# yangfei1223/CRFConv

Measured on AMD Instinct MI355X. Metric: M points/sec fwd+bwd, S3DIS 40960-pt cloud, K=16, 3 CRF iters; mIoU parity, higher is better.
Workload: dtype f32; 1 GPU; BASELINE configs[1]: S3DIS-like synthetic clouds (one point per 4 cm voxel of an 8x8x3 m box), 4 clouds x 40960 pts per GPU, K=16, ratios [4,4,4,4,2], PointConvBig(in=6, classes=13, use_crf, steps=3), train mode: fwd + weighted CE + bwd + flat-bucket grad all-reduce + SGD(momentum) step; tables resident in HBM; point order from the device collate: morton; global_batch=4, points_per_cloud=40960, parallelism=dp1 (batch-sharded)

## Files before the change

### crfconv_amd/_lib.py

```python
import ctypes
import os

_HERE = os.path.dirname(os.path.abspath(__file__))
LIB_PATH = os.environ.get('CRFCONV_LIB') or os.path.join(_HERE, 'libcrfconv_amd.so')

_vp, _i, _i64, _sz, _f = ctypes.c_void_p, ctypes.c_int, ctypes.c_int64, ctypes.c_size_t, ctypes.c_float
_d = ctypes.c_double
_u64 = ctypes.c_uint64

SIGNATURES = {
    'crfconv_abi_version': (_i, []),
    'crfconv_last_error': (ctypes.c_char_p, []),
    'crfconv_knn': (_i, [_vp, _sz, _sz, _vp, _sz, _sz, _vp]),
    'crfconv_knn_omp': (_i, [_vp, _sz, _sz, _vp, _sz, _sz, _vp]),
    'crfconv_knn_batch': (_i, [_vp, _sz, _sz, _sz, _vp, _sz, _sz, _vp]),
    'crfconv_knn_batch_omp': (_i, [_vp, _sz, _sz, _sz, _vp, _sz, _sz, _vp]),
    'crfconv_knn_batch_dev_workspace': (_sz, [_sz, _sz, _sz, _sz]),
    'crfconv_knn_batch_dev': (_i, [_vp, _sz, _sz, _sz, _vp, _sz, _sz, _vp, _vp, _vp, _sz, _vp]),
    'crfconv_fps': (_i, [_vp, _i, _vp, _vp, _vp, _vp, _vp, _vp, _vp, _vp]),
    'crfconv_grid_subsample': (_i64, [_vp, _i64, _vp, _i, _vp, _i, _f, _vp, _vp, _vp, _i64]),
    'crfconv_grid_subsample_dev_workspace': (_sz, [_i64, _i, _i]),
    'crfconv_grid_subsample_dev': (_i64, [_vp, _i64, _vp, _i, _vp, _i, _f, _vp, _vp, _vp, _i64, _vp, _sz, _vp]),
    'crfconv_index_narrow': (_i, [_vp, _i64, _i64, _i, _i64, _vp, _vp, _vp, _vp]),
    'crfconv_index_narrow_sorted': (_i, [_vp, _i64, _i64, _i, _i64, _i, _vp, _vp, _vp, _vp]),
    'crfconv_reverse_csr_workspace': (_sz, [_i64, _i64]),
    'crfconv_reverse_csr': (_i, [_vp, _i64, _i64, _vp, _vp, _vp, _sz, _vp]),
    'crfconv_reverse_csr_batched_workspace': (_sz, [_vp, _i]),
    'crfconv_reverse_csr_batched': (_i, [_vp, _i, _vp, _sz, _vp]),
    'crfconv_meanfield_forward': (_i, [_vp, _vp, _vp, _i, _i, _i64, _i, _vp, _vp, _i, _vp, _vp, _vp]),
    'crfconv_meanfield_forward_u16': (_i, [_vp, _vp, _vp, _vp, _i, _i, _i, _i, _i64, _i, _vp, _vp, _i, _vp, _vp, _vp]),
    'crfconv_meanfield_forward_block_rows': (_i, [_i64, _i, _i, _i, _i]),
    'crfconv_meanfield_forward_block': (_i, [_vp, _vp, _vp, _vp, _i, _i, _i, _i, _i64, _i, _vp, _vp, _i, _vp, _vp, _vp, _vp]),
    'crfconv_meanfield_forward_block_stamps': (_i, [_vp, _vp, _vp, _vp, _i, _i, _i64, _vp, _vp, _i, _vp, _vp, _vp, _i, _vp, _vp]),
    'crfconv_block_locality': (_i, [_vp, _i64, _i, _i, _i, _vp, _vp]),
    'crfconv_meanfield_bwd_edge': (_i, [_vp, _vp, _vp, _vp, _i, _i, _i64, _i, _vp, _vp, _vp, _vp, _i, _vp]),
    'crfconv_meanfield_bwd_scatter': (_i, [_vp, _vp, _vp, _vp, _i, _i, _i64, _i, _vp, _vp, _vp]),
    'crfconv_meanfield_backward_supported': (_i, [_i, _i, _i]),
    'crfconv_meanfield_backward_param_grads_inside': (_i, [_i]),
    'crfconv_meanfield_backward_workspace': (_sz, [_i64, _i, _i]),
    'crfconv_meanfield_backward': (_i, [_vp] * 7 + [_i, _i, _vp, _vp, _i, _i, _i64, _i, _vp, _vp, _i] + [_vp] * 11 + [_sz, _vp, _vp]),
    'crfconv_wide_similarity': (_i, [_vp, _vp, _i, _i, _i64, _i, _vp, _vp]),
    'crfconv_wide_aggregate': (_i, [_vp, _vp, _vp, _i, _i, _i64, _i, _vp, _vp]),
    'crfconv_wide_bwd_edge': (_i, [_vp, _vp, _vp, _i, _i, _i64, _i, _vp, _i, _vp]),
    'crfconv_wide_scatter': (_i, [_vp, _vp, _vp, _vp, _i, _i64, _i, _vp, _i, _vp, _vp]),
    'crfconv_wide_similarity_bwd': (_i, [_vp, _vp, _vp, _vp, _i, _i, _i64, _i, _vp, _vp, _vp]),
    'crfconv_similarity_bwd': (_i, [_vp, _vp, _vp, _vp, _i, _i, _i64, _i, _vp, _vp, _vp]),
    'crfconv_similarity_bwd_scatter': (_i, [_vp, _vp, _vp, _vp, _vp, _i, _i, _i64, _i, _vp, _vp]),
    'crfconv_pointconv_workspace': (_sz, [_i64, _i, _i]),
    'crfconv_pointconv_moments_packed': (_i, [_vp, _vp, _vp, _i, _i64, ctypes.c_double, _vp, _vp, _vp, _vp, _vp, _sz, _vp]),
    'crfconv_pointconv_moments': (_i, [_vp, _vp, _vp, _i, _i64, _vp, _vp, _sz, _vp]),
    'crfconv_pointconv_stats': (_i, [_vp, _vp, _vp, _i, _i64, _i, _vp, _vp, _vp, _f, _vp, _vp, _vp, _vp, _sz, _vp]),
    'crfconv_pointconv_forward_uv': (_i, [_vp, _vp, _vp, _vp, _i, _i64, _i, _vp, _vp, _vp, _f, _vp, _vp, _vp, _vp, _vp, _vp, _sz, _vp, _vp]),
    'crfconv_pointconv_forward_uv_hosts': (_i, [_i, _i]),
    'crfconv_pointconv_forward_uv_hosting': (_i, [_vp, _vp, _vp, _vp, _i, _i64, _i, _vp, _vp, _vp, _f, _vp, _vp, _vp, _vp, _vp, _vp, _sz, _vp,
                                                  _vp, _vp, _i, _vp, _vp, _vp]),
    'crfconv_pointconv_combine': (_i, [_vp, _vp, _vp, _vp, _vp, _vp, _d, _vp, _vp, _f, _f, _i64, _i, _vp, _vp, _vp, _vp, _vp]),
    'crfconv_pointconv_bwd_reduce_uv': (_i, [_vp, _vp, _vp, _i64, _i, _vp, _vp, _vp, _d, _i, _vp, _vp, _vp, _vp, _vp, _vp, _sz, _vp, _vp]),
    'crfconv_pointconv_forward': (_i, [_vp, _vp, _vp, _vp, _i, _i64, _i, _vp, _vp, _vp, _f, _vp, _vp, _vp, _vp]),
    'crfconv_pointconv_bwd_reduce': (_i, [_vp, _vp, _vp, _vp, _vp, _i, _i64, _i, _vp, _vp, _vp, _f, _vp, _vp, _vp, _sz, _vp]),
    'crfconv_pointconv_bwd_params': (_i, [_vp, _vp, _vp, _vp, _vp, _i, _i64, _i, _vp, _vp, _vp, _f, _vp, _vp, _vp,
                                          _vp, _vp, _vp, _sz, _vp]),
    'crfconv_pointconv_bwd_dump': (_i, [_vp, _vp, _vp, _vp, _vp, _i, _i64, _i, _vp, _vp, _vp, _f, _vp, _vp, _vp, _vp, _vp, _vp, _vp]),
    'crfconv_pointconv_bwd_a1_workspace': (_sz, [_i64, _i]),
    'crfconv_pointconv_bwd_a1': (_i, [_vp, _vp, _vp, _i64, _i, _f, _vp, _vp, _sz, _vp]),
    'crfconv_pointconv_bwd_input': (_i, [_vp, _vp, _vp, _vp, _vp, _i, _i64, _i, _vp, _vp, _vp, _f, _vp, _vp, _vp, _vp]),
    'crfconv_pointconv_bwd_input_reduce': (_i, [_vp, _vp, _vp, _vp, _vp, _i, _i64, _i64, _i, _vp, _vp, _vp, _f, _vp, _vp, _vp, _vp, _vp, _vp, _vp, _vp, _d, _i,
                                                _vp, _vp, _vp, _vp, _vp, _vp, _sz, _vp, _vp]),
    'crfconv_pointconv_fold1': (_i, [_vp, _vp, _vp, _vp, ctypes.c_double, _vp, _vp, _f, _f, _i, _i, _vp, _vp, _vp, _vp]),
    'crfconv_pointconv_fold1_batched': (_i, [_vp, _i, _vp]),
    'crfconv_pointconv_fold1_bwd_batched': (_i, [_vp, _i, _vp]),
    'crfconv_pointconv_fold1_bwd': (_i, [_vp, _vp, _vp, _vp, _vp, _f, _i, _i, _vp, _vp, _vp, _vp, _vp, _vp]),
    'crfconv_pointconv_fold2': (_i, [_vp, _vp, _vp, _vp, ctypes.c_double, _vp, _vp, _f, _f, _i, _i, _vp, _vp, _vp, _vp]),
    'crfconv_pointconv_fold2_bwd': (_i, [_vp, _vp, _vp, _vp, ctypes.c_double, _i, _i, _vp, _vp, _vp, _vp, _vp, _vp]),
    'crfconv_linear_wgrad_workspace': (_sz, [_i64, _i, _i]),
    'crfconv_linear_wgrad': (_i, [_vp, _vp, _i64, _i, _i, _vp, _vp, _vp, _sz, _vp]),
    'crfconv_random_subsets': (_i, [_vp, _vp, _vp, _vp, _i, _u64, _vp, _vp]),
    'crfconv_upindex_workspace': (_sz, [_i64, _i64]),
    'crfconv_upindex_from_table': (_i, [_vp, _vp, _vp, _vp, _i64, _i64, _i, _i64, _vp, _vp, _sz, _vp]),
    'crfconv_gather_rows_batched': (_i, [_vp, _vp, _vp, _i, _vp, _i, _i64, _i64, _i64, _vp]),
    'crfconv_argsort_codes_workspace': (_sz, [_i64, _i64]),
    'crfconv_argsort_codes': (_i, [_vp, _i64, _i64, _vp, _vp, _sz, _vp]),
    'crfconv_gridsync_workspace': (_sz, []),
    'crfconv_gridsync_fail_word': (_i, []),
    'crfconv_mlp_small_supported': (_i, [_i64, _i, _i]),
    'crfconv_mlp_small_workspace': (_sz, [_i64, _i]),
    'crfconv_mlp_small_forward': (_i, [_vp, _vp, _i64, _i, _i, _vp, _vp, _vp, _vp, _f, _f, _f, _vp, _vp, _vp, _vp, _sz, _vp, _sz, _vp]),
    'crfconv_mlp_small_forward_join': (_i, [_vp, _vp, _i64, _i, _i, _vp, _vp, _vp, _vp, _f, _f, _f, _vp, _f, _vp, _vp, _vp, _vp, _sz, _vp, _sz, _vp]),
    'crfconv_ticket_bytes': (_sz, []),
    'crfconv_mlp_backward_supported': (_i, [_i64, _i, _i]),
    'crfconv_mlp_backward_workspace': (_sz, [_i64, _i, _i]),
    'crfconv_mlp_backward': (_i, [_vp, _vp, _vp, _vp, _vp, _f, _i64, _i, _i, _vp, _vp, _vp, _vp, _vp, _sz, _vp, _vp]),
    'crfconv_linear_forward_cat': (_i, [_vp, _vp, _i, _vp, _vp, _i64, _i, _i, _vp, _vp, _vp]),
    'crfconv_mlp_dw_jobs': (_i, [_vp, _i, _vp]),
    'crfconv_mlp_dw_jobs_hosting': (_i, [_vp, _i, _vp, _vp, _vp, _vp, _vp, _i, _vp, _vp]),
    'crfconv_mlp_backward_add': (_i, [_vp, _vp, _vp, _vp, _vp, _f, _i64, _i, _i, _vp, _vp, _vp, _vp, _vp, _vp, _sz, _vp, _vp]),
    'crfconv_mlp_backward_cat': (_i, [_vp, _vp, _vp, _vp, _i, _vp, _vp, _f, _i64, _i, _i, _vp, _vp, _vp, _vp, _vp, _vp, _sz, _vp, _vp]),
    'crfconv_bn_workspace': (_sz, [_i64, _i]),
    'crfconv_bn_forward': (_i, [_vp, _i64, _i, _vp, _vp, _vp, _vp, _f, _f, _i, _f, _vp, _vp, _vp, _sz, _vp]),
    'crfconv_bn_backward': (_i, [_vp, _vp, _vp, _i64, _i, _i, _f, _vp, _vp, _vp, _vp, _sz, _vp]),
    'crfconv_bn_apply': (_i, [_vp, _i64, _i, _vp, _f, _vp, _vp]),
    'crfconv_pointconv_bwd_params_slabs': (_i, [_vp, _i64, _i, _vp, _vp, _vp]),
    'crfconv_pointconv_bwd_a1_nblk': (_i64, [_i64, _i]),
    'crfconv_reduce_jobs_f64': (_i, [_vp, _i, _vp]),
    'crfconv_pointconv_bwd_dump_jobs': (_i, [_vp, _i, _vp]),
    'crfconv_pointconv_bwd_a1_jobs': (_i, [_vp, _i, _vp]),
    'crfconv_pointconv_wide_params_supported': (_i, [_i64, _i, _i]),
    'crfconv_pointconv_wide_params_nblk': (_i64, [_i64, _i]),
    'crfconv_pointconv_wide_params_jobs': (_i, [_vp, _i, _vp]),
    'crfconv_gemm_jobs': (_i, [_vp, _i, _vp]),
    'crfconv_linear_wgrad_nblk': (_i, [_i64, _i, _i]),
    'crfconv_linear_wgrad_partial_jobs': (_i, [_vp, _i, _vp]),
    'crfconv_linear_wgrad_partial': (_i, [_vp, _vp, _i64, _i, _i, _i, _vp, _sz, _vp, _vp]),
    'crfconv_morton_codes': (_i, [_vp, _i64, _i64, _vp, _vp, _vp]),
    'crfconv_copy_jobs': (_i, [_vp, _i, _vp]),
    'crfconv_index_narrow_batched': (_i, [_vp, _i, _vp]),
    'crfconv_pointconv_moments_batched_workspace': (_sz, [_vp, _i]),
    'crfconv_pointconv_moments_batched': (_i, [_vp, _i, _vp, _sz, _vp]),
    'crfconv_reduce_jobs_both': (_i, [_vp, _i, _vp, _i, _vp]),
    'crfconv_reduce_jobs': (_i, [_vp, _i, _vp]),
    'crfconv_linear_forward_supported': (_i, [_i, _i]),
    'crfconv_linear_forward_stat_records': (_sz, [_i64]),
    'crfconv_linear_forward': (_i, [_vp, _vp, _vp, _i64, _i, _i, _i, _vp, _vp, _vp]),
    'crfconv_cat2': (_i, [_vp, _vp, _i64, _i, _i, _vp, _vp]),
    'crfconv_split2': (_i, [_vp, _i64, _i, _i, _vp, _vp, _vp]),
    'crfconv_add_i64': (_i, [_vp, _i64, _i64, _vp]),
    'crfconv_gate_mark': (_i, [_vp, _vp]),
    'crfconv_gate_wait': (_i, [_vp, _i, _vp]),
    'crfconv_mlp_small_backward_supported': (_i, [_i64, _i, _i]),
    'crfconv_gemm_stats_jobs': (_i, [_vp, _i, _vp]),
    'crfconv_bn_apply_from_records_jobs': (_i, [_vp, _i, _vp]),
    'crfconv_mlp_small_backward_jobs': (_i, [_vp, _i, _vp, _vp]),
    'crfconv_mlp_small_backward_jobs_one_launch': (_i, [_vp, _i, _vp, _vp, _vp]),
    'crfconv_mlp_small_backward_workspace': (_sz, [_i64, _i]),
    'crfconv_mlp_small_backward': (_i, [_vp, _vp, _vp, _vp, _vp, _i64, _i, _i, _i, _f, _vp, _vp, _vp, _vp, _vp, _sz, _vp, _vp]),
    'crfconv_gemm_stat_records': (_sz, [_i64]),
    'crfconv_gemm_stats': (_i, [_vp, _vp, _i64, _i, _i, _vp, _vp, _vp]),
    'crfconv_gemm_supported': (_i, [_i64, _i, _i]),
    'crfconv_gemm': (_i, [_vp, _vp, _vp, _vp, _i64, _i, _i, _i, _vp, _vp]),
    'crfconv_bn_apply_from_records': (_i, [_vp, _i64, _vp, _i64, _i, _vp, _vp, _vp, _vp, _f, _f, _vp, _f, _vp, _vp, _vp]),
    'crfconv_bn_coef_from_nrecords': (_i, [_vp, _i64, _i64, _i, _vp, _vp, _vp, _vp, _f, _f, _vp, _vp]),
    'crfconv_bn_coef_from_records': (_i, [_vp, _i64, _i, _vp, _vp, _vp, _vp, _f, _f, _vp, _vp]),
    'crfconv_softmax_ce_workspace': (_sz, [_i64]),
    'crfconv_softmax_ce_forward': (_i, [_vp, _vp, _vp, _i64, _i, _i64, _i64, _vp, _vp, _vp, _vp, _sz, _vp, _vp]),
    'crfconv_softmax_ce_backward': (_i, [_vp, _vp, _vp, _vp, _vp, _vp, _i64, _i, _i64, _i64, _vp, _vp]),
    'crfconv_crf_matrices': (_i, [_vp, _i, _vp, _vp, _vp]),
    'crfconv_crf_matrices_backward': (_i, [_vp, _vp, _vp, _vp, _i, _vp, _vp]),
    'crfconv_crf_matrices_batched': (_i, [_vp, _vp, _i, _vp, _vp, _vp]),
    'crfconv_crf_matrices_backward_batched': (_i, [_vp, _vp, _vp, _vp, _vp, _i, _vp, _vp]),
    'crfconv_add_lrelu': (_i, [_vp, _vp, _i64, _f, _vp, _vp]),
    'crfconv_bn_apply_add': (_i, [_vp, _i64, _i, _vp, _vp, _f, _vp, _vp]),
    'crfconv_bn_apply_dropout': (_i, [_vp, _i64, _i, _vp, _f, _f, _u64, _vp, _vp, _vp, _vp]),
    'crfconv_head_stats': (_i, [_vp, _vp, _i64, _i, _i, _vp, _vp]),
    'crfconv_head_stat_records': (_sz, [_i64]),
    'crfconv_head_supported': (_i, [_i64, _i, _i, _i]),
    'crfconv_head_mask_words': (_sz, [_i64]),
    'crfconv_head_backward_workspace': (_sz, [_i64, _i, _i, _i]),
    'crfconv_head_forward': (_i, [_vp, _vp, _vp, _f, _f, _u64, _vp, _vp, _vp, _i64, _i, _i, _i, _vp, _vp, _vp, _vp]),
    'crfconv_head_backward': (_i, [_vp, _vp, _vp, _vp, _f, _f, _vp, _vp, _i64, _i, _i, _i] + [_vp] * 7 + [_sz, _vp]),
    'crfconv_linear_forward_dropout': (_i, [_vp, _vp, _i64, _i, _i, _i, _f, _u64, _vp, _vp, _vp]),
    'crfconv_dropout_backward': (_i, [_vp, _i64, _f, _u64, _vp, _vp, _vp]),
    'crfconv_add_lrelu_backward': (_i, [_vp, _vp, _i64, _f, _vp, _vp]),
    'crfconv_sgd_step': (_i, [_vp, _vp, _vp, _i64, _f, _f, _f, _f, _i, _i, _vp]),
    'crfconv_sgd_step_hyper': (_i, [_vp, _vp, _vp, _i64, _vp, _i, _i, _vp]),
    'crfconv_sgd_step_guarded': (_i, [_vp, _vp, _vp, _i64, _vp, _i, _i, _vp, _vp]),
    'crfconv_sgd_step_guarded_all': (_i, [_vp, _vp, _vp, _i64, _vp, _i, _i, _vp, _i, _vp, _vp]),
    'crfconv_sgd_guard_publish': (_i, [_vp, _i, _vp, _vp]),
    'crfconv_spd_inverse': (_i, [_vp, _i, _vp, _vp]),
    'crfconv_spd_inverse_wide': (_i, [_vp, _i, _vp, _vp]),
    'crfconv_neighbor_maxpool_forward': (_i, [_vp, _vp, _i, _i64, _i, _vp, _vp, _vp]),
    'crfconv_neighbor_maxpool_affine_forward': (_i, [_vp, _vp, _vp, _i, _i64, _i, _vp, _vp, _vp]),
    'crfconv_neighbor_maxpool_backward': (_i, [_vp, _vp, _vp, _vp, _i, _i64, _i, _vp, _vp]),
    'crfconv_gather_rows': (_i, [_vp, _vp, _i64, _i, _vp, _vp]),
    'crfconv_gather_rows_backward': (_i, [_vp, _vp, _vp, _i64, _i, _vp, _vp]),
    'crfconv_meanfield_step': (_i, [_vp, _vp, _vp, _vp, _i, _i, _i64, _i, _vp, _vp, _vp, _vp]),
    'crfconv_kernel_weights_forward': (_i, [_vp, _vp, _i, _vp, _i, _i, _i64, _vp, _vp]),
    'crfconv_kernel_weights_partials': (_sz, [_i64]),
    'crfconv_kernel_weights_backward': (_i, [_vp, _vp, _vp, _vp, _vp, _i, _vp, _i, _i, _i64, _vp, _vp, _vp, _vp]),
    'crfconv_confusion_accumulate': (_i, [_vp, _vp, _vp, _i64, _i, _i64, _i64, _vp, _vp, _vp]),
    'crfconv_vote_accumulate': (_i, [_vp, _vp, _vp, _i64, _i, _d, _vp, _i64, _vp, _vp]),
    'crfconv_vote_accumulate_counted': (_i, [_vp, _vp, _vp, _i64, _i, _d, _vp, _i64, _vp, _vp, _vp]),
    'crfconv_vote_fold': (_i, [_vp, _vp, _vp, _vp, _i64, _i, _d, _vp]),
    'crfconv_vote_project': (_i, [_vp, _vp, _i64, _i, _i64, _i, _vp, _vp, _vp]),
    'crfconv_argmin_workspace': (_sz, []),
    'crfconv_argmin_f64': (_i, [_vp, _i64, _vp, _vp, _vp, _sz, _vp]),
    'crfconv_possibility_crop_workspace': (_sz, [_i64, _i64]),
    'crfconv_possibility_crop': (_i, [_vp, _i64, _i64, _vp, _vp, _vp, _vp, _vp, _vp, _vp, _vp, _vp, _sz, _vp]),
}



class ReduceJob(ctypes.Structure):
    _fields_ = [('partial', ctypes.c_void_p), ('out', ctypes.c_void_p), ('nblk', ctypes.c_int32), ('nslots', ctypes.c_int32)]


class CopyJob(ctypes.Structure):
    _fields_ = [('src', ctypes.c_void_p), ('dst', ctypes.c_void_p), ('nbytes', ctypes.c_int64)]


class MlpDwJob(ctypes.Structure):
    _fields_ = [('workspace', ctypes.c_void_p), ('coef', ctypes.c_void_p), ('dW', ctypes.c_void_p), ('M', ctypes.c_int64),
                ('Ci', ctypes.c_int32), ('Co', ctypes.c_int32)]


class PcDumpJob(ctypes.Structure):
    _fields_ = [('x', ctypes.c_void_p), ('gout', ctypes.c_void_p), ('pos_src', ctypes.c_void_p), ('pos_tgt', ctypes.c_void_p),
                ('idx32', ctypes.c_void_p), ('K', ctypes.c_int32), ('m_tgt', ctypes.c_int64), ('d', ctypes.c_int32), ('A1', ctypes.c_void_p),
                ('b1', ctypes.c_void_p), ('W2', ctypes.c_void_p), ('slope', ctypes.c_float), ('ca', ctypes.c_void_p), ('cb', ctypes.c_void_p),
                ('cc', ctypes.c_void_p), ('h1', ctypes.c_void_p), ('gh2', ctypes.c_void_p), ('rel', ctypes.c_void_p)]


class PcWideJob(ctypes.Structure):
    _fields_ = [('x', ctypes.c_void_p), ('gout', ctypes.c_void_p), ('pos_src', ctypes.c_void_p), ('pos_tgt', ctypes.c_void_p),
                ('idx32', ctypes.c_void_p), ('K', ctypes.c_int32), ('m_tgt', ctypes.c_int64), ('d', ctypes.c_int32), ('A1', ctypes.c_void_p),
                ('b1', ctypes.c_void_p), ('W2', ctypes.c_void_p), ('slope', ctypes.c_float), ('ca', ctypes.c_void_p), ('cb', ctypes.c_void_p),
                ('cc', ctypes.c_void_p), ('dw2_partial', ctypes.c_void_p), ('a1_partial', ctypes.c_void_p)]


class PcA1Job(ctypes.Structure):
    _fields_ = [('gw', ctypes.c_void_p), ('h1', ctypes.c_void_p), ('rel', ctypes.c_void_p), ('n_edges', ctypes.c_int64), ('d', ctypes.c_int32),
                ('slope', ctypes.c_float), ('workspace', ctypes.c_void_p), ('workspace_bytes', ctypes.c_size_t)]


class GemmJob(ctypes.Structure):
    _fields_ = [('A', ctypes.c_void_p), ('B', ctypes.c_void_p), ('C', ctypes.c_void_p), ('M', ctypes.c_int64), ('N', ctypes.c_int32),
                ('K', ctypes.c_int32)]


class GemmStatsJob(ctypes.Structure):
    _fields_ = [('A', ctypes.c_void_p), ('B', ctypes.c_void_p), ('M', ctypes.c_int64), ('N', ctypes.c_int32), ('K', ctypes.c_int32),
                ('C', ctypes.c_void_p), ('stat_rec', ctypes.c_void_p)]


class BnApplyJob(ctypes.Structure):
    _fields_ = [('stat_rec', ctypes.c_void_p), ('nrec', ctypes.c_int64), ('x', ctypes.c_void_p), ('M', ctypes.c_int64), ('C', ctypes.c_int32),
                ('gamma', ctypes.c_void_p), ('beta', ctypes.c_void_p), ('run_mean', ctypes.c_void_p), ('run_var', ctypes.c_void_p),
                ('momentum', ctypes.c_float), ('eps', ctypes.c_float), ('skip', ctypes.c_void_p), ('slope', ctypes.c_float),
                ('coef', ctypes.c_void_p), ('y', ctypes.c_void_p)]


class MlpBwdJob(ctypes.Structure):
    _fields_ = [('gA', ctypes.c_void_p), ('Y', ctypes.c_void_p), ('coef', ctypes.c_void_p), ('W', ctypes.c_void_p), ('addend', ctypes.c_void_p),
                ('M', ctypes.c_int64), ('Ci', ctypes.c_int32), ('Co', ctypes.c_int32), ('training', ctypes.c_int32), ('slope', ctypes.c_float),
                ('gY', ctypes.c_void_p), ('dX', ctypes.c_void_p), ('dgamma', ctypes.c_void_p), ('dbeta', ctypes.c_void_p),
                ('workspace', ctypes.c_void_p), ('workspace_bytes', ctypes.c_size_t)]


class Reduce64Job(ctypes.Structure):
    _fields_ = [('partial', ctypes.c_void_p), ('is_float', ctypes.c_int32), ('nblk', ctypes.c_int64), ('nslots', ctypes.c_int32),
                ('out', ctypes.c_void_p)]


class WgradJob(ctypes.Structure):
    _fields_ = [('G', ctypes.c_void_p), ('X', ctypes.c_void_p), ('M', ctypes.c_int64), ('Co', ctypes.c_int32), ('Ci', ctypes.c_int32),
                ('want_bias', ctypes.c_int32), ('workspace', ctypes.c_void_p), ('workspace_bytes', ctypes.c_size_t)]


class RevJob(ctypes.Structure):
    _fields_ = [('idx32', ctypes.c_void_p), ('E', ctypes.c_int64), ('m_src', ctypes.c_int64), ('rev_ptr', ctypes.c_void_p),
                ('rev_eid', ctypes.c_void_p)]


class NarrowJob(ctypes.Structure):
    _fields_ = [('idx64', ctypes.c_void_p), ('B', ctypes.c_int64), ('n_tgt', ctypes.c_int64), ('K', ctypes.c_int32),
                ('n_src', ctypes.c_int64), ('sort_from', ctypes.c_int32), ('idx32', ctypes.c_void_p), ('idx16', ctypes.c_void_p),
                ('bad_count', ctypes.c_void_p)]


class MomentsJob(ctypes.Structure):
    _fields_ = [('pos_src', ctypes.c_void_p), ('pos_tgt', ctypes.c_void_p), ('idx32', ctypes.c_void_p), ('K', ctypes.c_int32),
                ('m_tgt', ctypes.c_int64), ('n_edges', ctypes.c_double), ('mean', ctypes.c_void_p), ('cov', ctypes.c_void_p),
                ('packed', ctypes.c_void_p), ('mean32', ctypes.c_void_p)]


class Fold1Job(ctypes.Structure):
    _fields_ = [('W1', ctypes.c_void_p), ('gamma1', ctypes.c_void_p), ('beta1', ctypes.c_void_p), ('mom', ctypes.c_void_p),
                ('n_edges', ctypes.c_double), ('run_mean', ctypes.c_void_p), ('run_var', ctypes.c_void_p),
                ('momentum', ctypes.c_float), ('eps', ctypes.c_float), ('use_batch', ctypes.c_int32), ('d', ctypes.c_int32),
                ('A1', ctypes.c_void_p), ('b1', ctypes.c_void_p), ('aux1', ctypes.c_void_p)]


class Fold1BwdJob(ctypes.Structure):
    _fields_ = [('W1', ctypes.c_void_p), ('gamma1', ctypes.c_void_p), ('mom', ctypes.c_void_p), ('aux1', ctypes.c_void_p),
                ('dA1b1', ctypes.c_void_p), ('eps', ctypes.c_float), ('use_batch', ctypes.c_int32), ('d', ctypes.c_int32),
                ('pad_', ctypes.c_int32), ('dW1', ctypes.c_void_p), ('dgamma1', ctypes.c_void_p), ('dbeta1', ctypes.c_void_p),
                ('dW2_f64', ctypes.c_void_p), ('dW2_f32', ctypes.c_void_p)]


_lib = None


class CrfConvError(RuntimeError):
    pass


def load():
    global _lib
    if _lib is None:
        if not os.path.exists(LIB_PATH):
            raise CrfConvError(
                '%s not found: build it with `make -C crfconv_amd/csrc` (or __graft_entry__.build()). '
                'crfconv_amd has no CPU / PyTorch fallback.' % LIB_PATH)
        lib = ctypes.CDLL(LIB_PATH)
        for name, (res, args) in SIGNATURES.items():
            fn = getattr(lib, name)
            fn.restype = res
            fn.argtypes = args
        if lib.crfconv_abi_version() != 1:
            raise CrfConvError('libcrfconv_amd.so ABI version mismatch')
        _lib = lib
    return _lib


def last_error():
    return load().crfconv_last_error().decode('utf-8', 'replace')


def check(rc, what=''):
    if rc < 0:
        raise CrfConvError('%s failed (%d): %s' % (what or 'libcrfconv_amd call', rc, last_error()))
    return rc


_FN = {}


def call(name, *args):
    fn = _FN.get(name)
    if fn is None:
        fn = _FN[name] = getattr(load(), name)
    rc = fn(*args)
    if rc < 0:
        check(rc, name)
    return rc
```

### crfconv_amd/csrc/linear.hip

```cpp
#include "common.hpp"
#include "gridsync.hpp"
#include "wgrad_body.hpp"
#include "crf_matrices_body.hpp"
#include "reduce64_body.hpp"

#include <cstdlib>

namespace crf {

template <int TCO, int TCI>
__global__ __launch_bounds__(WG_BLOCK) void wgrad_kernel(const float* __restrict__ G,
                                                         const float* __restrict__ X, int64_t M, int Co,
                                                         int Ci, int rows_per_block,
                                                         float* __restrict__ partial ,
                                                         float* __restrict__ partial_b ) {
    __shared__ float s_red[WG_RED_BUFS * TCO * TCI * 256];
    __shared__ float s_b[WG_WAVES * TCO * 16];
    wgrad_body<TCO, TCI>(G, X, M, Co, Ci, rows_per_block, partial, partial_b, blockIdx.x, blockIdx.y, blockIdx.z, s_red, s_b);
}

__global__ __launch_bounds__(WG_BLOCK) void wgrad_jobs_any_kernel(const WgJobTable t) {
    __shared__ float s_red[WG_RED_BUFS * 4 * 4 * 256];
    __shared__ float s_b[WG_WAVES * 4 * 16];
    wgrad_any_run(t, (int)blockIdx.x, s_red, s_b);
}


__device__ __forceinline__ void mlp_channel_part(int c, double s1, double s2, const float* __restrict__ coef, int64_t M, int Co,
                                                 float* __restrict__ dgamma, float* __restrict__ dbeta, float* __restrict__ bcoef) {
    dbeta[c] = (float)s1;
    dgamma[c] = (float)s2;
    const double a = coef[c], mu = coef[2 * Co + c], rs = coef[3 * Co + c];
    const double c2 = s1 / (double)M, c3 = s2 / (double)M;
    bcoef[c] = coef[c];
    bcoef[Co + c] = coef[Co + c];
    bcoef[2 * Co + c] = (float)a;
    bcoef[3 * Co + c] = (float)(-a * c3 * rs);
    bcoef[4 * Co + c] = (float)(-a * c2 + a * c3 * rs * mu);
}

template <int TCO, int TCI>
__global__ __launch_bounds__(WG_BLOCK) void mlp_bwd_p1_kernel(const float* __restrict__ GA, const float* __restrict__ Y,
                                                              const float* __restrict__ X,
                                                              const float* __restrict__ X2, int split ,
                                                              const float* __restrict__ coef ,
                                                              float slope, int64_t M, int Co, int Ci, int rows_per_block,
                                                              float* __restrict__ PA ,
                                                              float* __restrict__ PB ,
                                                              float* __restrict__ PG ,
                                                              float* __restrict__ PX ,
                                                              unsigned* __restrict__ ticket ,
                                                              float* __restrict__ dgamma, float* __restrict__ dbeta,
                                                              float* __restrict__ bcoef) {
    const int lane = threadIdx.x & 63, wave = threadIdx.x >> 6;
    const int co_base = blockIdx.y * 16 * TCO, ci_base = blockIdx.z * 16 * TCI;
    const int kk = lane >> 4, cc = lane & 15;
    f32x4 accA[TCO][TCI], accB[TCO][TCI];
#pragma unroll
    for (int a = 0; a < TCO; ++a)
#pragma unroll
        for (int b = 0; b < TCI; ++b) { accA[a][b] = f32x4{0.f, 0.f, 0.f, 0.f}; accB[a][b] = f32x4{0.f, 0.f, 0.f, 0.f}; }
    float ca[TCO], cb[TCO], cm[TCO], cr[TCO], sg[TCO], sgy[TCO], sx[TCI];
#pragma unroll
    for (int a = 0; a < TCO; ++a) {
        const int co = co_base + 16 * a + cc;
        const bool ok = co < Co;
        ca[a] = ok ? coef[co] : 0.f;
        cb[a] = ok ? coef[Co + co] : 0.f;
        cm[a] = ok ? coef[2 * Co + co] : 0.f;
        cr[a] = ok ? coef[3 * Co + co] : 0.f;
        sg[a] = 0.f;
        sgy[a] = 0.f;
    }
#pragma unroll
    for (int b = 0; b < TCI; ++b) sx[b] = 0.f;

    const int64_t row_begin = (int64_t)blockIdx.x * rows_per_block;
    const int64_t row_end = row_begin + rows_per_block < M ? row_begin + rows_per_block : M;
#ifndef P1_PREFETCH_
#define P1_PREFETCH_ 0
#endif
    struct Frag { float gv[4][TCO], yv[4][TCO], bv[4][TCI]; };
    auto load = [&](int64_t r0, Frag& f) {
#pragma unroll
        for (int u = 0; u < 4; ++u) {
            const int64_t r = r0 + 4 * u + kk;
            const bool rv = r < row_end;
#pragma unroll
            for (int a = 0; a < TCO; ++a) {
                const int co = co_base + 16 * a + cc;
                const bool ok = rv && co < Co;
                f.gv[u][a] = ok ? GA[r * Co + co] : 0.f;
                f.yv[u][a] = ok ? Y[r * Co + co] : cm[a];
            }
#pragma unroll
            for (int b = 0; b < TCI; ++b) {
                const int ci = ci_base + 16 * b + cc;
                float xv = 0.f;
                if (rv && ci < Ci) xv = (X2 == nullptr || ci < split) ? X[r * (X2 ? split : Ci) + ci] : X2[r * (Ci - split) + (ci - split)];
                f.bv[u][b] = xv;
            }
        }
    };
    auto compute = [&](const Frag& f) {
#pragma unroll
        for (int u = 0; u < 4; ++u) {
#pragma unroll
            for (int b = 0; b < TCI; ++b) sx[b] += f.bv[u][b];
#pragma unroll
            for (int a = 0; a < TCO; ++a) {
                const float g1 = f.gv[u][a] * (fmaf(ca[a], f.yv[u][a], cb[a]) > 0.f ? 1.f : slope);
                const float yh = (f.yv[u][a] - cm[a]) * cr[a];
                sg[a] += g1;
                sgy[a] = fmaf(g1, yh, sgy[a]);
#pragma unroll
                for (int b = 0; b < TCI; ++b) {
                    accA[a][b] = __builtin_amdgcn_mfma_f32_16x16x4f32(g1, f.bv[u][b], accA[a][b], 0, 0, 0);
                    accB[a][b] = __builtin_amdgcn_mfma_f32_16x16x4f32(yh, f.bv[u][b], accB[a][b], 0, 0, 0);
                }
            }
        }
    };
    if constexpr (P1_PREFETCH_ != 0) {
        Frag cur, nxt;
        load(row_begin + 16 * wave, cur);
        for (int64_t r0 = row_begin + 16 * wave; r0 < row_end; r0 += 16 * WG_WAVES) {
            load(r0 + 16 * WG_WAVES, nxt);
            compute(cur);
            cur = nxt;
        }
    } else {
        for (int64_t r0 = row_begin + 16 * wave; r0 < row_end; r0 += 16 * WG_WAVES) {
            Frag f;
            load(r0, f);
            compute(f);
        }
    }
    __shared__ __attribute__((aligned(16))) float s_red[WG_WAVES][TCO * TCI * 256];
    __shared__ float s_v[WG_WAVES][(2 * TCO + TCI) * 16];
    const int64_t pb = (int64_t)blockIdx.x;
    for (int pass = 0; pass < 2; ++pass) {
        if (pass) __syncthreads();
#pragma unroll
        for (int a = 0; a < TCO; ++a)
#pragma unroll
            for (int b = 0; b < TCI; ++b)
#pragma unroll
                for (int g = 0; g < 4; ++g)
                    s_red[wave][(a * TCI + b) * 256 + (4 * kk + g) * 16 + cc] = pass ? accB[a][b][g] : accA[a][b][g];
        if (pass == 0) {
#pragma unroll
            for (int a = 0; a < TCO; ++a) {
                float t1 = sg[a], t2 = sgy[a];
                t1 += __shfl_xor(t1, 16, WAVE); t1 += __shfl_xor(t1, 32, WAVE);
                t2 += __shfl_xor(t2, 16, WAVE); t2 += __shfl_xor(t2, 32, WAVE);
                if (kk == 0) { s_v[wave][a * 16 + cc] = t1; s_v[wave][(TCO + a) * 16 + cc] = t2; }
            }
#pragma unroll
            for (int b = 0; b < TCI; ++b) {
                float t1 = sx[b];
                t1 += __shfl_xor(t1, 16, WAVE); t1 += __shfl_xor(t1, 32, WAVE);
                if (kk == 0) s_v[wave][(2 * TCO + b) * 16 + cc] = t1;
            }
        }
        __syncthreads();
        float* dst = pass ? PB : PA;
        for (int t = threadIdx.x; t < TCO * TCI * 256; t += WG_BLOCK) {
            float v = 0.f;
#pragma unroll
            for (int w = 0; w < WG_WAVES; ++w) v += s_red[w][t];
            const int tile = t >> 8, a = tile / TCI, b = tile % TCI, i = (t >> 4) & 15, j = t & 15;
            const int co = co_base + 16 * a + i, ci = ci_base + 16 * b + j;
            if (co < Co && ci < Ci) dst[(pb * Co + co) * Ci + ci] = v;
        }
    }
    const __amdgpu_buffer_rsrc_t pgr = make_rsrc(PG, (int)gridDim.x * 2 * Co * 4);
    for (int t = threadIdx.x; t < (2 * TCO + TCI) * 16; t += WG_BLOCK) {
        float v = 0.f;
#pragma unroll
        for (int w = 0; w < WG_WAVES; ++w) v += s_v[w][t];
        const int grp = t >> 4, c16 = t & 15;
        if (grp < 2 * TCO) {
            const int which = grp / TCO, co = co_base + 16 * (grp % TCO) + c16;
            if (blockIdx.z == 0 && co < Co) st1_sc1(pgr, (((int)pb * 2 + which) * Co + co) * 4, v);
        } else {
            const int ci = ci_base + 16 * (grp - 2 * TCO) + c16;
            if (blockIdx.y == 0 && ci < Ci) PX[pb * Ci + ci] = v;
        }
    }
    constexpr bool ALIAS = TCO * TCI >= 3;
    __shared__ double s_own[ALIAS ? 1 : 5 * WG_BLOCK];
    __shared__ int s_flag;
    if (ticket == nullptr || !last_workgroup(ticket, gridDim.x * gridDim.y * gridDim.z, &s_flag)) return;
    double* s_buf = ALIAS ? reinterpret_cast<double*>(&s_red[0][0]) : s_own;
    double* s_tot = s_buf + 4 * WG_BLOCK;
    sum_partial_rows_f64<WG_BLOCK>(pgr, (int)gridDim.x, 2 * Co, s_buf, s_tot);
    if ((int)threadIdx.x < Co) mlp_channel_part(threadIdx.x, s_tot[threadIdx.x], s_tot[Co + threadIdx.x], coef, M, Co, dgamma, dbeta, bcoef);
}

constexpr int MF_BLOCK = 1024, MF_WAVES = MF_BLOCK / WAVE;
__device__ __forceinline__ void mlp_dw_slots(const float* __restrict__ PA, const float* __restrict__ PB,
                                             const float* __restrict__ PG, const float* __restrict__ PX, int nblk,
                                             const float* __restrict__ coef, int64_t M, int Co, int Ci, int block,
                                             float* __restrict__ dW) {
    const int lane = threadIdx.x & 63, w = threadIdx.x >> 6;
    __shared__ float s_part[MF_WAVES][5][64];
    const int nslots = Co * Ci;
    const int slot = block * 64 + lane;
    const bool ok = slot < nslots;
    const int sl = ok ? slot : nslots - 1;
    const int co = sl / Ci, ci = sl - co * Ci;
    float a0 = 0.f, b0 = 0.f, x0 = 0.f, g1 = 0.f, g2 = 0.f;
    const int64_t sa = (int64_t)MF_WAVES * Co * Ci, sx = (int64_t)MF_WAVES * Ci, sg = (int64_t)MF_WAVES * 2 * Co;
    const float* pa = PA + ((int64_t)w * Co + co) * Ci + ci;
    const float* pb = PB + ((int64_t)w * Co + co) * Ci + ci;
    const float* px = PX + (int64_t)w * Ci + ci;
    const float* pg = PG + (int64_t)w * 2 * Co + co;
#pragma unroll 1
    for (int b = w; b < nblk; b += 4 * MF_WAVES) {
        float va[4], vb[4], vx[4], vg[4], vh[4];
#pragma unroll
        for (int u = 0; u < 4; ++u) {
            const bool in = b + MF_WAVES * u < nblk;
            va[u] = in ? pa[u * sa] : 0.f;
            vb[u] = in ? pb[u * sa] : 0.f;
            vx[u] = in ? px[u * sx] : 0.f;
            vg[u] = in ? pg[u * sg] : 0.f;
            vh[u] = in ? pg[u * sg + Co] : 0.f;
        }
#pragma unroll
        for (int u = 0; u < 4; ++u) { a0 += va[u]; b0 += vb[u]; x0 += vx[u]; g1 += vg[u]; g2 += vh[u]; }
        pa += 4 * sa; pb += 4 * sa; px += 4 * sx; pg += 4 * sg;
    }
    s_part[w][0][lane] = a0; s_part[w][1][lane] = b0; s_part[w][2][lane] = x0;
    s_part[w][3][lane] = g1; s_part[w][4][lane] = g2;
    __syncthreads();
    if (w == 0 && ok) {
        double A = 0.0, B = 0.0, Xs = 0.0, G1 = 0.0, G2 = 0.0;
        for (int k = 0; k < MF_WAVES; ++k) {
            A += s_part[k][0][lane]; B += s_part[k][1][lane]; Xs += s_part[k][2][lane];
            G1 += s_part[k][3][lane]; G2 += s_part[k][4][lane];
        }
        const double a = coef[co], c2 = G1 / (double)M, c3 = G2 / (double)M;
        dW[slot] = (float)(a * (A - c2 * Xs - c3 * B));
    }
}

__global__ __launch_bounds__(MF_BLOCK) void mlp_bwd_finalize_kernel(const float* __restrict__ PA, const float* __restrict__ PB,
                                                                    const float* __restrict__ PG, const float* __restrict__ PX,
                                                                    int nblk, const float* __restrict__ coef, int64_t M, int Co,
                                                                    int Ci, int nw, float* __restrict__ dW,
                                                                    float* __restrict__ dgamma, float* __restrict__ dbeta,
                                                                    float* __restrict__ bcoef) {
    const int lane = threadIdx.x & 63, w = threadIdx.x >> 6;
    if ((int)blockIdx.x >= nw) {
        const int c = ((int)blockIdx.x - nw) * MF_WAVES + w;
        if (c >= Co) return;
        double s1 = 0.0, s2 = 0.0;
        for (int b0 = lane; b0 < nblk; b0 += 8 * WAVE) {
            float v1[8], v2[8];
#pragma unroll
            for (int u = 0; u < 8; ++u) {
                const int b = b0 + u * WAVE;
                const bool in = b < nblk;
                v1[u] = in ? PG[((int64_t)b * 2 + 0) * Co + c] : 0.f;
                v2[u] = in ? PG[((int64_t)b * 2 + 1) * Co + c] : 0.f;
            }
#pragma unroll
            for (int u = 0; u < 8; ++u) { s1 += (double)v1[u]; s2 += (double)v2[u]; }
        }
#pragma unroll
        for (int o = 32; o > 0; o >>= 1) {
            s1 += __shfl_xor(s1, o, WAVE);
            s2 += __shfl_xor(s2, o, WAVE);
        }
        if (lane == 0) mlp_channel_part(c, s1, s2, coef, M, Co, dgamma, dbeta, bcoef);
        return;
    }
    mlp_dw_slots(PA, PB, PG, PX, nblk, coef, M, Co, Ci, (int)blockIdx.x, dW);
}

constexpr int MDW_MAX = 40;
struct MlpDwTable {
    const float* PA[MDW_MAX];
    const float* PB[MDW_MAX];
    const float* PG[MDW_MAX];
    const float* PX[MDW_MAX];
    const float* coef[MDW_MAX];
    float* dW[MDW_MAX];
    long long M[MDW_MAX];
    int nblk[MDW_MAX], Co[MDW_MAX], Ci[MDW_MAX];
    int group_begin[MDW_MAX + 1];
    int njobs;
};
__global__ __launch_bounds__(MF_BLOCK) void mlp_dw_jobs_kernel(const MlpDwTable t) {
    const int g = blockIdx.x;
    int lo = 0, hi = t.njobs;
    while (hi - lo > 1) {
        const int mid = (lo + hi) >> 1;
        if (t.group_begin[mid] <= g) lo = mid; else hi = mid;
    }
    mlp_dw_slots(t.PA[lo], t.PB[lo], t.PG[lo], t.PX[lo], t.nblk[lo], t.coef[lo], (int64_t)t.M[lo], t.Co[lo], t.Ci[lo],
                 g - t.group_begin[lo], t.dW[lo]);
}

__device__ __forceinline__ void reduce_slab64(const float* __restrict__ partial, int nblk, int nslots, int slot0,
                                              float* __restrict__ out, float (*s_part)[64]) {
    const int lane = threadIdx.x & 63, w = threadIdx.x >> 6;
    const int slot = slot0 + lane;
    const bool ok = slot < nslots;
    const float* p = partial + (ok ? slot : 0);
    float a0 = 0.f, a1 = 0.f, a2 = 0.f, a3 = 0.f;
    int b = w;
    for (; b + 28 < nblk; b += 32) {
        const float v0 = p[(int64_t)b * nslots], v1 = p[(int64_t)(b + 4) * nslots], v2 = p[(int64_t)(b + 8) * nslots];
        const float v3 = p[(int64_t)(b + 12) * nslots], v4 = p[(int64_t)(b + 16) * nslots], v5 = p[(int64_t)(b + 20) * nslots];
        const float v6 = p[(int64_t)(b + 24) * nslots], v7 = p[(int64_t)(b + 28) * nslots];
        a0 += v0; a1 += v1; a2 += v2; a3 += v3;
        a0 += v4; a1 += v5; a2 += v6; a3 += v7;
    }
    for (; b + 12 < nblk; b += 16) {
        a0 += p[(int64_t)b * nslots];
        a1 += p[(int64_t)(b + 4) * nslots];
        a2 += p[(int64_t)(b + 8) * nslots];
        a3 += p[(int64_t)(b + 12) * nslots];
    }
    for (; b < nblk; b += 4) a0 += p[(int64_t)b * nslots];
    s_part[w][lane] = (a0 + a1) + (a2 + a3);
    __syncthreads();
    if (w == 0 && ok) out[slot] = ((s_part[0][lane] + s_part[1][lane]) + s_part[2][lane]) + s_part[3][lane];
}

__global__ __launch_bounds__(256) void wgrad_reduce_kernel(const float* __restrict__ partial, int nblk,
                                                           int nslots, float* __restrict__ out) {
    __shared__ float s_part[4][64];
    reduce_slab64(partial, nblk, nslots, blockIdx.x * 64, out, s_part);
}

constexpr int RJ_MAX = 96;
struct ReduceJobTable {
    const float* partial[RJ_MAX];
    float* out[RJ_MAX];
    int nblk[RJ_MAX];
    int nslots[RJ_MAX];
    int group_begin[RJ_MAX + 1];
    int njobs;
};

__global__ __launch_bounds__(256) void reduce_jobs_kernel(const ReduceJobTable tbl) {
    __shared__ float s_part[4][64];
    const int g = blockIdx.x;
    int lo = 0, hi = tbl.njobs;
    while (hi - lo > 1) {
        const int mid = (lo + hi) >> 1;
        if (tbl.group_begin[mid] <= g) lo = mid; else hi = mid;
    }
    reduce_slab64(tbl.partial[lo], tbl.nblk[lo], tbl.nslots[lo], (g - tbl.group_begin[lo]) * 64, tbl.out[lo], s_part);
}


__global__ __launch_bounds__(256) void reduce_both_kernel(const ReduceJobTable tbl, const Reduce64Table t64, const int n64) {
    __shared__ float s_part[4][64];
    if ((int)blockIdx.x < n64) {
        reduce_jobs_f64_body(t64, blockIdx.x);
        return;
    }
    const int g = (int)blockIdx.x - n64;
    int lo = 0, hi = tbl.njobs;
    while (hi - lo > 1) {
        const int mid = (lo + hi) >> 1;
        if (tbl.group_begin[mid] <= g) lo = mid; else hi = mid;
    }
    reduce_slab64(tbl.partial[lo], tbl.nblk[lo], tbl.nslots[lo], (g - tbl.group_begin[lo]) * 64, tbl.out[lo], s_part);
}

}

using namespace crf;

extern "C" size_t crfconv_linear_wgrad_workspace(int64_t M, int Co, int Ci) {
    if (M <= 0 || Co <= 0 || Ci <= 0) return 0;
    const WgPlan p = wg_plan(M, Co, Ci);
    return sizeof(float) * (size_t)p.nblk * ((size_t)Co * Ci + (size_t)Co) + 256;
}

static int wgrad_launch(const float* G, const float* X, int64_t M, int Co, int Ci, const WgPlan& p, float* partial,
                        float* partial_b, hipStream_t st) {
    const dim3 grid((unsigned)p.nblk, (unsigned)p.gy, (unsigned)p.gz), blk(WG_BLOCK);
#define WG(TA, TB) hipLaunchKernelGGL((wgrad_kernel<TA, TB>), grid, blk, 0, st, G, X, M, Co, Ci, p.rows_per_block, partial, partial_b)
    switch (p.tco * 10 + p.tci) {
        case 11: WG(1, 1); break;
        case 12: WG(1, 2); break;
        case 14: WG(1, 4); break;
        case 21: WG(2, 1); break;
        case 22: WG(2, 2); break;
        case 24: WG(2, 4); break;
        case 41: WG(4, 1); break;
        case 42: WG(4, 2); break;
        default: WG(4, 4); break;
    }
#undef WG
    CRF_LAUNCH_CHECK();
    return CRF_OK;
}

extern "C" int crfconv_linear_wgrad_partial(const float* G, const float* X, int64_t M, int Co, int Ci, int want_bias,
                                            void* workspace, size_t workspace_bytes, int* nblk_out, crf_stream_t stream) {
// ... 65 lines not shown
    }
    return CRF_OK;
}

extern "C" int crfconv_reduce_jobs_f64(const crf_reduce64_job* jobs, int njobs, crf_stream_t stream);
extern "C" int crfconv_reduce_jobs_both(const crf_reduce_job* jobs, int njobs, const crf_reduce64_job* jobs64, int njobs64,
                                        crf_stream_t stream) {
    CRF_REQUIRE((jobs || njobs == 0) && (jobs64 || njobs64 == 0) && njobs >= 0 && njobs64 >= 0, CRF_ERR_ARG, "null pointer or negative count");
    if (njobs == 0 || njobs64 == 0 || njobs > RJ_MAX || njobs64 > R64_MAX) {
        if (njobs64 > 0)
            if (int rc = crfconv_reduce_jobs_f64(jobs64, njobs64, stream)) return rc;
        return njobs > 0 ? crfconv_reduce_jobs(jobs, njobs, stream) : CRF_OK;
    }
    ReduceJobTable tbl;
    int64_t total = 0;
    for (int j = 0; j < njobs; ++j) {
        const crf_reduce_job& jb = jobs[j];
        CRF_REQUIRE(jb.partial && jb.out && jb.nblk > 0 && jb.nslots > 0, CRF_ERR_ARG, "job %d is malformed", j);
        tbl.partial[j] = jb.partial; tbl.out[j] = jb.out; tbl.nblk[j] = jb.nblk; tbl.nslots[j] = jb.nslots;
        tbl.group_begin[j] = (int)total;
        total += (jb.nslots + 63) / 64;
    }
    for (int j = njobs; j <= RJ_MAX; ++j) tbl.group_begin[j] = (int)total;
    for (int j = njobs; j < RJ_MAX; ++j) { tbl.partial[j] = nullptr; tbl.out[j] = nullptr; tbl.nblk[j] = 0; tbl.nslots[j] = 0; }
    tbl.njobs = njobs;
    Reduce64Table t;
    int64_t waves = 0;
    for (int j = 0; j <= R64_MAX; ++j) {
        t.wave_base[j] = (int)waves;
        if (j < njobs64) {
            const crf_reduce64_job& jb = jobs64[j];
            CRF_REQUIRE(jb.partial && jb.out && jb.nblk > 0 && jb.nblk < ((int64_t)1 << 31) && jb.nslots > 0, CRF_ERR_ARG, "float64 job %d is malformed", j);
            t.partial[j] = jb.partial; t.out[j] = jb.out; t.is_float[j] = jb.is_float; t.nblk[j] = (int)jb.nblk; t.nslots[j] = jb.nslots;
            waves += jb.nslots;
        } else if (j < R64_MAX) {
            t.partial[j] = nullptr; t.out[j] = nullptr; t.is_float[j] = 0; t.nblk[j] = 0; t.nslots[j] = 0;
        }
    }
    t.njobs = njobs64;
    const int64_t n64 = cdiv(waves, 256 / WAVE);
    CRF_REQUIRE(total + n64 < ((int64_t)1 << 30), CRF_ERR_UNSUPPORTED, "too many slots in one batch");
    hipLaunchKernelGGL(reduce_both_kernel, dim3((unsigned)(total + n64)), dim3(256), 0, as_stream(stream), tbl, t, (int)n64);
    CRF_LAUNCH_CHECK();
    return CRF_OK;
}

extern "C" int crfconv_linear_wgrad(const float* G, const float* X, int64_t M, int Co, int Ci, float* dW,
                                    float* db, void* workspace, size_t workspace_bytes, crf_stream_t stream) {
    CRF_REQUIRE(G && X && dW && workspace, CRF_ERR_ARG, "null pointer");
    CRF_REQUIRE(M > 0 && Co > 0 && Ci > 0 && Co <= 4096 && Ci <= 4096, CRF_ERR_ARG, "bad shape M=%lld Co=%d Ci=%d",
                (long long)M, Co, Ci);
    CRF_REQUIRE(workspace_bytes >= crfconv_linear_wgrad_workspace(M, Co, Ci), CRF_ERR_WORKSPACE, "workspace too small");
    const WgPlan p = wg_plan(M, Co, Ci);
    hipStream_t st = as_stream(stream);
    float* partial = reinterpret_cast<float*>((reinterpret_cast<uintptr_t>(workspace) + 255) & ~(uintptr_t)255);
    float* partial_b = db ? partial + (size_t)p.nblk * Co * Ci : nullptr;
    if (int rc = wgrad_launch(G, X, M, Co, Ci, p, partial, partial_b, st)) return rc;
    hipLaunchKernelGGL(wgrad_reduce_kernel, dim3((unsigned)cdiv((int64_t)Co * Ci, 64)), dim3(256), 0, st, partial, p.nblk,
                       Co * Ci, dW);
    CRF_LAUNCH_CHECK();
    if (db) {
        hipLaunchKernelGGL(wgrad_reduce_kernel, dim3((unsigned)cdiv((int64_t)Co, 64)), dim3(256), 0, st, partial_b, p.nblk,
                           Co, db);
        CRF_LAUNCH_CHECK();
    }
    return CRF_OK;
}

namespace crf {
__device__ __forceinline__ void gauss_jordan_tiles(double (&t)[4][4], int H, double (*s_row)[64], double (*s_col)[64]) {
    const int tr = threadIdx.x >> 4, tc = threadIdx.x & 15;
#pragma unroll
    for (int ip = 0; ip < 4; ++ip) {
        for (int pp = 0; pp < 16; ++pp) {
            const int p = 16 * ip + pp;
            if (p >= H) break;
            const int b = p & 1;
            if (tr == pp) {
#pragma unroll
                for (int j = 0; j < 4; ++j) s_row[b][tc + 16 * j] = t[ip][j];
            }
            if (tc == pp) {
#pragma unroll
                for (int i = 0; i < 4; ++i) s_col[b][tr + 16 * i] = t[i][ip];
            }
            __syncthreads();
            const double piv = 1.0 / s_row[b][p];
            double rowv[4], colv[4];
#pragma unroll
            for (int j = 0; j < 4; ++j) rowv[j] = s_row[b][tc + 16 * j] * piv;
#pragma unroll
            for (int i = 0; i < 4; ++i) colv[i] = s_col[b][tr + 16 * i];
#pragma unroll
            for (int i = 0; i < 4; ++i)
#pragma unroll
                for (int j = 0; j < 4; ++j) {
                    const bool rp = (i == ip) && (tr == pp), cp = (j == ip) && (tc == pp);
                    const double upd = t[i][j] - colv[i] * rowv[j];
                    t[i][j] = rp ? (cp ? piv : rowv[j]) : (cp ? -colv[i] * piv : upd);
                }
        }
    }
}

__global__ __launch_bounds__(256) void spd_inverse_kernel(const float* __restrict__ Min, int H,
                                                          float* __restrict__ Qout) {
    __shared__ double s_row[2][64], s_col[2][64];
    const int tr = threadIdx.x >> 4, tc = threadIdx.x & 15;
    double t[4][4];
#pragma unroll
    for (int i = 0; i < 4; ++i)
#pragma unroll
        for (int j = 0; j < 4; ++j) {
            const int r = tr + 16 * i, c = tc + 16 * j;
            t[i][j] = (r < H && c < H) ? (double)Min[r * H + c] : (r == c ? 1.0 : 0.0);
        }
    gauss_jordan_tiles(t, H, s_row, s_col);
#pragma unroll
    for (int i = 0; i < 4; ++i)
#pragma unroll
        for (int j = 0; j < 4; ++j) {
            const int r = tr + 16 * i, c = tc + 16 * j;
            if (r < H && c < H) Qout[r * H + c] = (float)t[i][j];
        }
}

__global__ __launch_bounds__(CMF_BLOCK) void crf_matrices_kernel(const float* __restrict__ cmat, int H,
                                                           float* __restrict__ Qout, float* __restrict__ Pout) {
    __shared__ __attribute__((aligned(16))) char lds[CMF_LDS_BYTES];
    crf_matrices_body(cmat, H, Qout, Pout, lds);
}

__global__ __launch_bounds__(CMF_BLOCK) void crf_matrices_batched_kernel(const CrfMatJobs j) {
    const int b = blockIdx.x;
    __shared__ __attribute__((aligned(16))) char lds[CMF_LDS_BYTES];
    crf_matrices_body(j.c[b], j.H[b], j.Q[b], j.P[b], lds);
}

constexpr int CMB_ROWS = 8, CMB_BLOCK = CMB_ROWS * 64;
__device__ __forceinline__ void crf_matrices_bwd_slab(const float* __restrict__ cmat, const float* __restrict__ Q,
                                                      const float* __restrict__ dQ, const float* __restrict__ dP,
                                                      int H, int row0, float* __restrict__ dc) {
    __shared__ float s_q[64 * 65], s_d[64 * 65];
    __shared__ double s_t[2][CMB_ROWS][65];
    for (int e = threadIdx.x; e < H * H; e += (int)blockDim.x) {
        const int r = e / H, c = e % H;
        s_q[r * 65 + c] = Q[e];
        s_d[r * 65 + c] = (dQ ? dQ[e] : 0.f) - (dP ? dP[e] : 0.f);
    }
    const int r = (threadIdx.x >> 6) & (CMB_ROWS - 1), j = threadIdx.x & 63, row = row0 + r;
    const bool live = (int)threadIdx.x < CMB_BLOCK && row < H && j < H;
    if (live) s_t[0][r][j] = (double)cmat[row * H + j];
    __syncthreads();
    double acc = 0.0;
    if (live)
        for (int k = 0; k < H; ++k) acc += s_t[0][r][k] * (double)s_q[k * 65 + j];
    if (live) s_t[1][r][j] = acc;
    __syncthreads();
    acc = 0.0;
    if (live)
        for (int k = 0; k < H; ++k) acc += s_t[1][r][k] * ((double)s_d[k * 65 + j] + (double)s_d[j * 65 + k]);
    if (live) s_t[0][r][j] = acc;
    __syncthreads();
    acc = 0.0;
    if (live) {
        for (int k = 0; k < H; ++k) acc += s_t[0][r][k] * (double)s_q[k * 65 + j];
        dc[row * H + j] = (float)(-acc);
    }
}
__global__ __launch_bounds__(CMB_BLOCK) void crf_matrices_bwd_kernel(const float* __restrict__ cmat, const float* __restrict__ Q,
                                                               const float* __restrict__ dQ, const float* __restrict__ dP,
                                                               int H, float* __restrict__ dc) {
    crf_matrices_bwd_slab(cmat, Q, dQ, dP, H, (int)blockIdx.x * CMB_ROWS, dc);
}
__global__ __launch_bounds__(CMB_BLOCK) void crf_matrices_bwd_batched_kernel(const CrfMatJobs j) {
    int b = 0;
    while (b + 1 < CM_MAX && (int)blockIdx.x >= j.slab_base[b + 1]) ++b;
    crf_matrices_bwd_slab(j.c[b], j.Q_in[b], j.gQ[b], j.gP[b], j.H[b], ((int)blockIdx.x - j.slab_base[b]) * CMB_ROWS, j.dc[b]);
}
static_assert(MF_BLOCK >= CMB_BLOCK, "a rider fits the host's workgroup");
__global__ __launch_bounds__(MF_BLOCK) void mlp_dw_jobs_hosting_kernel(const MlpDwTable t, const CrfMatJobs j, const int n_side) {
    if ((int)blockIdx.x < n_side) {
        int b = 0;
        while (b + 1 < CM_MAX && (int)blockIdx.x >= j.slab_base[b + 1]) ++b;
        crf_matrices_bwd_slab(j.c[b], j.Q_in[b], j.gQ[b], j.gP[b], j.H[b], ((int)blockIdx.x - j.slab_base[b]) * CMB_ROWS, j.dc[b]);
        return;
    }
    const int g = (int)blockIdx.x - n_side;
    int lo = 0, hi = t.njobs;
    while (hi - lo > 1) {
        const int mid = (lo + hi) >> 1;
        if (t.group_begin[mid] <= g) lo = mid; else hi = mid;
    }
    mlp_dw_slots(t.PA[lo], t.PB[lo], t.PG[lo], t.PX[lo], t.nblk[lo], t.coef[lo], (int64_t)t.M[lo], t.Co[lo], t.Ci[lo],
                 g - t.group_begin[lo], t.dW[lo]);
}
}

extern "C" int crfconv_crf_matrices_batched(const float* const* c, const int* H, int n, float* const* Q, float* const* P,
                                            crf_stream_t stream) {
    CRF_REQUIRE(c && H && Q && P && n >= 1 && n <= crf::CM_MAX, CRF_ERR_ARG, "null pointer or n=%d outside [1, %d]", n, crf::CM_MAX);
    crf::CrfMatJobs j = {};
    for (int i = 0; i < n; ++i) {
        CRF_REQUIRE(c[i] && Q[i] && P[i] && H[i] >= 1 && H[i] <= 64, CRF_ERR_ARG, "job %d: null pointer or H=%d outside [1, 64]", i, H[i]);
        j.c[i] = c[i]; j.Q[i] = Q[i]; j.P[i] = P[i]; j.H[i] = H[i];
    }
    hipLaunchKernelGGL(crf::crf_matrices_batched_kernel, dim3((unsigned)n), dim3(crf::CMF_BLOCK), 0, crf::as_stream(stream), j);
    CRF_LAUNCH_CHECK();
    return CRF_OK;
}

static int crf_matrices_bwd_jobs(const float* const* c, const float* const* Q, const float* const* gQ, const float* const* gP, const int* H, int n,
                                 float* const* dc, crf::CrfMatJobs& j, int& nslab) {
    CRF_REQUIRE(c && Q && gQ && gP && H && dc && n >= 1 && n <= crf::CM_MAX, CRF_ERR_ARG, "null pointer or n=%d outside [1, %d]", n, crf::CM_MAX);
    j = crf::CrfMatJobs();
    for (int i = 0; i < n; ++i) {
        CRF_REQUIRE(c[i] && Q[i] && dc[i] && H[i] >= 1 && H[i] <= 64, CRF_ERR_ARG, "job %d: null pointer or H=%d outside [1, 64]", i, H[i]);
        j.c[i] = c[i]; j.Q_in[i] = Q[i]; j.gQ[i] = gQ[i]; j.gP[i] = gP[i]; j.dc[i] = dc[i]; j.H[i] = H[i];
        j.slab_base[i + 1] = j.slab_base[i] + (H[i] + crf::CMB_ROWS - 1) / crf::CMB_ROWS;
    }
    nslab = j.slab_base[n];
    for (int i = n; i < crf::CM_MAX; ++i) j.slab_base[i + 1] = 0x7fffffff;
    return CRF_OK;
}
extern "C" int crfconv_crf_matrices_backward_batched(const float* const* c, const float* const* Q, const float* const* gQ,
                                                     const float* const* gP, const int* H, int n, float* const* dc,
                                                     crf_stream_t stream) {
    crf::CrfMatJobs j;
    int nslab = 0;
    if (int rc = crf_matrices_bwd_jobs(c, Q, gQ, gP, H, n, dc, j, nslab)) return rc;
    hipLaunchKernelGGL(crf::crf_matrices_bwd_batched_kernel, dim3((unsigned)nslab), dim3(crf::CMB_BLOCK), 0, crf::as_stream(stream), j);
    CRF_LAUNCH_CHECK();
    return CRF_OK;
}

namespace crf {
constexpr int SW_BLOCK = 1024, SW_MAXH = 512;
__global__ __launch_bounds__(SW_BLOCK) void spd_inverse_wide_kernel(const float* __restrict__ M, int H, float* __restrict__ Q) {
    __shared__ float s_row[SW_MAXH], s_col[SW_MAXH];
    const int n = H * H;
    for (int e = threadIdx.x; e < n; e += SW_BLOCK) Q[e] = M[e];
    __syncthreads();
    for (int k = 0; k < H; ++k) {
        for (int t = threadIdx.x; t < H; t += SW_BLOCK) {
            s_row[t] = Q[k * H + t];
            s_col[t] = Q[t * H + k];
        }
        __syncthreads();
        const float inv = 1.0f / s_row[k];
        for (int e = threadIdx.x; e < n; e += SW_BLOCK) {
            const int i = e / H, j = e - i * H;
            float v;
            if (i == k) v = j == k ? inv : s_row[j] * inv;
            else if (j == k) v = -s_col[i] * inv;
            else v = fmaf(-s_col[i] * inv, s_row[j], Q[e]);
            Q[e] = v;
        }
        __syncthreads();
    }
}
}

extern "C" int crfconv_spd_inverse_wide(const float* M, int H, float* Q, crf_stream_t stream) {
    CRF_REQUIRE(M && Q && M != Q, CRF_ERR_ARG, "null pointer / aliased operands");
    CRF_REQUIRE(H >= 1 && H <= crf::SW_MAXH, CRF_ERR_UNSUPPORTED, "H=%d outside [1, %d]", H, crf::SW_MAXH);
    hipLaunchKernelGGL(crf::spd_inverse_wide_kernel, dim3(1), dim3(crf::SW_BLOCK), 0, crf::as_stream(stream), M, H, Q);
    CRF_LAUNCH_CHECK();
    return CRF_OK;
}

extern "C" int crfconv_spd_inverse(const float* M, int H, float* Q, crf_stream_t stream) {
    CRF_REQUIRE(M && Q, CRF_ERR_ARG, "null pointer");
    CRF_REQUIRE(H >= 1 && H <= 64, CRF_ERR_UNSUPPORTED, "H=%d outside [1, 64]", H);
    hipLaunchKernelGGL(crf::spd_inverse_kernel, dim3(1), dim3(256), 0, crf::as_stream(stream), M, H, Q);
    CRF_LAUNCH_CHECK();
    return CRF_OK;
}

extern "C" int crfconv_crf_matrices(const float* c, int H, float* Q, float* P, crf_stream_t stream) {
    CRF_REQUIRE(c && Q && P, CRF_ERR_ARG, "null pointer");
    CRF_REQUIRE(H >= 1 && H <= 64, CRF_ERR_UNSUPPORTED, "H=%d outside [1, 64]", H);
    hipLaunchKernelGGL(crf::crf_matrices_kernel, dim3(1), dim3(crf::CMF_BLOCK), 0, crf::as_stream(stream), c, H, Q, P);
    CRF_LAUNCH_CHECK();
    return CRF_OK;
}

extern "C" int crfconv_crf_matrices_backward(const float* c, const float* Q, const float* dQ, const float* dP, int H,
                                             float* dc, crf_stream_t stream) {
    CRF_REQUIRE(c && Q && dc, CRF_ERR_ARG, "null pointer");
    CRF_REQUIRE(H >= 1 && H <= 64, CRF_ERR_UNSUPPORTED, "H=%d outside [1, 64]", H);
    hipLaunchKernelGGL(crf::crf_matrices_bwd_kernel, dim3((unsigned)((H + crf::CMB_ROWS - 1) / crf::CMB_ROWS)), dim3(crf::CMB_BLOCK), 0,
                       crf::as_stream(stream), c, Q, dQ, dP, H, dc);
    CRF_LAUNCH_CHECK();
    return CRF_OK;
}

namespace crf {

#ifndef LF_BLOCK_
#define LF_BLOCK_ 256
#endif
constexpr int LF_BLOCK = LF_BLOCK_, LF_WAVES = LF_BLOCK / WAVE;

constexpr int EPI_NONE = 0, EPI_ADD = 1, EPI_DROPOUT = 2;
#ifndef LF_PF_MAX_
#define LF_PF_MAX_ 4
#endif
template <int TCO, bool PRO = false, bool VEC4 = true, int EPI = EPI_NONE, int NCH = 0>
__global__ __launch_bounds__(LF_BLOCK) void linear_fwd_kernel(const float* __restrict__ X, const float* __restrict__ W,
                                                              const float* __restrict__ bias, int64_t M, int Ci, int Co,
                                                              int transpose_w, float* __restrict__ Y,
                                                              float* __restrict__ stat_partial ,
                                                              const float* __restrict__ Y2 = nullptr,
                                                              const float* __restrict__ pro = nullptr, float slope = 1.f,
                                                              const float* __restrict__ Xb = nullptr, int xsplit = 0,
                                                              float* __restrict__ Yb = nullptr, int ysplit = 0,
                                                              const float* __restrict__ addend = nullptr,
                                                              const long long* __restrict__ drop_counter = nullptr,
                                                              unsigned long long drop_seed = 0ull, unsigned drop_threshold = 0u,
                                                              float drop_scale = 1.f) {
    extern __shared__ float sW[];
    const int Cip = ((Ci + 15) / 16) * 16 + 4;
    const int Cik = ((Ci + 15) / 16) * 16;
    float* sPro = sW + 16 * TCO * Cip;
    [[maybe_unused]] float* sTile = sPro + (PRO ? 5 * Cik : 0);
    if constexpr (PRO) {
        for (int t = threadIdx.x; t < 5 * Cik; t += LF_BLOCK) {
            const int which = t / Cik, k = t - which * Cik;
            sPro[t] = k < Ci ? pro[which * Ci + k] : 0.f;
        }
    }
    const int co_base = blockIdx.y * 16 * TCO;
    if (!transpose_w && (Ci % 4) == 0) {
        const int Cip4 = Cip / 4, Ci4 = Ci / 4;
        for (int t = threadIdx.x; t < 16 * TCO * Cip4; t += LF_BLOCK) {
            const int r = t / Cip4, k4 = t - r * Cip4;
            const int co = co_base + r;
            float4 v = make_float4(0.f, 0.f, 0.f, 0.f);
            if (co < Co && k4 < Ci4) v = *reinterpret_cast<const float4*>(W + (int64_t)co * Ci + 4 * k4);
            *reinterpret_cast<float4*>(sW + r * Cip + 4 * k4) = v;
        }
    } else {
        for (int t = threadIdx.x; t < 16 * TCO * Cip; t += LF_BLOCK) {
            const int r = t / Cip, k = t - r * Cip;
            const int co = co_base + r;
            float v = 0.f;
            if (co < Co && k < Ci) v = transpose_w ? W[(int64_t)k * Co + co] : W[(int64_t)co * Ci + k];
            sW[t] = v;
        }
    }
    __syncthreads();
    const int lane = threadIdx.x & 63, wave = threadIdx.x >> 6;
    const int rr = lane & 15, g = lane >> 4;
    const bool vec = (Ci % 4) == 0;
    float bsel[TCO][4];
#pragma unroll
    for (int t = 0; t < TCO; ++t)
#pragma unroll
        for (int e = 0; e < 4; ++e) {
            const int co = co_base + 16 * t + 4 * g + e;
            bsel[t][e] = (bias != nullptr && co < Co) ? bias[co] : 0.f;
        }
    float s1[TCO][4], s2[TCO][4], sh[TCO][4];
#pragma unroll
    for (int t = 0; t < TCO; ++t)
#pragma unroll
        for (int e = 0; e < 4; ++e) { s1[t][e] = 0.f; s2[t][e] = 0.f; sh[t][e] = 0.f; }
    bool have_shift = false;
    const int nchunk = (Ci + 15) / 16;

    const float4 zero4 = make_float4(0.f, 0.f, 0.f, 0.f);
    auto load_raw = [&](int64_t r, bool rv, int c, float4& xa, float4& xb2) {
        const int k0 = 16 * c + 4 * g;
        xa = zero4;
        xb2 = zero4;
        if (!rv || k0 >= Ci) return;
        if constexpr (PRO) {
            xa = *reinterpret_cast<const float4*>(X + r * Ci + k0);
            xb2 = *reinterpret_cast<const float4*>(Y2 + r * Ci + k0);
        } else if (Xb != nullptr) {
            if (k0 < xsplit) xa = *reinterpret_cast<const float4*>(X + r * xsplit + k0);
            else xa = *reinterpret_cast<const float4*>(Xb + r * (Ci - xsplit) + (k0 - xsplit));
        } else if (VEC4 || vec) {
            xa = *reinterpret_cast<const float4*>(X + r * Ci + k0);
        } else if constexpr (!VEC4) {
            const float* xp = X + r * Ci;
            xa.x = xp[k0];
            xa.y = k0 + 1 < Ci ? xp[k0 + 1] : 0.f;
            xa.z = k0 + 2 < Ci ? xp[k0 + 2] : 0.f;
            xa.w = k0 + 3 < Ci ? xp[k0 + 3] : 0.f;
        }
    };
    auto operand = [&](bool rv, int c, float4 gv, float4 yv) -> float4 {
        if constexpr (PRO) {
            const int k0 = 16 * c + 4 * g;
            float4 xv = zero4;
            if (rv && k0 < Ci) {
                const float4 pa = *reinterpret_cast<const float4*>(sPro + k0), pb = *reinterpret_cast<const float4*>(sPro + Cik + k0);
                const float4 al = *reinterpret_cast<const float4*>(sPro + 2 * Cik + k0), be = *reinterpret_cast<const float4*>(sPro + 3 * Cik + k0);
                const float4 de = *reinterpret_cast<const float4*>(sPro + 4 * Cik + k0);
                xv.x = fmaf(al.x * (fmaf(pa.x, yv.x, pb.x) > 0.f ? 1.f : slope), gv.x, fmaf(be.x, yv.x, de.x));
                xv.y = fmaf(al.y * (fmaf(pa.y, yv.y, pb.y) > 0.f ? 1.f : slope), gv.y, fmaf(be.y, yv.y, de.y));
                xv.z = fmaf(al.z * (fmaf(pa.z, yv.z, pb.z) > 0.f ? 1.f : slope), gv.z, fmaf(be.z, yv.z, de.z));
                xv.w = fmaf(al.w * (fmaf(pa.w, yv.w, pb.w) > 0.f ? 1.f : slope), gv.w, fmaf(be.w, yv.w, de.w));
            }
            return xv;
        } else {
            return gv;
        }
    };
    constexpr int NCA = NCH > 0 ? NCH : 1;
    constexpr bool PF = NCH > 0 && NCH <= LF_PF_MAX_;
    const int64_t row_stride = (int64_t)gridDim.x * (LF_BLOCK / WAVE) * 16;
    [[maybe_unused]] float4 fa[NCA], fb[PRO ? NCA : 1], na[PF ? NCA : 1], nb[(PF && PRO) ? NCA : 1];
    [[maybe_unused]] auto load_group = [&](int64_t rw0, float4 (&xa)[NCA], float4 (&xb)[PRO ? NCA : 1]) {
        const int64_t rq = rw0 + rr;
        const bool ok = rw0 < M && rq < M;
#pragma unroll
        for (int c = 0; c < NCA; ++c) {
            float4 t0, t1;
            load_raw(rq, ok, c, t0, t1);
            xa[c] = t0;
            if constexpr (PRO) xb[c] = t1;
        }
    };
    if constexpr (PF) load_group(((int64_t)blockIdx.x * (LF_BLOCK / WAVE) + wave) * 16, fa, fb);
    for (int64_t row0 = ((int64_t)blockIdx.x * (LF_BLOCK / WAVE) + wave) * 16; row0 < M; row0 += row_stride) {
        const int64_t r = row0 + rr;
        const bool rv = r < M;
        f32x4 acc[TCO];
#pragma unroll
        for (int t = 0; t < TCO; ++t) acc[t] = f32x4{bsel[t][0], bsel[t][1], bsel[t][2], bsel[t][3]};
        if constexpr (NCH > 0) {
            if constexpr (PF) {
                if constexpr (PRO) load_group(row0 + row_stride, na, nb);
                else load_group(row0 + row_stride, na, fb);
            } else {
                load_group(row0, fa, fb);
            }
#pragma unroll
            for (int c = 0; c < NCH; ++c) {
                const int k0 = 16 * c + 4 * g;
                const float4 xv = operand(rv, c, fa[c], fb[PRO ? c : 0]);
#pragma unroll
                for (int t = 0; t < TCO; ++t) {
                    const float4 wv = *reinterpret_cast<const float4*>(sW + (16 * t + rr) * Cip + k0);
                    acc[t] = __builtin_amdgcn_mfma_f32_16x16x4f32(wv.x, xv.x, acc[t], 0, 0, 0);
                    acc[t] = __builtin_amdgcn_mfma_f32_16x16x4f32(wv.y, xv.y, acc[t], 0, 0, 0);
                    acc[t] = __builtin_amdgcn_mfma_f32_16x16x4f32(wv.z, xv.z, acc[t], 0, 0, 0);
                    acc[t] = __builtin_amdgcn_mfma_f32_16x16x4f32(wv.w, xv.w, acc[t], 0, 0, 0);
                }
            }
            if constexpr (PF) {
#pragma unroll
                for (int c = 0; c < NCH; ++c) {
                    fa[c] = na[c];
                    if constexpr (PRO) fb[c] = nb[c];
                }
            }
        } else {
        for (int c = 0; c < nchunk; ++c) {
            const int k0 = 16 * c + 4 * g;
            float4 ra, rb;
            load_raw(r, rv, c, ra, rb);
            const float4 xv = operand(rv, c, ra, rb);
#pragma unroll
            for (int t = 0; t < TCO; ++t) {
                const float4 wv = *reinterpret_cast<const float4*>(sW + (16 * t + rr) * Cip + k0);
                acc[t] = __builtin_amdgcn_mfma_f32_16x16x4f32(wv.x, xv.x, acc[t], 0, 0, 0);
                acc[t] = __builtin_amdgcn_mfma_f32_16x16x4f32(wv.y, xv.y, acc[t], 0, 0, 0);
                acc[t] = __builtin_amdgcn_mfma_f32_16x16x4f32(wv.z, xv.z, acc[t], 0, 0, 0);
                acc[t] = __builtin_amdgcn_mfma_f32_16x16x4f32(wv.w, xv.w, acc[t], 0, 0, 0);
            }
        }
        }
        if constexpr (TCO >= 2) {
            constexpr int TW = 16 * TCO, TLD = TW + 4, F4R = TW / 4;
            float* tile = sTile + wave * 16 * TLD;
#pragma unroll
            for (int t = 0; t < TCO; ++t)
                *reinterpret_cast<float4*>(tile + rr * TLD + 16 * t + 4 * g) = make_float4(acc[t][0], acc[t][1], acc[t][2], acc[t][3]);
            __builtin_amdgcn_wave_barrier();
#pragma unroll
            for (int i = 0; i < (16 * F4R) / WAVE; ++i) {
                const int qd = lane + WAVE * i, trow = qd / F4R, tc4 = qd - trow * F4R;
                const int64_t orow = row0 + trow;
                const int co = co_base + 4 * tc4;
                if (orow < M && co < Co) {
                    float4 o4 = *reinterpret_cast<const float4*>(tile + trow * TLD + 4 * tc4);
                    if constexpr (EPI == EPI_ADD) {
                        {
                            if (VEC4 || (Co % 4) == 0) {
                                const float4 a4 = *reinterpret_cast<const float4*>(addend + orow * Co + co);
                                o4.x += a4.x; o4.y += a4.y; o4.z += a4.z; o4.w += a4.w;
                            } else {
                                o4.x += addend[orow * Co + co];
                                if (co + 1 < Co) o4.y += addend[orow * Co + co + 1];
                                if (co + 2 < Co) o4.z += addend[orow * Co + co + 2];
                                if (co + 3 < Co) o4.w += addend[orow * Co + co + 3];
                            }
                        }
                    }
                    if constexpr (EPI == EPI_DROPOUT) {
                        {
                            const unsigned long long ctr = (unsigned long long)drop_counter[0];
                            const unsigned long long e = (unsigned long long)(orow * Co + co);
                            o4.x = dropout_keep(drop_seed, ctr, e, drop_threshold) ? o4.x * drop_scale : 0.f;
                            o4.y = dropout_keep(drop_seed, ctr, e + 1, drop_threshold) ? o4.y * drop_scale : 0.f;
                            o4.z = dropout_keep(drop_seed, ctr, e + 2, drop_threshold) ? o4.z * drop_scale : 0.f;
                            o4.w = dropout_keep(drop_seed, ctr, e + 3, drop_threshold) ? o4.w * drop_scale : 0.f;
                        }
                    }
                    if (Yb != nullptr) {
                        if (co < ysplit) *reinterpret_cast<float4*>(Y + orow * ysplit + co) = o4;
                        else *reinterpret_cast<float4*>(Yb + orow * (Co - ysplit) + (co - ysplit)) = o4;
                    } else if (VEC4 || (Co % 4) == 0) {
                        *reinterpret_cast<float4*>(Y + orow * Co + co) = o4;
                    } else if constexpr (!VEC4) {
                        const float ov[4] = {o4.x, o4.y, o4.z, o4.w};
#pragma unroll
                        for (int e = 0; e < 4; ++e)
                            if (co + e < Co) Y[orow * Co + co + e] = ov[e];
                    }
                }
            }
            __builtin_amdgcn_wave_barrier();
        } else {
#pragma unroll
        for (int t = 0; t < TCO; ++t) {
            const int co = co_base + 16 * t + 4 * g;
            if constexpr (EPI == EPI_ADD) {
                if (rv) {
#pragma unroll
                    for (int e = 0; e < 4; ++e)
                        if (co + e < Co) acc[t][e] += addend[r * Co + co + e];
                }
            }
            if constexpr (EPI == EPI_DROPOUT) {
                if (rv) {
                    const unsigned long long ctr = (unsigned long long)drop_counter[0];
#pragma unroll
                    for (int e = 0; e < 4; ++e)
                        if (co + e < Co)
                            acc[t][e] = dropout_keep(drop_seed, ctr, (unsigned long long)(r * Co + co + e), drop_threshold)
                                            ? acc[t][e] * drop_scale : 0.f;
                }
            }
            if (rv) {
                if (Yb != nullptr) {
                    const float4 o4 = make_float4(acc[t][0], acc[t][1], acc[t][2], acc[t][3]);
                    if (co < ysplit) *reinterpret_cast<float4*>(Y + r * ysplit + co) = o4;
                    else if (co < Co) *reinterpret_cast<float4*>(Yb + r * (Co - ysplit) + (co - ysplit)) = o4;
                } else if (VEC4) {
                    if (co < Co) *reinterpret_cast<float4*>(Y + r * Co + co) = make_float4(acc[t][0], acc[t][1], acc[t][2], acc[t][3]);
                } else if (co + 3 < Co && (Co % 4) == 0) {
                    *reinterpret_cast<float4*>(Y + r * Co + co) = make_float4(acc[t][0], acc[t][1], acc[t][2], acc[t][3]);
                } else if constexpr (!VEC4) {
#pragma unroll
                    for (int e = 0; e < 4; ++e)
                        if (co + e < Co) Y[r * Co + co + e] = acc[t][e];
                }
            }
        }
        }
        if (stat_partial != nullptr) {
            if (!have_shift) {
#pragma unroll
                for (int t = 0; t < TCO; ++t)
#pragma unroll
                    for (int e = 0; e < 4; ++e) sh[t][e] = __shfl(acc[t][e], 16 * g, WAVE);
                have_shift = true;
            }
            if (rv) {
#pragma unroll
                for (int t = 0; t < TCO; ++t)
#pragma unroll
                    for (int e = 0; e < 4; ++e) {
                        const float dlt = acc[t][e] - sh[t][e];
                        s1[t][e] += dlt;
                        s2[t][e] = fmaf(dlt, dlt, s2[t][e]);
                    }
            }
        }
    }
    if (stat_partial != nullptr) {
        __syncthreads();
        float* sw = sW + wave * 4 * 16 * TCO;
        int64_t nrows = 0;
        for (int64_t row0 = ((int64_t)blockIdx.x * (LF_BLOCK / WAVE) + wave) * 16; row0 < M;
             row0 += (int64_t)gridDim.x * (LF_BLOCK / WAVE) * 16)
            nrows += (M - row0) < 16 ? (M - row0) : 16;
#pragma unroll
        for (int t = 0; t < TCO; ++t)
#pragma unroll
            for (int e = 0; e < 4; ++e) {
                float a = s1[t][e], b = s2[t][e];
#pragma unroll
                for (int o = 8; o > 0; o >>= 1) {
                    a += __shfl_xor(a, o, WAVE);
                    b += __shfl_xor(b, o, WAVE);
                }
                if (rr == 0) {
                    const int cl = 16 * t + 4 * g + e;
                    sw[cl] = sh[t][e];
                    sw[16 * TCO + cl] = (float)nrows;
                    sw[2 * 16 * TCO + cl] = a;
                    sw[3 * 16 * TCO + cl] = b;
                }
            }
        __syncthreads();
        for (int cl = threadIdx.x; cl < 16 * TCO; cl += LF_BLOCK) {
            const int co = co_base + cl;
            if (co >= Co) continue;
            const float s0 = sW[cl];
            double n = 0.0, S1 = 0.0, S2 = 0.0;
            for (int w = 0; w < LF_BLOCK / WAVE; ++w) {
                const float* q = sW + w * 4 * 16 * TCO;
                const double nb = q[16 * TCO + cl];
                if (nb <= 0.0) continue;
                const double d = (double)q[cl] - (double)s0, a = q[2 * 16 * TCO + cl], b = q[3 * 16 * TCO + cl];
                n += nb;
                S1 += a + nb * d;
                S2 += b + 2.0 * d * a + nb * d * d;
            }
            *reinterpret_cast<float4*>(stat_partial + ((int64_t)blockIdx.x * Co + co) * 4) =
                make_float4(s0, (float)n, (float)S1, (float)S2);
        }
    }
}

constexpr int FR_BLOCK = 1024, FR_CH = 16, FR_RL = FR_BLOCK / FR_CH;
template <int FR_UN = 8>
__device__ __forceinline__ bool bn_finalize_records_body(const float* __restrict__ rec, int nrec, int64_t M, int C,
                                                         const float* __restrict__ gamma, const float* __restrict__ beta, float eps,
                                                         float* __restrict__ run_mean, float* __restrict__ run_var, float momentum,
                                                         float* __restrict__ coef, int slab, bool write, float (&ab)[2]) {
    __shared__ double s_red[FR_BLOCK / WAVE][2][FR_CH];
    const int cl = threadIdx.x & (FR_CH - 1), rl = threadIdx.x >> 4;
    const int c = slab * FR_CH + cl;
    const bool cv = c < C;
    const int cc = cv ? c : C - 1;
    const double s0 = rec[(int64_t)cc * 4];
    double S1 = 0.0, S2 = 0.0;
    for (int r0 = rl; r0 < nrec; r0 += FR_UN * FR_RL) {
        float4 v[FR_UN];
#pragma unroll
        for (int u = 0; u < FR_UN; ++u) {
            const int r = r0 + u * FR_RL;
            v[u] = r < nrec ? *reinterpret_cast<const float4*>(rec + ((int64_t)r * C + cc) * 4)
                            : make_float4(0.f, 0.f, 0.f, 0.f);
        }
#pragma unroll
        for (int u = 0; u < FR_UN; ++u) {
            const double nb = v[u].y;
            if (nb > 0.0) {
                const double d = (double)v[u].x - s0, a = v[u].z, b = v[u].w;
                S1 += a + nb * d;
                S2 += b + 2.0 * d * a + nb * d * d;
            }
        }
    }
    S1 += __shfl_xor(S1, 16, WAVE); S2 += __shfl_xor(S2, 16, WAVE);
    S1 += __shfl_xor(S1, 32, WAVE); S2 += __shfl_xor(S2, 32, WAVE);
    const int wave = threadIdx.x >> 6;
    if ((threadIdx.x & 63) < FR_CH) { s_red[wave][0][cl] = S1; s_red[wave][1][cl] = S2; }
    __syncthreads();
    if (threadIdx.x >= FR_CH || !cv) return false;
    S1 = 0.0; S2 = 0.0;
    for (int w = 0; w < FR_BLOCK / WAVE; ++w) { S1 += s_red[w][0][cl]; S2 += s_red[w][1][cl]; }
    const double m1 = S1 / (double)M;
    const double mean = s0 + m1;
    const double m2 = S2 - S1 * m1;
    double var = m2 / (double)M;
    if (var < 0.0) var = 0.0;
    const double rstd = 1.0 / sqrt(var + (double)eps);
    const double a = (double)gamma[c] * rstd;
    ab[0] = (float)a;
    ab[1] = (float)((double)beta[c] - a * mean);
    if (!write) return true;
    coef[c] = ab[0];
    coef[C + c] = ab[1];
    coef[2 * C + c] = (float)mean;
    coef[3 * C + c] = (float)rstd;
    if (run_mean != nullptr) {
        const double unb = M > 1 ? var * ((double)M / (double)(M - 1)) : var;
        run_mean[c] = (float)((1.0 - (double)momentum) * (double)run_mean[c] + (double)momentum * mean);
        run_var[c] = (float)((1.0 - (double)momentum) * (double)run_var[c] + (double)momentum * unb);
    }
    return true;
}
__global__ __launch_bounds__(FR_BLOCK) void bn_finalize_records_kernel(const float* __restrict__ rec, int nrec, int64_t M,
                                                                       int C, const float* __restrict__ gamma,
                                                                       const float* __restrict__ beta, float eps,
                                                                       float* __restrict__ run_mean, float* __restrict__ run_var,
                                                                       float momentum, float* __restrict__ coef) {
    float ab[2];
    bn_finalize_records_body(rec, nrec, M, C, gamma, beta, eps, run_mean, run_var, momentum, coef, blockIdx.x, true, ab);
}

template <bool ADD, int UN = 8>
__device__ __forceinline__ void bn_apply_records_body(const float* __restrict__ rec, int nrec, int64_t M, int C,
                                                      const float* __restrict__ gamma, const float* __restrict__ beta,
                                                      float eps, float* __restrict__ run_mean, float* __restrict__ run_var,
                                                      float momentum, float* __restrict__ coef, const float* __restrict__ x,
                                                      const float* __restrict__ skip, float slope, int rows_per_tile,
                                                      float* __restrict__ y, const int slab, const int tile) {
    __shared__ float s_ab[2][FR_CH];
    float ab[2];
    const int q = threadIdx.x & 3, rl = threadIdx.x >> 2;
    const int c = slab * FR_CH + 4 * q;
    const bool cok = c < C;
    const int64_t r0 = (int64_t)tile * rows_per_tile;
    const int64_t r1 = r0 + rows_per_tile < M ? r0 + rows_per_tile : M;
    float4 v[4];
    [[maybe_unused]] float4 k[ADD ? 4 : 1];
    auto request = [&](int64_t rb) {
#pragma unroll
        for (int u = 0; u < 4; ++u) {
            const int64_t r = rb + (int64_t)u * (FR_BLOCK / 4);
            const bool in = cok && r < r1;
            v[u] = in ? *reinterpret_cast<const float4*>(x + r * C + c) : make_float4(0.f, 0.f, 0.f, 0.f);
            if constexpr (ADD) k[u] = in ? *reinterpret_cast<const float4*>(skip + r * C + c) : make_float4(0.f, 0.f, 0.f, 0.f);
        }
    };
#ifndef BN_APPLY_PREFETCH_
#define BN_APPLY_PREFETCH_ 1
#endif
    if (BN_APPLY_PREFETCH_) request(r0 + rl);
    if (bn_finalize_records_body<UN>(rec, nrec, M, C, gamma, beta, eps, run_mean, run_var, momentum, coef, slab, tile == 0, ab)) {
        s_ab[0][threadIdx.x] = ab[0];
        s_ab[1][threadIdx.x] = ab[1];
    }
    __syncthreads();
    if (!cok) return;
    const float4 a = *reinterpret_cast<const float4*>(&s_ab[0][4 * q]), b = *reinterpret_cast<const float4*>(&s_ab[1][4 * q]);
    for (int64_t rb = r0 + rl; rb < r1; rb += 4 * (FR_BLOCK / 4)) {
        if (!BN_APPLY_PREFETCH_ || rb != r0 + rl) request(rb);
#pragma unroll
        for (int u = 0; u < 4; ++u) {
            const int64_t r = rb + (int64_t)u * (FR_BLOCK / 4);
            if (r >= r1) continue;
            float4 o = make_float4(fmaf(a.x, v[u].x, b.x), fmaf(a.y, v[u].y, b.y), fmaf(a.z, v[u].z, b.z), fmaf(a.w, v[u].w, b.w));
            if constexpr (ADD) {
                o.x = add_rn(o.x, k[u].x); o.y = add_rn(o.y, k[u].y); o.z = add_rn(o.z, k[u].z); o.w = add_rn(o.w, k[u].w);
            }
            o.x = o.x > 0.f ? o.x : slope * o.x;
            o.y = o.y > 0.f ? o.y : slope * o.y;
            o.z = o.z > 0.f ? o.z : slope * o.z;
            o.w = o.w > 0.f ? o.w : slope * o.w;
            *reinterpret_cast<float4*>(y + r * C + c) = o;
        }
    }
}

template <bool ADD>
__global__ __launch_bounds__(FR_BLOCK) void bn_apply_records_kernel(const float* __restrict__ rec, int nrec, int64_t M, int C,
                                                                    const float* __restrict__ gamma, const float* __restrict__ beta,
                                                                    float eps, float* __restrict__ run_mean, float* __restrict__ run_var,
                                                                    float momentum, float* __restrict__ coef, const float* __restrict__ x,
                                                                    const float* __restrict__ skip, float slope, int rows_per_tile,
                                                                    float* __restrict__ y) {
    bn_apply_records_body<ADD>(rec, nrec, M, C, gamma, beta, eps, run_mean, run_var, momentum, coef, x, skip, slope, rows_per_tile, y,
                               blockIdx.y, blockIdx.x);
}
constexpr int BA_MAX = 4;
struct BnApplyJobs {
    const float* rec[BA_MAX]; const float* gamma[BA_MAX]; const float* beta[BA_MAX]; float* run_mean[BA_MAX]; float* run_var[BA_MAX];
    float* coef[BA_MAX]; const float* x[BA_MAX]; const float* skip[BA_MAX]; float* y[BA_MAX];
    long long M[BA_MAX];
    int nrec[BA_MAX], C[BA_MAX], rows_per_tile[BA_MAX], tiles[BA_MAX];
    float eps[BA_MAX], momentum[BA_MAX], slope[BA_MAX];
    int blk_base[BA_MAX + 1];
    int njobs;
};
__global__ __launch_bounds__(FR_BLOCK) void bn_apply_records_jobs_kernel(const BnApplyJobs t) {
    int j = 0;
    while (j + 1 < t.njobs && t.blk_base[j + 1] <= (int)blockIdx.x) ++j;
    const int local = (int)blockIdx.x - t.blk_base[j];
    const int tiles = uni(t.tiles[j]);
    const int tile = uni(local % tiles), slab = uni(local / tiles);
    const float* rec = uni(t.rec[j]); const float* gamma = uni(t.gamma[j]); const float* beta = uni(t.beta[j]);
    float* run_mean = uni(t.run_mean[j]); float* run_var = uni(t.run_var[j]); float* coef = uni(t.coef[j]);
    const float* x = uni(t.x[j]); const float* skip = uni(t.skip[j]); float* y = uni(t.y[j]);
    const long long M = uni(t.M[j]);
    const int nrec = uni(t.nrec[j]), C = uni(t.C[j]), rows = uni(t.rows_per_tile[j]);
    const float eps = uni(t.eps[j]), momentum = uni(t.momentum[j]), slope = uni(t.slope[j]);
    if (skip != nullptr) bn_apply_records_body<true, 4>(rec, nrec, M, C, gamma, beta, eps, run_mean, run_var, momentum, coef, x, skip, slope, rows, y, slab, tile);
    else bn_apply_records_body<false, 4>(rec, nrec, M, C, gamma, beta, eps, run_mean, run_var, momentum, coef, x, nullptr, slope, rows, y, slab, tile);
}

static int lf_blocks(int64_t M) {
    constexpr int cap = 512;
    int64_t nb = (M + 16 * LF_WAVES - 1) / (16 * LF_WAVES);
    if (nb > cap) nb = cap;
    return (int)(nb < 1 ? 1 : nb);
}

}

static size_t lf_lds_bytes_at(int Ci, int tco, bool pro) {
    const size_t cip = (size_t)((Ci + 15) / 16) * 16 + 4, cik = cip - 4;
    size_t floats = 16 * (size_t)tco * cip;
    const size_t stats = (size_t)crf::LF_WAVES * 4 * 16 * (size_t)tco;
    if (floats < stats) floats = stats;
    if (pro) floats += 5 * cik;
    if (tco >= 2) floats += (size_t)crf::LF_WAVES * 16 * (16 * (size_t)tco + 4);
    return sizeof(float) * floats;
}
static int lf_tco(int Ci, int Co, bool pro) {
    constexpr int max_tco = 4;
    const int tiles = (Co + 15) / 16;
    int tco = tiles >= 8 ? 8 : (tiles >= 4 ? 4 : (tiles >= 2 ? 2 : 1));
    if (tco > max_tco) tco = max_tco;
    while (tco > 1 && lf_lds_bytes_at(Ci, tco, pro) > 64 * 1024) tco >>= 1;
    return tco;
}
static size_t lf_lds_bytes(int Ci, int Co, bool pro) { return lf_lds_bytes_at(Ci, lf_tco(Ci, Co, pro), pro); }
static int lf_hoist_chunks(int Ci, bool vec4) {
    if (!vec4 || Ci > 128) return 0;
    const int n = (Ci + 15) / 16;
    return n <= 1 ? 1 : (n <= 2 ? 2 : (n <= 4 ? 4 : 8));
}

extern "C" int crfconv_linear_forward_supported(int Ci, int Co) {
    if (Ci < 1 || Co < 1) return 0;
    return lf_lds_bytes(Ci, Co, false) <= 64 * 1024 ? 1 : 0;
}

extern "C" size_t crfconv_linear_forward_stat_records(int64_t M) { return (size_t)crf::lf_blocks(M); }

struct LinearDropout {
    const long long* counter = nullptr;
    unsigned long long seed = 0ull;
    unsigned threshold = 0u;
    float scale = 1.f;
};

static int linear_forward_impl(const float* X, const float* Xb, int xsplit, const float* W, const float* bias, int64_t M,
                               int Ci, int Co, int transpose_w, float* Y, float* stat_rec, crf_stream_t stream,
                               LinearDropout drop = LinearDropout()) {
    CRF_REQUIRE(X && W && Y, CRF_ERR_ARG, "null pointer");
    CRF_REQUIRE(M > 0, CRF_ERR_ARG, "M must be positive");
    CRF_REQUIRE(crfconv_linear_forward_supported(Ci, Co), CRF_ERR_UNSUPPORTED, "weight slab %dx%d does not fit LDS", Co, Ci);
    CRF_REQUIRE(Xb == nullptr || (xsplit > 0 && xsplit < Ci && xsplit % 4 == 0 && Ci % 4 == 0), CRF_ERR_ARG,
                "two-operand form needs 0 < split < Ci, both multiples of 4 (split=%d Ci=%d)", xsplit, Ci);
    const int tiles = (Co + 15) / 16;
    const int tco = lf_tco(Ci, Co, false);
    const int gy = (tiles + tco - 1) / tco;
    const dim3 grid((unsigned)crf::lf_blocks(M), (unsigned)gy), blk(crf::LF_BLOCK);
    const size_t lds = lf_lds_bytes(Ci, Co, false);
    hipStream_t st = crf::as_stream(stream);
    const bool vec4 = (Ci % 4) == 0 && (Co % 4) == 0;
    const int nch = lf_hoist_chunks(Ci, vec4);
#define LF4(T, V, E, N) hipLaunchKernelGGL((crf::linear_fwd_kernel<T, false, V, E, N>), grid, blk, lds, st, X, W, bias, M, Ci, Co, transpose_w, Y, stat_rec, (const float*)nullptr, (const float*)nullptr, 1.f, Xb, xsplit, (float*)nullptr, 0, (const float*)nullptr, drop.counter, drop.seed, drop.threshold, drop.scale)
#define LF3(T, V, E) do { if (V && nch == 1) LF4(T, V, E, 1); else if (V && nch == 2) LF4(T, V, E, 2); else if (V && nch == 4) LF4(T, V, E, 4); else if (V && nch == 8) LF4(T, V, E, 8); else LF4(T, V, E, 0); } while (0)
#define LF2(T, V) do { if (drop.counter != nullptr) LF4(T, V, crf::EPI_DROPOUT, 0); else LF3(T, V, crf::EPI_NONE); } while (0)
#define LF(T) do { if (vec4) LF2(T, true); else if (drop.counter != nullptr) LF4(T, false, crf::EPI_DROPOUT, 0); else LF4(T, false, crf::EPI_NONE, 0); } while (0)
    switch (tco) {
        case 1: LF(1); break;
        case 2: LF(2); break;
        case 4: LF(4); break;
        default: LF(8); break;
    }
#undef LF
#undef LF2
#undef LF3
#undef LF4
    CRF_LAUNCH_CHECK();
    return CRF_OK;
}

extern "C" int crfconv_linear_forward(const float* X, const float* W, const float* bias, int64_t M, int Ci, int Co,
                                      int transpose_w, float* Y, float* stat_rec, crf_stream_t stream) {
    return linear_forward_impl(X, nullptr, 0, W, bias, M, Ci, Co, transpose_w, Y, stat_rec, stream);
}

extern "C" int crfconv_linear_forward_dropout(const float* X, const float* W, int64_t M, int Ci, int Co, int transpose_w,
                                              float p, uint64_t seed, const int64_t* counter, float* Y, crf_stream_t stream) {
    CRF_REQUIRE(counter, CRF_ERR_ARG, "null pointer");
    CRF_REQUIRE(p >= 0.f && p < 1.f, CRF_ERR_ARG, "dropout probability %g outside [0, 1)", (double)p);
    LinearDropout d;
    d.counter = reinterpret_cast<const long long*>(counter);
    d.seed = (unsigned long long)seed;
    d.threshold = crf::dropout_threshold(p);
    d.scale = 1.f / (1.f - p);
    return linear_forward_impl(X, nullptr, 0, W, nullptr, M, Ci, Co, transpose_w, Y, nullptr, stream, d);
}

extern "C" int crfconv_linear_forward_cat(const float* Xa, const float* Xb, int split, const float* W, const float* bias,
                                          int64_t M, int Ci, int Co, float* Y, float* stat_rec, crf_stream_t stream) {
    CRF_REQUIRE(Xb, CRF_ERR_ARG, "null pointer");
    return linear_forward_impl(Xa, Xb, split, W, bias, M, Ci, Co, 0, Y, stat_rec, stream);
}

extern "C" int crfconv_bn_coef_from_records(const float* stat_rec, int64_t M, int C, const float* gamma,
                                            const float* beta, float* run_mean, float* run_var, float momentum,
                                            float eps, float* coef, crf_stream_t stream) {
    CRF_REQUIRE(stat_rec && gamma && beta && coef, CRF_ERR_ARG, "null pointer");
    CRF_REQUIRE(M > 0 && C > 0, CRF_ERR_ARG, "bad shape");
    return crfconv_bn_coef_from_nrecords(stat_rec, (int64_t)crfconv_linear_forward_stat_records(M), M, C, gamma, beta, run_mean, run_var,
                                         momentum, eps, coef, stream);
}

extern "C" int crfconv_bn_coef_from_nrecords(const float* stat_rec, int64_t nrec, int64_t M, int C, const float* gamma,
                                             const float* beta, float* run_mean, float* run_var, float momentum,
                                             float eps, float* coef, crf_stream_t stream) {
    CRF_REQUIRE(stat_rec && gamma && beta && coef, CRF_ERR_ARG, "null pointer");
    CRF_REQUIRE(M > 0 && C > 0 && nrec > 0 && nrec < ((int64_t)1 << 31), CRF_ERR_ARG, "bad shape");
    hipLaunchKernelGGL(crf::bn_finalize_records_kernel, dim3((C + crf::FR_CH - 1) / crf::FR_CH), dim3(crf::FR_BLOCK), 0, crf::as_stream(stream), stat_rec,
                       (int)nrec, M, C, gamma, beta, eps, run_mean, run_var, momentum, coef);
    CRF_LAUNCH_CHECK();
    return CRF_OK;
}

#ifndef BN_APPLY_WGS_
#define BN_APPLY_WGS_ 256
#endif
static void bn_apply_plan(int64_t M, int C, int wgs, int64_t& tiles, int64_t& rows) {
    const int slabs = (C + crf::FR_CH - 1) / crf::FR_CH;
    tiles = wgs / slabs;
    if (tiles < 1) tiles = 1;
    rows = (M + tiles - 1) / tiles;
    rows = (rows + 1023) / 1024 * 1024;
    tiles = (M + rows - 1) / rows;
    if (tiles > 8) tiles = (tiles + 7) / 8 * 8;
}

extern "C" int crfconv_bn_apply_from_records(const float* stat_rec, int64_t nrec, const float* x, int64_t M, int C, const float* gamma,
                                             const float* beta, float* run_mean, float* run_var, float momentum, float eps,
                                             const float* skip, float slope, float* coef, float* y, crf_stream_t stream) {
    CRF_REQUIRE(stat_rec && x && gamma && beta && coef && y, CRF_ERR_ARG, "null pointer");
    CRF_REQUIRE(M > 0 && C >= 4 && C % 4 == 0 && nrec > 0 && nrec < ((int64_t)1 << 31), CRF_ERR_ARG, "bad shape");
    const int slabs = (C + crf::FR_CH - 1) / crf::FR_CH;
    int64_t tiles, rows;
    bn_apply_plan(M, C, BN_APPLY_WGS_, tiles, rows);
    const dim3 grid((unsigned)tiles, (unsigned)slabs), blk(crf::FR_BLOCK);
    if (skip != nullptr)
        hipLaunchKernelGGL(crf::bn_apply_records_kernel<true>, grid, blk, 0, crf::as_stream(stream), stat_rec, (int)nrec, M, C, gamma, beta, eps,
                           run_mean, run_var, momentum, coef, x, skip, slope, (int)rows, y);
    else
        hipLaunchKernelGGL(crf::bn_apply_records_kernel<false>, grid, blk, 0, crf::as_stream(stream), stat_rec, (int)nrec, M, C, gamma, beta, eps,
                           run_mean, run_var, momentum, coef, x, skip, slope, (int)rows, y);
    CRF_LAUNCH_CHECK();
    return CRF_OK;
}

extern "C" int crfconv_bn_apply_from_records_jobs(const crf_bn_apply_job* jobs, int njobs, crf_stream_t stream) {
    CRF_REQUIRE(jobs && njobs >= 1 && njobs <= crf::BA_MAX, CRF_ERR_ARG, "1 .. %d jobs (got %d)", crf::BA_MAX, njobs);
    crf::BnApplyJobs t;
    int64_t blocks = 0;
    for (int j = 0; j <= crf::BA_MAX; ++j) {
        t.blk_base[j] = (int)blocks;
        if (j >= crf::BA_MAX) break;
        if (j >= njobs) {
            t.rec[j] = nullptr; t.gamma[j] = nullptr; t.beta[j] = nullptr; t.run_mean[j] = nullptr; t.run_var[j] = nullptr; t.coef[j] = nullptr;
            t.x[j] = nullptr; t.skip[j] = nullptr; t.y[j] = nullptr; t.M[j] = 0; t.nrec[j] = 0; t.C[j] = 4; t.rows_per_tile[j] = 1024; t.tiles[j] = 1;
            t.eps[j] = 0.f; t.momentum[j] = 0.f; t.slope[j] = 1.f;
            continue;
        }
        const crf_bn_apply_job& b = jobs[j];
        CRF_REQUIRE(b.stat_rec && b.x && b.gamma && b.beta && b.coef && b.y, CRF_ERR_ARG, "job %d: null pointer", j);
        CRF_REQUIRE(b.M > 0 && b.C >= 4 && b.C % 4 == 0 && b.nrec > 0 && b.nrec < ((int64_t)1 << 31), CRF_ERR_ARG, "job %d: bad shape", j);
        int64_t tiles, rows;
        bn_apply_plan(b.M, b.C, BN_APPLY_WGS_ / njobs, tiles, rows);
        t.rec[j] = b.stat_rec; t.gamma[j] = b.gamma; t.beta[j] = b.beta; t.run_mean[j] = b.run_mean; t.run_var[j] = b.run_var; t.coef[j] = b.coef;
        t.x[j] = b.x; t.skip[j] = b.skip; t.y[j] = b.y; t.M[j] = (long long)b.M; t.nrec[j] = (int)b.nrec; t.C[j] = b.C; t.rows_per_tile[j] = (int)rows;
        t.tiles[j] = (int)tiles; t.eps[j] = b.eps; t.momentum[j] = b.momentum; t.slope[j] = b.slope;
        blocks += tiles * ((b.C + crf::FR_CH - 1) / crf::FR_CH);
        CRF_REQUIRE(blocks < ((int64_t)1 << 31), CRF_ERR_UNSUPPORTED, "too many workgroups in one batch");
    }
    t.njobs = njobs;
    hipLaunchKernelGGL(crf::bn_apply_records_jobs_kernel, dim3((unsigned)blocks), dim3(crf::FR_BLOCK), 0, crf::as_stream(stream), t);
    CRF_LAUNCH_CHECK();
    return CRF_OK;
}

namespace crf {
struct MlpPlan {
    int tco, tci, gy, gz, nblk, rows_per_block;
};
static MlpPlan mlp_plan(int64_t M, int Co, int Ci) {
    MlpPlan p;
    const int t_co = (Co + 15) / 16, t_ci = (Ci + 15) / 16;
    p.tco = t_co >= 4 ? 4 : (t_co >= 2 ? 2 : 1);
    p.tci = t_ci >= 4 ? 4 : (t_ci >= 2 ? 2 : 1);
    if (p.tco * p.tci == 16) p.tci = 2;
    p.gy = (t_co + p.tco - 1) / p.tco;
    p.gz = (t_ci + p.tci - 1) / p.tci;
#ifndef MLP_P1_TARGET_
#define MLP_P1_TARGET_ 512
#endif
    constexpr int target = MLP_P1_TARGET_;
    int64_t slices = target / ((int64_t)p.gy * p.gz);
    if (slices < 32) slices = 32;
    int64_t rows = (M + slices - 1) / slices;
    if (rows < 64) rows = 64;
    rows = (rows + 63) / 64 * 64;
    p.rows_per_block = (int)rows;
    p.nblk = (int)((M + rows - 1) / rows);
    return p;
}
static size_t mlp_ws_layout(int64_t M, int Co, int Ci, size_t off[5]) {
    const MlpPlan p = mlp_plan(M, Co, Ci);
    auto up = [](size_t v) { return (v + 255) & ~(size_t)255; };
    size_t o = 0;
    off[0] = o; o = up(o + sizeof(float) * (size_t)p.nblk * Co * Ci);
    off[1] = o; o = up(o + sizeof(float) * (size_t)p.nblk * Co * Ci);
    off[2] = o; o = up(o + sizeof(float) * (size_t)p.nblk * 2 * Co);
    off[3] = o; o = up(o + sizeof(float) * (size_t)p.nblk * Ci);
    off[4] = o; o = up(o + sizeof(float) * 5 * (size_t)Co);
    return o;
}
}

extern "C" size_t crfconv_ticket_bytes(void) { return sizeof(unsigned) * crf::LW_TICKET_WORDS; }

extern "C" int crfconv_mlp_backward_supported(int64_t M, int Ci, int Co) {
    if (!(M > 0 && Co % 4 == 0 && Ci >= 1 && Co >= 4 && Co <= 1024 && Ci <= 1024)) return 0;
    return lf_lds_bytes(Co, Ci, true) <= 64 * 1024 ? 1 : 0;
}

extern "C" size_t crfconv_mlp_backward_workspace(int64_t M, int Ci, int Co) {
    if (M <= 0 || Co <= 0 || Ci <= 0) return 0;
    size_t off[5];
    return crf::mlp_ws_layout(M, Co, Ci, off) + 256;
}

static int mlp_backward_impl(const float* gA, const float* Y, const float* X, const float* Xb, int xsplit, const float* W,
                             const float* coef, float slope, int64_t M, int Ci, int Co, float* dX, float* dXb, float* dW,
                             float* dgamma, float* dbeta, void* workspace, size_t workspace_bytes, unsigned* ticket,
                             crf_stream_t stream, const float* dX_add = nullptr);

extern "C" int crfconv_mlp_backward(const float* gA, const float* Y, const float* X, const float* W, const float* coef,
                                    float slope, int64_t M, int Ci, int Co, float* dX, float* dW, float* dgamma,
                                    float* dbeta, void* workspace, size_t workspace_bytes, unsigned* ticket,
                                    crf_stream_t stream) {
    return mlp_backward_impl(gA, Y, X, nullptr, 0, W, coef, slope, M, Ci, Co, dX, nullptr, dW, dgamma, dbeta, workspace,
                             workspace_bytes, ticket, stream);
}

extern "C" int crfconv_mlp_backward_add(const float* gA, const float* Y, const float* X, const float* W, const float* coef,
                                        float slope, int64_t M, int Ci, int Co, const float* dX_add, float* dX, float* dW,
                                        float* dgamma, float* dbeta, void* workspace, size_t workspace_bytes,
                                        unsigned* ticket, crf_stream_t stream) {
    CRF_REQUIRE(dX != nullptr || dX_add == nullptr, CRF_ERR_ARG, "dX_add without dX");
    return mlp_backward_impl(gA, Y, X, nullptr, 0, W, coef, slope, M, Ci, Co, dX, nullptr, dW, dgamma, dbeta, workspace,
                             workspace_bytes, ticket, stream, dX_add);
}

extern "C" int crfconv_mlp_backward_cat(const float* gA, const float* Y, const float* Xa, const float* Xb, int split,
                                        const float* W, const float* coef, float slope, int64_t M, int Ci, int Co,
                                        float* dXa, float* dXb, float* dW, float* dgamma, float* dbeta, void* workspace,
                                        size_t workspace_bytes, unsigned* ticket, crf_stream_t stream) {
    CRF_REQUIRE(Xb && split > 0 && split < Ci && split % 4 == 0 && Ci % 4 == 0 && ((dXa == nullptr) == (dXb == nullptr)),
                CRF_ERR_ARG, "two-operand form: split=%d Ci=%d must be multiples of 4, dXa / dXb both or neither", split, Ci);
    return mlp_backward_impl(gA, Y, Xa, Xb, split, W, coef, slope, M, Ci, Co, dXa, dXb, dW, dgamma, dbeta, workspace,
                             workspace_bytes, ticket, stream);
}

static int mlp_dw_jobs_impl(const crf_mlp_dw_job* jobs, int njobs, const crf::CrfMatJobs* side, int nside, crf_stream_t stream) {
    CRF_REQUIRE(jobs || njobs == 0, CRF_ERR_ARG, "null pointer");
    CRF_REQUIRE(njobs >= 0, CRF_ERR_ARG, "njobs=%d < 0", njobs);
    hipStream_t st = crf::as_stream(stream);
    for (int j0 = 0; j0 < njobs; j0 += crf::MDW_MAX) {
        crf::MlpDwTable t;
        const int n = njobs - j0 < crf::MDW_MAX ? njobs - j0 : crf::MDW_MAX;
        int64_t total = 0;
        for (int j = 0; j < crf::MDW_MAX; ++j) {
            const crf_mlp_dw_job& jb = jobs[j0 + (j < n ? j : 0)];
            if (j < n) {
                CRF_REQUIRE(jb.workspace && jb.coef && jb.dW, CRF_ERR_ARG, "job %d: null pointer", j0 + j);
                CRF_REQUIRE(crfconv_mlp_backward_supported(jb.M, jb.Ci, jb.Co) == 1, CRF_ERR_UNSUPPORTED,
                            "job %d: shape M=%lld Ci=%d Co=%d not supported", j0 + j, (long long)jb.M, jb.Ci, jb.Co);
            }
            const char* base = reinterpret_cast<const char*>((reinterpret_cast<uintptr_t>(jb.workspace) + 255) & ~(uintptr_t)255);
            size_t off[5];
            crf::mlp_ws_layout(jb.M, jb.Co, jb.Ci, off);
            t.PA[j] = reinterpret_cast<const float*>(base + off[0]);
            t.PB[j] = reinterpret_cast<const float*>(base + off[1]);
            t.PG[j] = reinterpret_cast<const float*>(base + off[2]);
            t.PX[j] = reinterpret_cast<const float*>(base + off[3]);
            t.coef[j] = jb.coef;
            t.dW[j] = jb.dW;
            t.M[j] = (long long)jb.M;
            t.nblk[j] = crf::mlp_plan(jb.M, jb.Co, jb.Ci).nblk;
            t.Co[j] = jb.Co;
            t.Ci[j] = jb.Ci;
            t.group_begin[j] = (int)total;
            if (j < n) total += crf::cdiv((int64_t)jb.Co * jb.Ci, 64);
            CRF_REQUIRE(total < ((int64_t)1 << 30), CRF_ERR_ARG, "too many slots in one batch");
        }
        t.group_begin[crf::MDW_MAX] = (int)total;
        t.njobs = n;
        if (side != nullptr && j0 == 0)
            hipLaunchKernelGGL(crf::mlp_dw_jobs_hosting_kernel, dim3((unsigned)(total + nside)), dim3(crf::MF_BLOCK), 0, st, t, *side, nside);
        else
            hipLaunchKernelGGL(crf::mlp_dw_jobs_kernel, dim3((unsigned)total), dim3(crf::MF_BLOCK), 0, st, t);
        CRF_LAUNCH_CHECK();
    }
    return CRF_OK;
}
extern "C" int crfconv_mlp_dw_jobs(const crf_mlp_dw_job* jobs, int njobs, crf_stream_t stream) {
    return mlp_dw_jobs_impl(jobs, njobs, nullptr, 0, stream);
}
extern "C" int crfconv_mlp_dw_jobs_hosting(const crf_mlp_dw_job* jobs, int njobs, const float* const* c, const float* const* Q,
                                           const float* const* gQ, const float* const* gP, const int* H, int n, float* const* dc,
                                           crf_stream_t stream) {
    CRF_REQUIRE(njobs >= 1, CRF_ERR_ARG, "a hosting launch needs at least one job of its own (got %d)", njobs);
    crf::CrfMatJobs j;
    int nslab = 0;
    if (int rc = crf_matrices_bwd_jobs(c, Q, gQ, gP, H, n, dc, j, nslab)) return rc;
    return mlp_dw_jobs_impl(jobs, njobs, &j, nslab, stream);
}

static int mlp_backward_impl(const float* gA, const float* Y, const float* X, const float* Xb, int xsplit, const float* W,
                             const float* coef, float slope, int64_t M, int Ci, int Co, float* dX, float* dXb, float* dW,
                             float* dgamma, float* dbeta, void* workspace, size_t workspace_bytes, unsigned* ticket,
                             crf_stream_t stream, const float* dX_add) {
    CRF_REQUIRE(gA && Y && X && W && coef && dgamma && dbeta && workspace, CRF_ERR_ARG, "null pointer");
    CRF_REQUIRE(dX_add == nullptr || dXb == nullptr, CRF_ERR_ARG, "dX_add is for the one-operand form");
    CRF_REQUIRE(crfconv_mlp_backward_supported(M, Ci, Co) == 1, CRF_ERR_UNSUPPORTED, "shape M=%lld Ci=%d Co=%d not supported",
                (long long)M, Ci, Co);
    CRF_REQUIRE(workspace_bytes >= crfconv_mlp_backward_workspace(M, Ci, Co), CRF_ERR_WORKSPACE, "workspace too small");
    hipStream_t st = crf::as_stream(stream);
    char* base = reinterpret_cast<char*>((reinterpret_cast<uintptr_t>(workspace) + 255) & ~(uintptr_t)255);
    size_t off[5];
    crf::mlp_ws_layout(M, Co, Ci, off);
    float* PA = reinterpret_cast<float*>(base + off[0]);
    float* PB = reinterpret_cast<float*>(base + off[1]);
    float* PG = reinterpret_cast<float*>(base + off[2]);
    float* PX = reinterpret_cast<float*>(base + off[3]);
    float* pro = reinterpret_cast<float*>(base + off[4]);
    const crf::MlpPlan p = crf::mlp_plan(M, Co, Ci);
    if (!(2 * Co <= crf::WG_BLOCK && crf::WG_BLOCK % (Co / 2) == 0 && (int64_t)p.nblk * 2 * Co * 4 < ((int64_t)1 << 31))) ticket = nullptr;
    {
        const dim3 grid((unsigned)p.nblk, (unsigned)p.gy, (unsigned)p.gz), blk(crf::WG_BLOCK);
#define P1(TA, TB) hipLaunchKernelGGL((crf::mlp_bwd_p1_kernel<TA, TB>), grid, blk, 0, st, gA, Y, X, Xb, xsplit, coef, slope, M, Co, Ci, p.rows_per_block, PA, PB, PG, PX, ticket, dgamma, dbeta, pro)
        switch (p.tco * 10 + p.tci) {
            case 11: P1(1, 1); break;
            case 12: P1(1, 2); break;
            case 14: P1(1, 4); break;
            case 21: P1(2, 1); break;
            case 22: P1(2, 2); break;
            case 24: P1(2, 4); break;
            case 41: P1(4, 1); break;
            default: P1(4, 2); break;
        }
#undef P1
        CRF_LAUNCH_CHECK();
    }
    const int nw = dW != nullptr ? (int)crf::cdiv((int64_t)Co * Ci, 64) : 0;
    const int nc = ticket != nullptr ? 0 : (Co + crf::MF_WAVES - 1) / crf::MF_WAVES;
    if (nw + nc > 0) {
        hipLaunchKernelGGL(crf::mlp_bwd_finalize_kernel, dim3((unsigned)(nw + nc)), dim3(crf::MF_BLOCK), 0, st, PA, PB, PG, PX, p.nblk, coef, M, Co,
                           Ci, nw, dW, dgamma, dbeta, pro);
        CRF_LAUNCH_CHECK();
    }
    if (dX != nullptr) {
        const int gCi = Co, gCo = Ci;
        const int tiles = (gCo + 15) / 16;
        const int tco = lf_tco(gCi, gCo, true);
        const int gy = (tiles + tco - 1) / tco;
        const dim3 grid((unsigned)crf::lf_blocks(M), (unsigned)gy), blk(crf::LF_BLOCK);
        const size_t lds = lf_lds_bytes(gCi, gCo, true);
        const bool vec4 = (gCi % 4) == 0 && (gCo % 4) == 0;
        const int nch = lf_hoist_chunks(gCi, vec4);
#define DX4(T, V, E, N) hipLaunchKernelGGL((crf::linear_fwd_kernel<T, true, V, E, N>), grid, blk, lds, st, gA, W, (const float*)nullptr, M, gCi, gCo, 1, dX, (float*)nullptr, Y, pro, slope, (const float*)nullptr, 0, dXb, xsplit, dX_add)
#define DX3(T, V, E) do { if (V && nch == 1) DX4(T, V, E, 1); else if (V && nch == 2) DX4(T, V, E, 2); else if (V && nch == 4) DX4(T, V, E, 4); else if (V && nch == 8) DX4(T, V, E, 8); else DX4(T, V, E, 0); } while (0)
#define DX2(T, V) do { if (dX_add != nullptr) DX3(T, V, crf::EPI_ADD); else DX3(T, V, crf::EPI_NONE); } while (0)
#define DX(T) do { if (vec4) DX2(T, true); else if (dX_add != nullptr) DX4(T, false, crf::EPI_ADD, 0); else DX4(T, false, crf::EPI_NONE, 0); } while (0)
        switch (tco) {
            case 1: DX(1); break;
            case 2: DX(2); break;
            case 4: DX(4); break;
            default: DX(8); break;
        }
#undef DX
#undef DX2
#undef DX3
#undef DX4
        CRF_LAUNCH_CHECK();
    }
    return CRF_OK;
}
```

### crfconv_amd/ops/_base.py

```python
import ctypes

import torch

from .. import _lib
from ..graph import NeighborTable, ptr, require_gpu, stream_ptr

BN_EPS = 1e-5


def _f32c(t):
    if t.dtype is torch.float32 and t.is_contiguous():
        return t.detach()
    return t.detach().to(torch.float32).contiguous()


def _pad_channels(t, C):
    if t.shape[-1] == C:
        return t
    return torch.nn.functional.pad(t, (0, C - t.shape[-1]))


def _next_supported(c, choices):
    for v in choices:
        if c <= v:
            return v
    raise _lib.CrfConvError('channel count %d exceeds the largest supported (%d)' % (c, choices[-1]))


def _ptr_array(tensors):
    return (ctypes.c_void_p * len(tensors))(*[None if t is None else t.data_ptr() for t in tensors])



_TICKETS = {}
_raw_stream = getattr(torch._C, '_cuda_getCurrentRawStream', None)


def _stream_key(device):
    idx = device.index if isinstance(device, torch.device) else None
    if idx is None:
        dev = torch.device(device)
        idx = dev.index if dev.index is not None else torch.cuda.current_device()
    if torch.cuda.is_current_stream_capturing():
        return idx, 'capture'
    if _raw_stream is not None:
        return idx, int(_raw_stream(idx))
    return idx, int(torch.cuda.current_stream(idx).cuda_stream)


def _stream_buf(table, device, make):
    key = _stream_key(device)
    buf = table.get(key)
    if buf is None:
        buf = table[key] = make()
        if key[1] != 'capture' and (key[0], 'capture') not in table:
            table[(key[0], 'capture')] = make()
    return buf


def _ticket(device):
    return _stream_buf(_TICKETS, device, lambda: torch.zeros(_lib.load().crfconv_ticket_bytes() // 4, dtype=torch.int32, device=device))




def _pc_ticket(device):
    return ptr(_ticket(device))




def _mlp_ticket(device):
    return ptr(_ticket(device))


_sync_ws = {}


def gridsync_ws(dev):
    return _stream_buf(_sync_ws, dev, lambda: torch.zeros(_lib.load().crfconv_gridsync_workspace() // 4, dtype=torch.int32, device=dev))




def fail_word_ptrs(dev):
    want = torch.device(dev).index
    if want is None:
        want = torch.cuda.current_device()
    word = _lib.load().crfconv_gridsync_fail_word()
    keys = [k for k in _sync_ws if k[0] == want]
    first = [k for k in ((want, 'capture'), (want, int(torch.cuda.current_stream(want).cuda_stream))) if k in _sync_ws]
    rest = [k for k in reversed(keys) if k not in first]
    if len(first) + len(rest) > 8:
        import warnings
        warnings.warn('fail_word_ptrs: %d barrier workspaces on device %d, the update guard watches 8 (capture buffer, current stream, '
                      'newest streams); ops.check_gridsync() reads all of them' % (len(first) + len(rest), want))
    return [_sync_ws[k].data_ptr() + 4 * word for k in (first + rest)[:8]]


def check_gridsync(dev=None, reduced_flag=None):
    word = _lib.load().crfconv_gridsync_fail_word()
    bad = []
    want = None if dev is None else torch.device(dev).index
    for table in (_sync_ws,):
        for key, ws in list(table.items()):
            if want is not None and key[0] is not None and key[0] != want:
                continue
            code = int(ws[word].item())
            if code != 0:
                ws.zero_()
                bad.append((key, code))
    remote = False
    if reduced_flag is not None and reduced_flag.numel():
        v = float(reduced_flag.reshape(-1)[0].item())
        remote = not (v == 0.0)
        if remote:
            reduced_flag.zero_()
    if bad or remote:
        state.small_mlp_disabled = True
        where = ('device(s) %s (code 0x%x)' % (sorted({k[0] for k, _ in bad}), bad[0][1])) if bad else 'another rank of the process group'
        raise _lib.CrfConvError('grid barrier timed out on %s: a one-launch kernel could not get all its '
                                'workgroups resident; its outputs were poisoned with NaN.  The one-launch MLP path is now '
                                'disabled for this process (CRFCONV_NO_ONE_LAUNCH_MLP=1 does the same up front).' % where)




class _State:
    no_join = False
    no_fork = False
    no_prefold = False
    small_mlp_disabled = __import__('os').environ.get('CRFCONV_NO_ONE_LAUNCH_MLP') is not None
    small_bwd_one_launch = __import__('os').environ.get('CRFCONV_SMALL_BWD_TWO_LAUNCHES') is None
    dw_hosts_mats = __import__('os').environ.get('CRFCONV_NO_TAIL_RIDERS') is None
    mfma_min_rows = 12288
    mf_block = __import__('os').environ.get('CRFCONV_MF_BLOCK', 'auto')
    mf_block_min_rows = 65536
    mf_block_min_locality = 0.6


state = _State()
```

### crfconv_amd/ops/mlp.py

```python
import ctypes

import torch

from .. import _lib
from ..graph import NeighborTable, ptr, require_gpu, stream_ptr
from ._base import _f32c, _mlp_ticket, _ticket, gridsync_ws, state



class _MLPBlock(torch.autograd.Function):

    @staticmethod
    def forward(ctx, x_in, W, gamma, beta, run_mean, run_var, momentum, eps, slope, fork=False):
        x = x_in.contiguous()
        Wc = W.contiguous()
        m, ci = x.shape
        co = Wc.shape[0]
        y, rec = _mfma_matmul(x, Wc, None, False, True)
        coef = torch.empty(4 * co, dtype=torch.float32, device=x.device)
        g, b = _f32c(gamma), _f32c(beta)
        out = torch.empty_like(y)
        _lib.call('crfconv_bn_apply_from_records', ptr(rec), rec.shape[0], ptr(y), m, co, ptr(g), ptr(b), ptr(run_mean), ptr(run_var),
                  float(momentum), float(eps), None, float(slope), ptr(coef), ptr(out), stream_ptr())
        ctx.prm = (W, gamma, beta)
        ctx.save_for_backward(x, Wc, y, coef)
        ctx.slope = float(slope)
        if fork:
            ctx.set_materialize_grads(False)
            return out, x_in
        return out

    @staticmethod
    def backward(ctx, gA, g_alias=None):
        x, W, y, coef = ctx.saved_tensors
        m, ci = x.shape
        co = W.shape[0]
        dev = x.device
        gA = torch.zeros_like(y) if gA is None else gA.contiguous()
        dX = torch.empty_like(x) if ctx.needs_input_grad[0] else None
        add = _f32c(g_alias) if (g_alias is not None and dX is not None) else None
        outs, dfr = _mlp_param_outs(ctx.prm, W, dev)
        dW, dgamma, dbeta = (o[0] for o in outs)
        nbytes = _lib.load().crfconv_mlp_backward_workspace(m, ci, co)
        ws = torch.empty(nbytes, dtype=torch.uint8, device=dev)
        _lib.call('crfconv_mlp_backward_add', ptr(gA), ptr(y), ptr(x), ptr(W), ptr(coef), ctx.slope, m, ci, co, ptr(add), ptr(dX),
                  ptr(None if dfr else dW), ptr(dgamma), ptr(dbeta), ptr(ws), nbytes, _mlp_ticket(dev), stream_ptr())
        return dX, *_mlp_param_rets(ctx.prm, outs, dfr, ws, m, ci, co, coef), None, None, None, None, None, None




class _MLPBlockJoin(torch.autograd.Function):

    @staticmethod
    def forward(ctx, x, W, gamma, beta, run_mean, run_var, momentum, eps, skip, slope):
        x, Wc, skip = x.contiguous(), W.contiguous(), skip.contiguous()
        m, ci = x.shape
        co = Wc.shape[0]
        y, rec = _mfma_matmul(x, Wc, None, False, True)
        coef = torch.empty(4 * co, dtype=torch.float32, device=x.device)
        st = stream_ptr()
        out = torch.empty_like(y)
        _lib.call('crfconv_bn_apply_from_records', ptr(rec), rec.shape[0], ptr(y), m, co, ptr(_f32c(gamma)), ptr(_f32c(beta)),
                  ptr(run_mean), ptr(run_var), float(momentum), float(eps), ptr(skip), float(slope), ptr(coef), ptr(out), st)
        ctx.prm = (W, gamma, beta)
        ctx.save_for_backward(x, Wc, y, coef, out)
        ctx.slope = float(slope)
        return out

    @staticmethod
    def backward(ctx, g):
        x, W, y, coef, out = ctx.saved_tensors
        m, ci = x.shape
        co = W.shape[0]
        dev = x.device
        g = g.contiguous()
        g1 = torch.empty_like(g)
        st = stream_ptr()
        _lib.call('crfconv_add_lrelu_backward', ptr(g), ptr(out), out.numel(), ctx.slope, ptr(g1), st)
        dX = torch.empty_like(x) if ctx.needs_input_grad[0] else None
        outs, dfr = _mlp_param_outs(ctx.prm, W, dev)
        dW, dgamma, dbeta = (o[0] for o in outs)
        nbytes = _lib.load().crfconv_mlp_backward_workspace(m, ci, co)
        ws = torch.empty(nbytes, dtype=torch.uint8, device=dev)
        _lib.call('crfconv_mlp_backward', ptr(g1), ptr(y), ptr(x), ptr(W), ptr(coef), 1.0, m, ci, co, ptr(dX), ptr(None if dfr else dW),
                  ptr(dgamma), ptr(dbeta), ptr(ws), nbytes, _mlp_ticket(dev), st)
        gskip = g1 if ctx.needs_input_grad[8] else None
        return dX, *_mlp_param_rets(ctx.prm, outs, dfr, ws, m, ci, co, coef), None, None, None, None, gskip, None




class _MLPBlockDropout(torch.autograd.Function):

    @staticmethod
    def forward(ctx, x, W, gamma, beta, run_mean, run_var, momentum, eps, slope, p, seed, counter):
        x, Wc = x.contiguous(), W.contiguous()
        m, ci = x.shape
        co = Wc.shape[0]
        y, rec = _mfma_matmul(x, Wc, None, False, True)
        coef = torch.empty(4 * co, dtype=torch.float32, device=x.device)
        st = stream_ptr()
        _lib.call('crfconv_bn_coef_from_records', ptr(rec), m, co, ptr(_f32c(gamma)), ptr(_f32c(beta)), ptr(run_mean),
                  ptr(run_var), float(momentum), float(eps), ptr(coef), st)
        out = torch.empty_like(y)
        used = torch.empty(1, dtype=torch.int64, device=x.device)
        _lib.call('crfconv_bn_apply_dropout', ptr(y), m, co, ptr(coef), float(slope), float(p), int(seed), ptr(counter), ptr(out),
                  ptr(used), st)
        counter = used
        ctx.prm = (W, gamma, beta)
        ctx.save_for_backward(x, Wc, y, coef, counter)
        ctx.slope, ctx.p, ctx.seed = float(slope), float(p), int(seed)
        return out

    @staticmethod
    def backward(ctx, g):
        x, W, y, coef, counter = ctx.saved_tensors
        m, ci = x.shape
        co = W.shape[0]
        dev = x.device
        g = g.contiguous()
        gA = torch.empty_like(g)
        st = stream_ptr()
        _lib.call('crfconv_dropout_backward', ptr(g), g.numel(), ctx.p, ctx.seed, ptr(counter), ptr(gA), st)
        dX = torch.empty_like(x) if ctx.needs_input_grad[0] else None
        outs, dfr = _mlp_param_outs(ctx.prm, W, dev)
        dW, dgamma, dbeta = (o[0] for o in outs)
        nbytes = _lib.load().crfconv_mlp_backward_workspace(m, ci, co)
        ws = torch.empty(nbytes, dtype=torch.uint8, device=dev)
        _lib.call('crfconv_mlp_backward', ptr(gA), ptr(y), ptr(x), ptr(W), ptr(coef), ctx.slope, m, ci, co, ptr(dX), ptr(None if dfr else dW),
                  ptr(dgamma), ptr(dbeta), ptr(ws), nbytes, _mlp_ticket(dev), st)
        return dX, *_mlp_param_rets(ctx.prm, outs, dfr, ws, m, ci, co, coef), None, None, None, None, None, None, None, None


class _MLPDropoutLinear(torch.autograd.Function):

    @staticmethod
    def forward(ctx, x, W, gamma, beta, run_mean, run_var, momentum, eps, slope, p, seed, counter, W2, b2):
        x, Wc, W2c = x.contiguous(), W.contiguous(), W2.contiguous()
        m, ci = x.shape
        co = Wc.shape[0]
        y, rec = _mfma_matmul(x, Wc, None, False, True)
        coef = torch.empty(4 * co, dtype=torch.float32, device=x.device)
        st = stream_ptr()
        _lib.call('crfconv_bn_coef_from_records', ptr(rec), m, co, ptr(_f32c(gamma)), ptr(_f32c(beta)), ptr(run_mean),
                  ptr(run_var), float(momentum), float(eps), ptr(coef), st)
        h = torch.empty_like(y)
        used = torch.empty(1, dtype=torch.int64, device=x.device)
        _lib.call('crfconv_bn_apply_dropout', ptr(y), m, co, ptr(coef), float(slope), float(p), int(seed), ptr(counter), ptr(h),
                  ptr(used), st)
        counter = used
        logits = _mfma_matmul(h, W2c, None if b2 is None else b2.contiguous(), False)[0]
        ctx.prm = (W, gamma, beta)
        ctx.save_for_backward(x, Wc, y, coef, counter, h, W2c)
        ctx.slope, ctx.p, ctx.seed = float(slope), float(p), int(seed)
        ctx.params2 = (W2, b2)
        return logits

    @staticmethod
    def backward(ctx, g):
        x, W, y, coef, counter, h, W2 = ctx.saved_tensors
        m, ci = x.shape
        co, c2 = W.shape[0], W2.shape[0]
        dev = x.device
        g = g.contiguous()
        st = stream_ptr()
        gA = torch.empty((m, co), dtype=torch.float32, device=dev)
        _lib.call('crfconv_linear_forward_dropout', ptr(g), ptr(W2), m, c2, co, 1, ctx.p, ctx.seed, ptr(counter), ptr(gA), st)
        W2p, b2p = ctx.params2
        dW2 = db2 = None
        if _defer_ok(ctx.params2):
            _defer_weight_grad(g, h, ctx.params2, b2p is not None)
        else:
            dW2 = torch.empty((c2, co), dtype=torch.float32, device=dev)
            db2 = torch.empty(c2, dtype=torch.float32, device=dev) if b2p is not None else None
            nb = _lib.load().crfconv_linear_wgrad_workspace(m, c2, co)
            wsw = torch.empty(nb, dtype=torch.uint8, device=dev)
            _lib.call('crfconv_linear_wgrad', ptr(g), ptr(h), m, c2, co, ptr(dW2), ptr(db2), ptr(wsw), nb, st)
        dX = torch.empty_like(x) if ctx.needs_input_grad[0] else None
        outs, dfr = _mlp_param_outs(ctx.prm, W, dev)
        dW, dgamma, dbeta = (o[0] for o in outs)
        nbytes = _lib.load().crfconv_mlp_backward_workspace(m, ci, co)
        ws = torch.empty(nbytes, dtype=torch.uint8, device=dev)
        _lib.call('crfconv_mlp_backward', ptr(gA), ptr(y), ptr(x), ptr(W), ptr(coef), ctx.slope, m, ci, co, ptr(dX), ptr(None if dfr else dW),
                  ptr(dgamma), ptr(dbeta), ptr(ws), nbytes, _mlp_ticket(dev), st)
        return dX, *_mlp_param_rets(ctx.prm, outs, dfr, ws, m, ci, co, coef), None, None, None, None, None, None, None, None, dW2, db2




class _HeadRecompute(torch.autograd.Function):

    @staticmethod
    def forward(ctx, x, W, gamma, beta, run_mean, run_var, momentum, eps, slope, p, seed, counter, W2, b2):
        x, Wc, W2c = x.contiguous(), W.contiguous(), W2.contiguous()
        m, ci = x.shape
        co, c2 = Wc.shape[0], W2c.shape[0]
        dev = x.device
        lib = _lib.load()
        st = stream_ptr()
        nrec = lib.crfconv_head_stat_records(m)
        rec = torch.empty((nrec, co, 4), dtype=torch.float32, device=dev)
        _lib.call('crfconv_head_stats', ptr(x), ptr(Wc), m, ci, co, ptr(rec), st)
        coef = torch.empty(4 * co, dtype=torch.float32, device=dev)
        _lib.call('crfconv_bn_coef_from_nrecords', ptr(rec), nrec, m, co, ptr(_f32c(gamma)), ptr(_f32c(beta)), ptr(run_mean),
                  ptr(run_var), float(momentum), float(eps), ptr(coef), st)
        logits = torch.empty((m, c2), dtype=torch.float32, device=dev)
        mask = torch.empty(lib.crfconv_head_mask_words(m), dtype=torch.int32, device=dev)
        b2c = None if b2 is None else b2.contiguous()
        _lib.call('crfconv_head_forward', ptr(x), ptr(Wc), ptr(coef), float(slope), float(p), int(seed), ptr(counter), ptr(W2c),
                  ptr(b2c), m, ci, co, c2, ptr(logits), ptr(mask), None, st)
        ctx.prm = (W, gamma, beta, W2, b2)
        ctx.save_for_backward(x, Wc, coef, mask, W2c)
        ctx.slope, ctx.p = float(slope), float(p)
        return logits

    @staticmethod
    def backward(ctx, g):
        x, W, coef, mask, W2 = ctx.saved_tensors
        m, ci = x.shape
        co, c2 = W.shape[0], W2.shape[0]
        dev = x.device
        g = g.contiguous()
        Wp, gp, bp, W2p, b2p = ctx.prm
        outs = [_param_out(Wp, (co, ci), dev), _param_out(gp, (co,), dev), _param_out(bp, (co,), dev), _param_out(W2p, (c2, co), dev)]
        ob2 = _param_out(b2p, (c2,), dev) if b2p is not None else (None, False)
        dX = torch.empty_like(x) if ctx.needs_input_grad[0] else None
        nbytes = _lib.load().crfconv_head_backward_workspace(m, ci, co, c2)
        ws = torch.empty(nbytes, dtype=torch.uint8, device=dev)
        _lib.call('crfconv_head_backward', ptr(g), ptr(x), ptr(W), ptr(coef), ctx.slope, ctx.p, ptr(W2), ptr(mask), m, ci, co, c2,
                  ptr(dX), ptr(outs[0][0]), ptr(outs[1][0]), ptr(outs[2][0]), ptr(outs[3][0]), ptr(ob2[0]), ptr(ws), nbytes, stream_ptr())
        rets = [_param_ret(prm, o[0], o[1]) for prm, o in zip((Wp, gp, bp, W2p), outs)]
        rb2 = _param_ret(b2p, ob2[0], ob2[1]) if b2p is not None else None
        return dX, rets[0], rets[1], rets[2], None, None, None, None, None, None, None, None, rets[3], rb2


def dropout_seed(ci, co):
    return (torch.initial_seed() * 0x9E3779B97F4A7C15 + co * 7919 + ci) & 0xFFFFFFFFFFFFFFFF


def dropout_keep_mask(seed, counter, n, p):
    import numpy as np
    t = float(p) * 4294967296.0
    thr = np.uint32(0xffffffff if t >= 4294967295.0 else (0 if t <= 0.0 else int(t)))
    mask64 = 0xFFFFFFFFFFFFFFFF
    z = (int(seed) + 0x9E3779B97F4A7C15 * (int(counter) + 1)) & mask64
    z = ((z ^ (z >> 30)) * 0xBF58476D1CE4E5B9) & mask64
    z = ((z ^ (z >> 27)) * 0x94D049BB133111EB) & mask64
    z ^= z >> 31
    k0, k1 = np.uint32(z & 0xFFFFFFFF), np.uint32(z >> 32)
    with np.errstate(over='ignore'):
        e = np.arange(int(n), dtype=np.uint64)
        hi = (e >> np.uint64(32)).astype(np.uint32)
        x = e.astype(np.uint32) + k0 + ((hi << np.uint32(13)) | (hi >> np.uint32(19)))
        x ^= x >> np.uint32(16)
        x *= np.uint32(0x7feb352d)
        x ^= x >> np.uint32(15)
        x += k1
        x *= np.uint32(0x846ca68b)
        x ^= x >> np.uint32(16)
    return x >= thr


def mlp_dropout_linear(x, W, bn, slope, p, W2, b2, recompute=None):
    if not (0.0 <= p < 1.0) or bn.num_batches_tracked is None:
        return None
    m = x.numel() // x.shape[-1]
    ci, co, c2 = x.shape[-1], W.shape[0], W2.shape[0]
    if not (mlp_block_ok(x, W, None, bn, True) and not _mlp_small_ok(m, ci, co) and _mfma_ok(m, co, c2) and _mfma_ok(m, c2, co)
            and W2.dtype == torch.float32):
        return None
    require_gpu(x, W, W2)
    tick(bn)
    mom = 0.1 if bn.momentum is None else bn.momentum
    seed = dropout_seed(ci, co)
    node = _MLPDropoutLinear
    head_ok = bool(_lib.load().crfconv_head_supported(m, ci, co, c2))
    if recompute and not head_ok:
        return None
    if head_ok and (recompute or recompute is None):
        node = _HeadRecompute
    out = node.apply(x.reshape(-1, ci), W, bn.weight, bn.bias, bn.running_mean, bn.running_var, mom, bn.eps, slope,
                                  p, seed, bn.num_batches_tracked, W2, b2)
    return out.reshape(x.shape[:-1] + (c2,))


def mlp_block_dropout(x, W, bn, slope, p):
    if not (0.0 <= p < 1.0) or bn.num_batches_tracked is None:
        return None
    m = x.numel() // x.shape[-1]
    ci, co = x.shape[-1], W.shape[0]
    if not mlp_block_ok(x, W, None, bn, True):
        return None
    if _mlp_small_ok(m, ci, co):
        lib = _lib.load()
        if not (co % 4 == 0 and lib.crfconv_linear_forward_supported(ci, co) and lib.crfconv_mlp_backward_supported(m, ci, co) == 1):
            return None
    require_gpu(x, W)
    tick(bn)
    mom = 0.1 if bn.momentum is None else bn.momentum
    seed = dropout_seed(ci, co)
    out = _MLPBlockDropout.apply(x.reshape(-1, ci), W, bn.weight, bn.bias, bn.running_mean, bn.running_var, mom, bn.eps, slope,
                                 p, seed, bn.num_batches_tracked)
    return out.reshape(x.shape[:-1] + (co,))


class _MLPBlockPool(torch.autograd.Function):

    @staticmethod
    def forward(ctx, x_in, W, gamma, beta, run_mean, run_var, momentum, eps, table, fork=False):
        x, Wc = x_in.contiguous(), W.contiguous()
        m, ci = x.shape
        co = Wc.shape[0]
        dev = x.device
        y, rec = _mfma_matmul(x, Wc, None, False, True)
        coef = torch.empty(4 * co, dtype=torch.float32, device=dev)
        st = stream_ptr()
        _lib.call('crfconv_bn_coef_from_records', ptr(rec), m, co, ptr(_f32c(gamma)), ptr(_f32c(beta)), ptr(run_mean),
                  ptr(run_var), float(momentum), float(eps), ptr(coef), st)
        out = torch.empty((table.m_tgt, co), dtype=torch.float32, device=dev)
        arg = torch.empty((table.m_tgt, co), dtype=torch.int32, device=dev)
        _lib.call('crfconv_neighbor_maxpool_affine_forward', ptr(y), ptr(coef), ptr(table.idx32), table.K, table.m_tgt, co,
                  ptr(out), ptr(arg), st)
        ctx.table = table
        ctx.prm = (W, gamma, beta)
        ctx.save_for_backward(x, Wc, y, coef, arg)
        if fork:
            ctx.set_materialize_grads(False)
            return out, x_in
        return out

    @staticmethod
    def backward(ctx, g, g_alias=None):
        x, W, y, coef, arg = ctx.saved_tensors
        table = ctx.table
        m, ci = x.shape
        co = W.shape[0]
        dev = x.device
        g = torch.zeros((table.m_tgt, co), dtype=torch.float32, device=dev) if g is None else _f32c(g)
        st = stream_ptr()
        rev_ptr, rev_eid = table.reverse
        gA = torch.empty((m, co), dtype=torch.float32, device=dev)
        _lib.call('crfconv_neighbor_maxpool_backward', ptr(g), ptr(arg), ptr(rev_ptr), ptr(rev_eid), table.K, m, co, ptr(gA), st)
        dX = torch.empty_like(x) if ctx.needs_input_grad[0] else None
        add = _f32c(g_alias) if (g_alias is not None and dX is not None) else None
        outs, dfr = _mlp_param_outs(ctx.prm, W, dev)
        dW, dgamma, dbeta = (o[0] for o in outs)
        nbytes = _lib.load().crfconv_mlp_backward_workspace(m, ci, co)
        ws = torch.empty(nbytes, dtype=torch.uint8, device=dev)
        _lib.call('crfconv_mlp_backward_add', ptr(gA), ptr(y), ptr(x), ptr(W), ptr(coef), 1.0, m, ci, co, ptr(add), ptr(dX),
                  ptr(None if dfr else dW), ptr(dgamma), ptr(dbeta), ptr(ws), nbytes, _mlp_ticket(dev), st)
        return dX, *_mlp_param_rets(ctx.prm, outs, dfr, ws, m, ci, co, coef), None, None, None, None, None, None


def mlp_block_pool(x, W, bn, table, fork=False):
    if state.no_join or table.padded:
        return None
    m, ci = x.shape
    co = W.shape[0]
    if m != table.m_src or not (mlp_block_ok(x, W, None, bn, True) and not _mlp_small_ok(m, ci, co)):
        return None
    require_gpu(x, W)
    tick(bn)
    mom = 0.1 if bn.momentum is None else bn.momentum
    if fork and x.requires_grad and torch.is_grad_enabled() and not state.no_fork:
        return _MLPBlockPool.apply(x, W, bn.weight, bn.bias, bn.running_mean, bn.running_var, mom, bn.eps, table, True)
    out = _MLPBlockPool.apply(x, W, bn.weight, bn.bias, bn.running_mean, bn.running_var, mom, bn.eps, table, False)
    return (out, x) if fork else out




def _small_bwd_jobs(jobs, n, dev, st):
    if state.small_bwd_one_launch and not state.small_mlp_disabled:
        _lib.call('crfconv_mlp_small_backward_jobs_one_launch', ctypes.cast(jobs, ctypes.c_void_p), n, ptr(_ticket(dev)), ptr(gridsync_ws(dev)), st)
    else:
        _lib.call('crfconv_mlp_small_backward_jobs', ctypes.cast(jobs, ctypes.c_void_p), n, ptr(_ticket(dev)), st)


def _small_bwd(gA, y, coef, W, addend, slope, dgamma, dbeta, need_dx):
    m, co = y.shape
    ci = W.shape[1]
    dev = y.device
    gY = torch.empty_like(y)
    lib = _lib.load()
    if need_dx and lib.crfconv_mlp_small_backward_supported(m, ci, co) == 1:
        dX = torch.empty((m, ci), dtype=torch.float32, device=dev)
        nbytes = lib.crfconv_mlp_small_backward_workspace(m, co)
        ws = torch.empty(nbytes, dtype=torch.uint8, device=dev)
# ... 434 lines not shown
```

### include/crfconv_amd.h

```cpp
#ifndef CRFCONV_AMD_H
#define CRFCONV_AMD_H

#include <stddef.h>
#include <stdint.h>

#ifdef __cplusplus
extern "C" {
#endif

typedef void* crf_stream_t;

enum {
    CRF_OK = 0,
    CRF_ERR_ARG = -1,
    CRF_ERR_HIP = -2,
    CRF_ERR_UNSUPPORTED = -3,
    CRF_ERR_WORKSPACE = -4
};

#define CRFCONV_ABI_VERSION 1
int crfconv_abi_version(void);
const char* crfconv_last_error(void);


int crfconv_knn(const float* points, size_t npts, size_t dim, const float* queries, size_t nqueries,
                size_t K, long* indices);
int crfconv_knn_omp(const float* points, size_t npts, size_t dim, const float* queries,
                    size_t nqueries, size_t K, long* indices);
int crfconv_knn_batch(const float* batch_data, size_t batch_size, size_t npts, size_t dim,
                      const float* queries, size_t nqueries, size_t K, long* batch_indices);
int crfconv_knn_batch_omp(const float* batch_data, size_t batch_size, size_t npts, size_t dim,
                          const float* queries, size_t nqueries, size_t K, long* batch_indices);

size_t crfconv_knn_batch_dev_workspace(size_t batch_size, size_t npts, size_t nqueries, size_t K);
int crfconv_knn_batch_dev(const float* pts, size_t batch_size, size_t npts, size_t dim,
                          const float* queries, size_t nqueries, size_t K, int64_t* out_i64,
                          int32_t* out_i32, void* workspace, size_t workspace_bytes,
                          crf_stream_t stream);

int crfconv_fps(const float* pos, int n_clouds, const int64_t* seg_start, const int64_t* seg_count,
                const int64_t* out_start, const int64_t* n_sample, const int64_t* first, float* dist_ws,
                int64_t* out, crf_stream_t stream);

int64_t crfconv_grid_subsample(const float* points, int64_t N, const float* feats, int fdim,
                               const int32_t* classes, int ldim, float sampleDl, float* out_points,
                               float* out_feats, int32_t* out_classes, int64_t cap);
size_t crfconv_grid_subsample_dev_workspace(int64_t N, int fdim, int ldim);
int64_t crfconv_grid_subsample_dev(const float* points, int64_t N, const float* feats, int fdim,
                                   const int32_t* classes, int ldim, float sampleDl,
                                   float* out_points, float* out_feats, int32_t* out_classes,
                                   int64_t cap, void* workspace, size_t workspace_bytes,
                                   crf_stream_t stream);

int crfconv_index_narrow(const int64_t* idx64, int64_t B, int64_t n_tgt, int K, int64_t n_src,
                         int32_t* idx32, uint16_t* idx16, int32_t* bad_count, crf_stream_t stream);

int crfconv_index_narrow_sorted(const int64_t* idx64, int64_t B, int64_t n_tgt, int K, int64_t n_src,
                                int sort_from, int32_t* idx32, uint16_t* idx16, int32_t* bad_count,
                                crf_stream_t stream);

int crfconv_morton_codes(const float* pts, int64_t B, int64_t npts, float* box_ws, int64_t* codes, crf_stream_t stream);

typedef struct { const void* src; void* dst; int64_t nbytes; } crf_copy_job;
int crfconv_copy_jobs(const crf_copy_job* jobs, int njobs, crf_stream_t stream);

size_t crfconv_reverse_csr_workspace(int64_t E, int64_t m_src);
int crfconv_reverse_csr(const int32_t* idx32, int64_t E, int64_t m_src, int32_t* rev_ptr,
                        int32_t* rev_eid, void* workspace, size_t workspace_bytes,
                        crf_stream_t stream);
typedef struct { const int64_t* idx64; int64_t B; int64_t n_tgt; int K; int64_t n_src; int sort_from; int32_t* idx32;
                 uint16_t* idx16; int32_t* bad_count; } crf_narrow_job;
int crfconv_index_narrow_batched(const crf_narrow_job* jobs, int njobs, crf_stream_t stream);
typedef struct { const int32_t* idx32; int64_t E; int64_t m_src; int32_t* rev_ptr; int32_t* rev_eid; } crf_rev_job;
size_t crfconv_reverse_csr_batched_workspace(const crf_rev_job* jobs, int njobs);
int crfconv_reverse_csr_batched(const crf_rev_job* jobs, int njobs, void* workspace, size_t workspace_bytes,
                                crf_stream_t stream);

int crfconv_meanfield_forward(const float* z, const float* y, const int32_t* idx32, int K, int k0,
                              int64_t m, int H, const float* Q, const float* P, int T, float* s,
                              float* xs, crf_stream_t stream);

int crfconv_meanfield_forward_u16(const float* z, const float* y, const int32_t* idx32, const uint16_t* idx16,
                                  int n_tgt, int n_src, int K, int k0, int64_t m, int H, const float* Q,
                                  const float* P, int T, float* s, float* xs, crf_stream_t stream);

int crfconv_meanfield_forward_block_rows(int64_t m, int H, int K, int k0, int T);
int crfconv_meanfield_forward_block(const float* z, const float* y, const int32_t* idx32, const uint16_t* idx16,
                                    int n_tgt, int n_src, int K, int k0, int64_t m, int H, const float* Q,
                                    const float* P, int T, float* s, float* xs, void* ws, crf_stream_t stream);
int crfconv_meanfield_forward_block_stamps(const float* z, const float* y, const int32_t* idx32, const uint16_t* idx16, int n_tgt, int n_src,
                                           int64_t m, const float* Q, const float* P, int T, float* s, float* xs, void* ws, int shape,
                                           unsigned long long* dbg, crf_stream_t stream);
int crfconv_block_locality(const int32_t* idx32, int64_t m, int K, int k0, int rows, unsigned long long* count, crf_stream_t stream);

int crfconv_meanfield_bwd_edge(const float* G, const float* xprev, const float* s,
                               const int32_t* idx32, int K, int k0, int64_t m, int H,
                               const float* P, float* gm, float* ds, float* mt, int accumulate,
                               crf_stream_t stream);
int crfconv_meanfield_bwd_scatter(const float* gm, const float* s, const int32_t* rev_ptr,
                                  const int32_t* rev_eid, int K, int k0, int64_t m_src, int H,
                                  const float* add, float* Gprev, crf_stream_t stream);
int crfconv_meanfield_backward_supported(int H, int K, int k0);
int crfconv_meanfield_backward_param_grads_inside(int H);
size_t crfconv_meanfield_backward_workspace(int64_t m, int H, int K);
int crfconv_meanfield_backward(const float* gout, const float* z, const float* y, const float* s, const float* xs,
                               const int32_t* idx32, const uint16_t* idx16, int n_tgt, int n_src,
                               const int32_t* rev_ptr, const int32_t* rev_eid, int K, int k0, int64_t m, int H,
                               const float* Q, const float* P, int T, float* Gs, float* dzq, float* mts, float* sumG,
                               float* dz, float* w, float* dy_self, float* dy, float* dP, float* dQ, void* ws,
                               size_t ws_bytes, unsigned* ticket, crf_stream_t stream);


int crfconv_wide_similarity(const float* y, const int32_t* idx32, int K, int k0, int64_t m, int H, float* s,
                            crf_stream_t stream);
int crfconv_wide_aggregate(const float* x, const float* s, const int32_t* idx32, int K, int k0, int64_t m, int H,
                           float* out, crf_stream_t stream);
int crfconv_wide_bwd_edge(const float* gm, const float* xprev, const int32_t* idx32, int K, int k0, int64_t m, int H,
                          float* ds, int accumulate, crf_stream_t stream);
int crfconv_wide_scatter(const float* src, const float* coef, const int32_t* rev_ptr, const int32_t* rev_eid, int K,
                         int64_t m_src, int H, const float* add, int similarity, float* out, crf_stream_t stream);
int crfconv_wide_similarity_bwd(const float* ds, const float* s, const float* y, const int32_t* idx32, int K, int k0,
                                int64_t m, int H, float* w, float* dy_self, crf_stream_t stream);

int crfconv_similarity_bwd(const float* ds, const float* s, const float* y, const int32_t* idx32,
                           int K, int k0, int64_t m, int H, float* w, float* dy_self,
                           crf_stream_t stream);
int crfconv_similarity_bwd_scatter(const float* w, const float* y, const float* dy_self,
                                   const int32_t* rev_ptr, const int32_t* rev_eid, int K, int k0,
                                   int64_t m_src, int H, float* dy, crf_stream_t stream);


size_t crfconv_pointconv_workspace(int64_t m_tgt, int K, int d);
int crfconv_pointconv_moments(const float* pos_src, const float* pos_tgt, const int32_t* idx32,
                              int K, int64_t m_tgt, double* out9, void* workspace,
                              size_t workspace_bytes, crf_stream_t stream);
int crfconv_pointconv_moments_packed(const float* pos_src, const float* pos_tgt, const int32_t* idx32, int K, int64_t m_tgt,
                                     double n_edges, double* mean, double* cov, double* packed, float* mean32,
                                     void* workspace, size_t workspace_bytes, crf_stream_t stream);
typedef struct { const float* pos_src; const float* pos_tgt; const int32_t* idx32; int K; int64_t m_tgt; double n_edges;
                 double* mean; double* cov; double* packed; float* mean32; } crf_moments_job;
size_t crfconv_pointconv_moments_batched_workspace(const crf_moments_job* jobs, int njobs);
int crfconv_pointconv_moments_batched(const crf_moments_job* jobs, int njobs, void* workspace, size_t workspace_bytes,
                                      crf_stream_t stream);
int crfconv_pointconv_stats(const float* pos_src, const float* pos_tgt, const int32_t* idx32, int K,
                            int64_t m_tgt, int d, const float* A1, const float* b1,
                            const float* W2, float slope, const float* mean_rel3, float* shift, double* stats,
                            void* workspace, size_t workspace_bytes, crf_stream_t stream);
int crfconv_pointconv_forward_uv(const float* x, const float* pos_src, const float* pos_tgt,
                                 const int32_t* idx32, int K, int64_t m_tgt, int d, const float* A1,
                                 const float* b1, const float* W2, float slope, const float* mean_rel3,
                                 float* shift, double* stats, float* U, float* V, void* workspace,
                                 size_t workspace_bytes, unsigned* ticket, crf_stream_t stream);
int crfconv_pointconv_forward_uv_hosts(int K, int d);
int crfconv_pointconv_forward_uv_hosting(const float* x, const float* pos_src, const float* pos_tgt, const int32_t* idx32, int K,
                                         int64_t m_tgt, int d, const float* A1, const float* b1, const float* W2, float slope,
                                         const float* mean_rel3, float* shift, double* stats, float* U, float* V, void* workspace,
                                         size_t workspace_bytes, unsigned* ticket, const float* const* c, const int* H, int n,
                                         float* const* Q, float* const* P, crf_stream_t stream);
int crfconv_pointconv_combine(const float* U, const float* V, const double* stats, const float* shift,
                              const float* gamma2, const float* beta2, double n_edges, float* run_mean,
                              float* run_var, float momentum, float eps, int64_t m_tgt, int d, float* a2, float* b2,
                              double* aux2, float* out, crf_stream_t stream);
int crfconv_pointconv_bwd_reduce_uv(const float* gout, const float* U, const float* V, int64_t m_tgt, int d,
                                    const float* shift, const double* aux2, const float* gamma2, double n_edges,
                                    int use_batch, float* ca, float* cb, float* cc, float* dgamma2, float* dbeta2,
                                    void* workspace, size_t workspace_bytes, unsigned* ticket, crf_stream_t stream);
int crfconv_pointconv_forward(const float* x, const float* pos_src, const float* pos_tgt,
                              const int32_t* idx32, int K, int64_t m_tgt, int d, const float* A1,
                              const float* b1, const float* W2, float slope, const float* a2, const float* b2,
                              float* out, crf_stream_t stream);
int crfconv_pointconv_bwd_reduce(const float* x, const float* gout, const float* pos_src,
                                 const float* pos_tgt, const int32_t* idx32, int K, int64_t m_tgt,
                                 int d, const float* A1, const float* b1, const float* W2, float slope,
                                 const float* shift, double* red1, void* workspace, size_t workspace_bytes,
                                 crf_stream_t stream);
int crfconv_pointconv_bwd_params(const float* x, const float* gout, const float* pos_src,
                                 const float* pos_tgt, const int32_t* idx32, int K, int64_t m_tgt,
                                 int d, const float* A1, const float* b1, const float* W2, float slope,
                                 const float* ca, const float* cb, const float* cc, double* dW2,
                                 double* dA1b1, void* workspace, size_t workspace_bytes,
                                 crf_stream_t stream);
int crfconv_pointconv_bwd_dump(const float* x, const float* gout, const float* pos_src,
                               const float* pos_tgt, const int32_t* idx32, int K, int64_t m_tgt, int d,
                               const float* A1, const float* b1, const float* W2, float slope, const float* ca,
                               const float* cb, const float* cc, float* h1, float* gh2, float* rel,
                               crf_stream_t stream);
size_t crfconv_pointconv_bwd_a1_workspace(int64_t n_edges, int d);
int crfconv_pointconv_bwd_a1(const float* gw, const float* h1, const float* rel, int64_t n_edges, int d,
                             float slope, double* dA1b1, void* workspace, size_t workspace_bytes,
                             crf_stream_t stream);
typedef struct { const float* x; const float* gout; const float* pos_src; const float* pos_tgt; const int32_t* idx32; int K; int64_t m_tgt;
                 int d; const float* A1; const float* b1; const float* W2; float slope; const float* ca; const float* cb; const float* cc;
                 float* h1; float* gh2; float* rel; } crf_pc_dump_job;
typedef struct { const float* gw; const float* h1; const float* rel; int64_t n_edges; int d; float slope; void* workspace;
                 size_t workspace_bytes; } crf_pc_a1_job;
int crfconv_pointconv_bwd_dump_jobs(const crf_pc_dump_job* jobs, int njobs, crf_stream_t stream);
typedef struct { const float* x; const float* gout; const float* pos_src; const float* pos_tgt; const int32_t* idx32; int K; int64_t m_tgt;
                 int d; const float* A1; const float* b1; const float* W2; float slope; const float* ca; const float* cb; const float* cc;
                 float* dw2_partial; double* a1_partial; } crf_pc_wide_job;
int crfconv_pointconv_wide_params_supported(int64_t m_tgt, int K, int d);
int64_t crfconv_pointconv_wide_params_nblk(int64_t m_tgt, int d);
int crfconv_pointconv_wide_params_jobs(const crf_pc_wide_job* jobs, int njobs, crf_stream_t stream);
int crfconv_pointconv_bwd_a1_jobs(const crf_pc_a1_job* jobs, int njobs, crf_stream_t stream);
typedef struct { const void* partial; int is_float; int64_t nblk; int nslots; double* out; } crf_reduce64_job;
int crfconv_pointconv_bwd_params_slabs(void* workspace, int64_t m_tgt, int d, const float** slab_w2, const double** slab_a1,
                                       int64_t* nblk_out);
int64_t crfconv_pointconv_bwd_a1_nblk(int64_t n_edges, int d);
int crfconv_reduce_jobs_f64(const crf_reduce64_job* jobs, int njobs, crf_stream_t stream);
int crfconv_pointconv_bwd_input(const float* gout, const float* pos_src, const float* pos_tgt,
                                const int32_t* rev_ptr, const int32_t* rev_eid, int K,
                                int64_t m_src, int d, const float* A1, const float* b1,
                                const float* W2, float slope, const float* a2, const float* b2, float* dx,
                                crf_stream_t stream);
int crfconv_pointconv_bwd_input_reduce(const float* gout, const float* pos_src, const float* pos_tgt, const int32_t* rev_ptr,
                                       const int32_t* rev_eid, int K, int64_t m_src, int64_t m_tgt, int d, const float* A1, const float* b1,
                                       const float* W2, float slope, const float* a2, const float* b2, float* dx, const float* U,
                                       const float* V, const float* shift, const double* aux2, const float* gamma2, double n_edges,
                                       int use_batch, float* ca, float* cb, float* cc, float* dgamma2, float* dbeta2, void* workspace,
                                       size_t workspace_bytes, unsigned* ticket, crf_stream_t stream);

int crfconv_pointconv_fold1(const float* W1, const float* gamma1, const float* beta1, const double* mom,
                            double n_edges, float* run_mean, float* run_var, float momentum, float eps,
                            int use_batch, int d, float* A1, float* b1, double* aux1, crf_stream_t stream);
int crfconv_pointconv_fold1_bwd(const float* W1, const float* gamma1, const double* mom, const double* aux1,
                                const double* dA1b1, float eps, int use_batch, int d, float* dW1,
                                float* dgamma1, float* dbeta1, const double* dW2_f64, float* dW2_f32, crf_stream_t stream);
typedef struct {
    const float* W1; const float* gamma1; const float* beta1; const double* mom; double n_edges;
    float* run_mean; float* run_var; float momentum; float eps; int32_t use_batch; int32_t d;
    float* A1; float* b1; double* aux1;
} crf_fold1_job;
int crfconv_pointconv_fold1_batched(const crf_fold1_job* jobs, int njobs, crf_stream_t stream);
typedef struct {
    const float* W1; const float* gamma1; const double* mom; const double* aux1; const double* dA1b1;
    float eps; int32_t use_batch; int32_t d; int32_t pad_;
    float* dW1; float* dgamma1; float* dbeta1; const double* dW2_f64; float* dW2_f32;
} crf_fold1_bwd_job;
int crfconv_pointconv_fold1_bwd_batched(const crf_fold1_bwd_job* jobs, int njobs, crf_stream_t stream);
int crfconv_pointconv_fold2(const double* stats, const float* shift, const float* gamma2, const float* beta2,
                            double n_edges, float* run_mean, float* run_var, float momentum, float eps,
                            int use_batch, int d, float* a2, float* b2, double* aux2, crf_stream_t stream);
int crfconv_pointconv_fold2_bwd(const double* red, const float* shift, const double* aux2, const float* gamma2,
                                double n_edges, int use_batch, int d, float* ca, float* cb, float* cc,
                                float* dgamma2, float* dbeta2, crf_stream_t stream);

size_t crfconv_linear_wgrad_workspace(int64_t M, int Co, int Ci);
int crfconv_linear_wgrad(const float* G, const float* X, int64_t M, int Co, int Ci, float* dW, float* db,
                         void* workspace, size_t workspace_bytes, crf_stream_t stream);
typedef struct { const float* partial; float* out; int32_t nblk; int32_t nslots; } crf_reduce_job;
int crfconv_linear_wgrad_partial(const float* G, const float* X, int64_t M, int Co, int Ci, int want_bias,
                                 void* workspace, size_t workspace_bytes, int* nblk_out, crf_stream_t stream);
typedef struct { const float* G; const float* X; int64_t M; int Co; int Ci; int want_bias; void* workspace; size_t workspace_bytes; } crf_wgrad_job;
int crfconv_linear_wgrad_nblk(int64_t M, int Co, int Ci);
int crfconv_linear_wgrad_partial_jobs(const crf_wgrad_job* jobs, int njobs, crf_stream_t stream);
int crfconv_reduce_jobs(const crf_reduce_job* jobs, int njobs, crf_stream_t stream);
int crfconv_reduce_jobs_both(const crf_reduce_job* jobs, int njobs, const crf_reduce64_job* jobs64, int njobs64, crf_stream_t stream);

size_t crfconv_gridsync_workspace(void);
int crfconv_gridsync_fail_word(void);
int crfconv_mlp_small_supported(int64_t M, int Ci, int Co);
size_t crfconv_mlp_small_workspace(int64_t M, int Co);
int crfconv_mlp_small_forward(const float* X, const float* W, int64_t M, int Ci, int Co, const float* gamma,
                              const float* beta, float* run_mean, float* run_var, float momentum, float eps, float slope,
                              float* Y, float* A, float* coef, void* workspace, size_t workspace_bytes, void* sync_ws,
                              size_t sync_bytes, crf_stream_t stream);

int crfconv_mlp_small_forward_join(const float* X, const float* W, int64_t M, int Ci, int Co, const float* gamma,
                                   const float* beta, float* run_mean, float* run_var, float momentum, float eps, float slope,
                                   const float* skip, float join_slope, float* Y, float* A, float* coef, void* workspace,
                                   size_t workspace_bytes, void* sync_ws, size_t sync_bytes, crf_stream_t stream);

size_t crfconv_ticket_bytes(void);
int crfconv_mlp_backward_supported(int64_t M, int Ci, int Co);
size_t crfconv_mlp_backward_workspace(int64_t M, int Ci, int Co);
int crfconv_mlp_backward(const float* gA, const float* Y, const float* X, const float* W, const float* coef, float slope,
                         int64_t M, int Ci, int Co, float* dX, float* dW, float* dgamma, float* dbeta, void* workspace,
                         size_t workspace_bytes, unsigned* ticket, crf_stream_t stream);
typedef struct { const void* workspace; const float* coef; float* dW; int64_t M; int32_t Ci; int32_t Co; } crf_mlp_dw_job;
int crfconv_mlp_dw_jobs(const crf_mlp_dw_job* jobs, int njobs, crf_stream_t stream);
int crfconv_mlp_dw_jobs_hosting(const crf_mlp_dw_job* jobs, int njobs, const float* const* c, const float* const* Q,
                                const float* const* gQ, const float* const* gP, const int* H, int n, float* const* dc,
                                crf_stream_t stream);
int crfconv_mlp_backward_add(const float* gA, const float* Y, const float* X, const float* W, const float* coef, float slope,
                             int64_t M, int Ci, int Co, const float* dX_add, float* dX, float* dW, float* dgamma, float* dbeta,
                             void* workspace, size_t workspace_bytes, unsigned* ticket, crf_stream_t stream);
int crfconv_linear_forward_cat(const float* Xa, const float* Xb, int split, const float* W, const float* bias, int64_t M,
                               int Ci, int Co, float* Y, float* stat_rec, crf_stream_t stream);
int crfconv_mlp_backward_cat(const float* gA, const float* Y, const float* Xa, const float* Xb, int split, const float* W,
                             const float* coef, float slope, int64_t M, int Ci, int Co, float* dXa, float* dXb, float* dW,
                             float* dgamma, float* dbeta, void* workspace, size_t workspace_bytes, unsigned* ticket,
                             crf_stream_t stream);

size_t crfconv_bn_workspace(int64_t M, int C);
int crfconv_bn_forward(const float* x, int64_t M, int C, const float* gamma, const float* beta, float* run_mean,
                       float* run_var, float momentum, float eps, int use_batch_stats, float slope, float* coef,
                       float* y, void* workspace, size_t workspace_bytes, crf_stream_t stream);
int crfconv_bn_backward(const float* gy, const float* x, const float* coef, int64_t M, int C, int training,
                        float slope, float* gx, float* dgamma, float* dbeta, void* workspace,
                        size_t workspace_bytes, crf_stream_t stream);

int crfconv_bn_apply(const float* x, int64_t M, int C, const float* coef, float slope, float* y, crf_stream_t stream);

int crfconv_linear_forward_supported(int Ci, int Co);
size_t crfconv_linear_forward_stat_records(int64_t M);
int crfconv_linear_forward(const float* X, const float* W, const float* bias, int64_t M, int Ci, int Co,
                           int transpose_w, float* Y, float* stat_rec, crf_stream_t stream);
int crfconv_cat2(const float* xa, const float* xb, int64_t m, int ca, int cb, float* out, crf_stream_t stream);
int crfconv_split2(const float* g, int64_t m, int ca, int cb, float* ga, float* gb, crf_stream_t stream);
int crfconv_add_i64(int64_t* x, int64_t n, int64_t delta, crf_stream_t stream);
int crfconv_gate_mark(uint64_t* gate, crf_stream_t stream);
int crfconv_gate_wait(uint64_t* gate, int max_wait_us, crf_stream_t stream);

int crfconv_mlp_small_backward_supported(int64_t M, int Ci, int Co);
size_t crfconv_mlp_small_backward_workspace(int64_t M, int Co);
int crfconv_mlp_small_backward(const float* gA, const float* Y, const float* coef, const float* W, const float* addend, int64_t M,
                               int Ci, int Co, int training, float slope, float* gY, float* dX, float* dgamma, float* dbeta,
                               void* workspace, size_t workspace_bytes, unsigned* ticket, crf_stream_t stream);
size_t crfconv_gemm_stat_records(int64_t M);
int crfconv_gemm_stats(const float* A, const float* B, int64_t M, int N, int K, float* C, float* stat_rec, crf_stream_t stream);
typedef struct { const float* A; const float* B; int64_t M; int N; int K; float* C; float* stat_rec; } crf_gemm_stats_job;
int crfconv_gemm_stats_jobs(const crf_gemm_stats_job* jobs, int njobs, crf_stream_t stream);
typedef struct { const float* stat_rec; int64_t nrec; const float* x; int64_t M; int C; const float* gamma; const float* beta;
                 float* run_mean; float* run_var; float momentum; float eps; const float* skip; float slope; float* coef; float* y;
} crf_bn_apply_job;
int crfconv_bn_apply_from_records_jobs(const crf_bn_apply_job* jobs, int njobs, crf_stream_t stream);
typedef struct { const float* gA; const float* Y; const float* coef; const float* W; const float* addend; int64_t M; int Ci; int Co;
                 int training; float slope; float* gY; float* dX; float* dgamma; float* dbeta; void* workspace; size_t workspace_bytes;
} crf_mlp_bwd_job;
int crfconv_mlp_small_backward_jobs(const crf_mlp_bwd_job* jobs, int njobs, unsigned* ticket, crf_stream_t stream);
int crfconv_mlp_small_backward_jobs_one_launch(const crf_mlp_bwd_job* jobs, int njobs, unsigned* ticket, unsigned* sync_ws,
                                               crf_stream_t stream);
typedef struct { const float* A; const float* B; float* C; int64_t M; int N; int K; } crf_gemm_job;
int crfconv_gemm_jobs(const crf_gemm_job* jobs, int njobs, crf_stream_t stream);
int crfconv_gemm_supported(int64_t M, int N, int K);
int crfconv_gemm(const float* A, const float* B, const float* bias, const float* addend, int64_t M, int N, int K,
                 int b_is_nk, float* C, crf_stream_t stream);
int crfconv_bn_coef_from_records(const float* stat_rec, int64_t M, int C, const float* gamma, const float* beta,
                                 float* run_mean, float* run_var, float momentum, float eps, float* coef,
                                 crf_stream_t stream);
int crfconv_bn_apply_from_records(const float* stat_rec, int64_t nrec, const float* x, int64_t M, int C, const float* gamma,
                                  const float* beta, float* run_mean, float* run_var, float momentum, float eps, const float* skip,
                                  float slope, float* coef, float* y, crf_stream_t stream);
int crfconv_bn_coef_from_nrecords(const float* stat_rec, int64_t nrec, int64_t M, int C, const float* gamma, const float* beta,
                                  float* run_mean, float* run_var, float momentum, float eps, float* coef, crf_stream_t stream);

int crfconv_spd_inverse(const float* M, int H, float* Q, crf_stream_t stream);
int crfconv_spd_inverse_wide(const float* M, int H, float* Q, crf_stream_t stream);
int crfconv_crf_matrices(const float* c, int H, float* Q, float* P, crf_stream_t stream);
int crfconv_crf_matrices_backward(const float* c, const float* Q, const float* dQ, const float* dP, int H,
                                  float* dc, crf_stream_t stream);
int crfconv_crf_matrices_batched(const float* const* c, const int* H, int n, float* const* Q, float* const* P,
                                 crf_stream_t stream);
int crfconv_crf_matrices_backward_batched(const float* const* c, const float* const* Q, const float* const* gQ,
                                          const float* const* gP, const int* H, int n, float* const* dc,
                                          crf_stream_t stream);

int crfconv_neighbor_maxpool_forward(const float* x, const int32_t* idx32, int K, int64_t m_tgt,
                                     int C, float* out, int32_t* arg, crf_stream_t stream);
int crfconv_neighbor_maxpool_affine_forward(const float* x, const float* coef, const int32_t* idx32, int K, int64_t m_tgt,
                                            int C, float* out, int32_t* arg, crf_stream_t stream);
int crfconv_neighbor_maxpool_backward(const float* gout, const int32_t* arg,
                                      const int32_t* rev_ptr, const int32_t* rev_eid, int K,
                                      int64_t m_src, int C, float* dx, crf_stream_t stream);
int crfconv_gather_rows(const float* x, const int32_t* idx32, int64_t m_tgt, int C, float* out,
                        crf_stream_t stream);
int crfconv_gather_rows_backward(const float* gout, const int32_t* rev_ptr,
                                 const int32_t* rev_eid, int64_t m_src, int C, float* dx,
                                 crf_stream_t stream);

int crfconv_add_lrelu(const float* a, const float* b, int64_t n, float slope, float* out, crf_stream_t stream);
int crfconv_bn_apply_dropout(const float* x, int64_t M, int C, const float* coef, float slope, float p, uint64_t seed,
                             const int64_t* counter, float* out, int64_t* counter_used, crf_stream_t stream);
int crfconv_dropout_backward(const float* g, int64_t n, float p, uint64_t seed, const int64_t* counter, float* gin,
                             crf_stream_t stream);
int crfconv_linear_forward_dropout(const float* X, const float* W, int64_t M, int Ci, int Co, int transpose_w, float p,
                                   uint64_t seed, const int64_t* counter, float* Y, crf_stream_t stream);
int crfconv_head_supported(int64_t M, int Ci, int Co, int C2);
size_t crfconv_head_mask_words(int64_t M);
size_t crfconv_head_stat_records(int64_t M);
int crfconv_head_stats(const float* X, const float* W1, int64_t M, int Ci, int Co, float* stat_rec, crf_stream_t stream);
size_t crfconv_head_backward_workspace(int64_t M, int Ci, int Co, int C2);
int crfconv_head_forward(const float* X, const float* W1, const float* coef, float slope, float p, uint64_t seed,
                         const int64_t* counter, const float* W2, const float* b2, int64_t M, int Ci, int Co, int C2,
                         float* logits, uint32_t* mask_bits, int64_t* counter_used, crf_stream_t stream);
int crfconv_head_backward(const float* g, const float* X, const float* W1, const float* coef, float slope, float p,
                          const float* W2, const uint32_t* mask_bits, int64_t M, int Ci, int Co, int C2, float* dX, float* dW1,
                          float* dgamma, float* dbeta, float* dW2, float* db2, void* workspace, size_t workspace_bytes,
                          crf_stream_t stream);
int crfconv_bn_apply_add(const float* x, int64_t M, int C, const float* coef, const float* skip, float slope, float* out,
                         crf_stream_t stream);
int crfconv_add_lrelu_backward(const float* gout, const float* out, int64_t n, float slope, float* gin,
                               crf_stream_t stream);

size_t crfconv_softmax_ce_workspace(int64_t m);
int crfconv_softmax_ce_forward(const float* logits, const int64_t* target, const float* weight, int64_t m, int C,
                               int64_t ignore_index, int64_t label_shift, float* lse, double* sums, float* loss,
                               void* workspace, size_t workspace_bytes, unsigned* ticket, crf_stream_t stream);
int crfconv_softmax_ce_backward(const float* logits, const int64_t* target, const float* weight, const float* lse,
                                const double* sums, const float* grad_loss, int64_t m, int C, int64_t ignore_index,
                                int64_t label_shift, float* dlogits, crf_stream_t stream);

int crfconv_sgd_step(float* param, const float* grad, float* momentum_buf, int64_t n, float lr, float momentum,
                     float dampening, float weight_decay, int nesterov, int first_step, crf_stream_t stream);
int crfconv_sgd_step_hyper(float* param, const float* grad, float* momentum_buf, int64_t n, const float* hyper,
                           int nesterov, int first_step, crf_stream_t stream);
int crfconv_sgd_step_guarded(float* param, const float* grad, float* momentum_buf, int64_t n, const float* hyper,
                             int nesterov, int first_step, const unsigned* fail_word, crf_stream_t stream);
int crfconv_sgd_step_guarded_all(float* param, const float* grad, float* momentum_buf, int64_t n, const float* hyper,
                                 int nesterov, int first_step, const unsigned* const* fail_words, int n_fail_words,
                                 const float* reduced_flag, crf_stream_t stream);
int crfconv_sgd_guard_publish(const unsigned* const* fail_words, int n_fail_words, float* slot, crf_stream_t stream);

int crfconv_random_subsets(const int* n, const int* s, int64_t* const* out, int32_t* const* rank, int nlevels, uint64_t seed,
                           const int64_t* counter, crf_stream_t stream);
size_t crfconv_upindex_workspace(int64_t B, int64_t N);
int crfconv_upindex_from_table(const float* pos, const float* sub_pos, const int64_t* neighbor_idx, const int32_t* rank, int64_t B, int64_t N,
                               int K, int64_t S, int64_t* up_idx, void* workspace, size_t workspace_bytes, crf_stream_t stream);
int crfconv_gather_rows_batched(const void* const* src, void* const* dst, const int* row_bytes, int njobs, const int64_t* index,
                                int per_cloud, int64_t B, int64_t N, int64_t S, crf_stream_t stream);
size_t crfconv_argsort_codes_workspace(int64_t B, int64_t N);
int crfconv_argsort_codes(const int64_t* code, int64_t B, int64_t N, int64_t* order, void* workspace,
                          size_t workspace_bytes, crf_stream_t stream);

int crfconv_meanfield_step(const float* xin, const float* z, const float* s, const int32_t* idx32, int K, int k0,
                           int64_t m, int H, const float* Q, const float* P, float* xout, crf_stream_t stream);

int crfconv_kernel_weights_forward(const float* fk, const int32_t* idx32, int K, const float* Wg, int G, int H,
                                   int64_t m, float* w, crf_stream_t stream);
size_t crfconv_kernel_weights_partials(int64_t m);
int crfconv_kernel_weights_backward(const float* gw, const float* fk, const int32_t* idx32, const int32_t* rev_ptr,
                                    const int32_t* rev_eid, int K, const float* Wg, int G, int H, int64_t m,
                                    float* dfk_self, float* dfk, double* dW_partial, crf_stream_t stream);

int crfconv_confusion_accumulate(const int64_t* y_true, const int64_t* y_pred, const float* logits, int64_t n_rows,
                                 int n_class, int64_t ignore_index, int64_t label_shift, int64_t* hist,
                                 int32_t* bad_count, crf_stream_t stream);

int crfconv_vote_accumulate(const float* probs, const float* logits, const int64_t* point_idx, int64_t n_rows, int C,
                            double smooth, float* test_probs, int64_t n_cloud, int32_t* bad_count, crf_stream_t stream);
int crfconv_vote_accumulate_counted(const float* probs, const float* logits, const int64_t* point_idx, int64_t n_rows, int C, double smooth,
                                    float* test_probs, int64_t n_cloud, int32_t* bad_count, int32_t* visits, crf_stream_t stream);
int crfconv_vote_fold(float* acc, int32_t* acc_visits, const float* later, const int32_t* later_visits, int64_t n, int C, double smooth,
                      crf_stream_t stream);

int crfconv_vote_project(const float* test_probs, const int64_t* proj_idx, int64_t n_proj, int C, int64_t n_cloud,
                         int label_offset, uint8_t* preds, int32_t* bad_count, crf_stream_t stream);

size_t crfconv_argmin_workspace(void);
int crfconv_argmin_f64(const double* values, int64_t n, double* out_value, int64_t* out_index, void* workspace,
                       size_t workspace_bytes, crf_stream_t stream);

size_t crfconv_possibility_crop_workspace(int64_t n, int64_t k);
int crfconv_possibility_crop(const float* points, int64_t n, int64_t k, const int64_t* pick_index, const double* noise,
                             const int64_t* perm, const double* point_weight, double* possibility, int64_t* out_idx,
                             float* out_xyz, double* out_center, void* workspace, size_t workspace_bytes,
                             crf_stream_t stream);

#ifdef __cplusplus
}
#endif
#endif
```

Measured before the change: 44.48 M points/s.

## Recompute narrow-input MLP pre-activation instead of storing it for backward

For MLP blocks with small input width (Ci<=16) and Co>=2*Ci, the forward pass no longer writes the pre-BN output y. A stats-only linear kernel produces the BN records, and a fused apply kernel recomputes x@W^T with MFMA before applying BN, skip and leaky ReLU. The backward kernels rebuild y from x and W on the fly. This trades extra cheap MFMA work for less HBM traffic and memory, since the wide y tensor is never written or re-read. It is on by default through an environment flag.

After: 44.72 M points/s (median of 6 runs). About the same (+0.5%).

```diff
diff --git a/crfconv_amd/_lib.py b/crfconv_amd/_lib.py
--- a/crfconv_amd/_lib.py
+++ b/crfconv_amd/_lib.py
@@ -95,6 +95,11 @@
     'crfconv_mlp_dw_jobs_hosting': (_i, [_vp, _i, _vp, _vp, _vp, _vp, _vp, _i, _vp, _vp]),
     'crfconv_mlp_backward_add': (_i, [_vp, _vp, _vp, _vp, _vp, _f, _i64, _i, _i, _vp, _vp, _vp, _vp, _vp, _vp, _sz, _vp, _vp]),
     'crfconv_mlp_backward_cat': (_i, [_vp, _vp, _vp, _vp, _i, _vp, _vp, _f, _i64, _i, _i, _vp, _vp, _vp, _vp, _vp, _vp, _sz, _vp, _vp]),
+    'crfconv_mlp_rc_supported': (_i, [_i64, _i, _i]),
+    'crfconv_linear_forward_stats_only': (_i, [_vp, _vp, _i64, _i, _i, _vp, _vp]),
+    'crfconv_mlp_rc_apply': (_i, [_vp, _i64, _vp, _vp, _i64, _i, _i, _vp, _vp, _vp, _vp, _f, _f, _vp, _f, _vp, _vp, _vp]),
+    'crfconv_mlp_backward_rc_workspace': (_sz, [_i64, _i, _i]),
+    'crfconv_mlp_backward_rc': (_i, [_vp, _vp, _vp, _vp, _f, _i64, _i, _i, _vp, _vp, _vp, _vp, _vp, _vp, _sz, _vp, _vp]),
     'crfconv_bn_workspace': (_sz, [_i64, _i]),
     'crfconv_bn_forward': (_i, [_vp, _i64, _i, _vp, _vp, _vp, _vp, _f, _f, _i, _f, _vp, _vp, _vp, _sz, _vp]),
     'crfconv_bn_backward': (_i, [_vp, _vp, _vp, _i64, _i, _i, _f, _vp, _vp, _vp, _vp, _sz, _vp]),
diff --git a/crfconv_amd/csrc/linear.hip b/crfconv_amd/csrc/linear.hip
--- a/crfconv_amd/csrc/linear.hip
+++ b/crfconv_amd/csrc/linear.hip
@@ -39,7 +39,7 @@
     bcoef[4 * Co + c] = (float)(-a * c2 + a * c3 * rs * mu);
 }
 
-template <int TCO, int TCI>
+template <int TCO, int TCI, bool RC = false>
 __global__ __launch_bounds__(WG_BLOCK) void mlp_bwd_p1_kernel(const float* __restrict__ GA, const float* __restrict__ Y,
                                                               const float* __restrict__ X,
                                                               const float* __restrict__ X2, int split ,
@@ -51,7 +51,8 @@
                                                               float* __restrict__ PX ,
                                                               unsigned* __restrict__ ticket ,
                                                               float* __restrict__ dgamma, float* __restrict__ dbeta,
-                                                              float* __restrict__ bcoef) {
+                                                              float* __restrict__ bcoef, const float* __restrict__ W1 = nullptr) {
+    static_assert(!RC || TCI == 1, "the rebuilt y takes Ci <= 16");
     const int lane = threadIdx.x & 63, wave = threadIdx.x >> 6;
     const int co_base = blockIdx.y * 16 * TCO, ci_base = blockIdx.z * 16 * TCI;
     const int kk = lane >> 4, cc = lane & 15;
@@ -74,14 +75,27 @@
     }
 #pragma unroll
     for (int b = 0; b < TCI; ++b) sx[b] = 0.f;
+    [[maybe_unused]] float4 w1r[RC ? TCO : 1];
+    if constexpr (RC) {
+#pragma unroll
+        for (int a = 0; a < TCO; ++a) {
+            const int co = co_base + 16 * a + cc;
+            w1r[a] = (co < Co && 4 * kk < Ci) ? *reinterpret_cast<const float4*>(W1 + (int64_t)co * Ci + 4 * kk)
+                                              : make_float4(0.f, 0.f, 0.f, 0.f);
+        }
+    }
 
     const int64_t row_begin = (int64_t)blockIdx.x * rows_per_block;
     const int64_t row_end = row_begin + rows_per_block < M ? row_begin + rows_per_block : M;
 #ifndef P1_PREFETCH_
 #define P1_PREFETCH_ 0
 #endif
-    struct Frag { float gv[4][TCO], yv[4][TCO], bv[4][TCI]; };
+    struct Frag { float gv[4][TCO], yv[4][TCO], bv[4][TCI]; float4 xr; bool ok[4][TCO]; };
     auto load = [&](int64_t r0, Frag& f) {
+        if constexpr (RC) {
+            const int64_t r = r0 + 4 * (cc & 3) + (cc >> 2);
+            f.xr = (r < row_end && 4 * kk < Ci) ? *reinterpret_cast<const float4*>(X + r * Ci + 4 * kk) : make_float4(0.f, 0.f, 0.f, 0.f);
+        }
 #pragma unroll
         for (int u = 0; u < 4; ++u) {
             const int64_t r = r0 + 4 * u + kk;
@@ -91,7 +105,8 @@
                 const int co = co_base + 16 * a + cc;
                 const bool ok = rv && co < Co;
                 f.gv[u][a] = ok ? GA[r * Co + co] : 0.f;
-                f.yv[u][a] = ok ? Y[r * Co + co] : cm[a];
+                if constexpr (!RC) f.yv[u][a] = ok ? Y[r * Co + co] : cm[a];
+                else f.ok[u][a] = ok;
             }
 #pragma unroll
             for (int b = 0; b < TCI; ++b) {
@@ -102,7 +117,22 @@
             }
         }
     };
-    auto compute = [&](const Frag& f) {
+    auto compute = [&](const Frag& f0) {
+        [[maybe_unused]] Frag fr;
+        if constexpr (RC) {
+            fr = f0;
+#pragma unroll
+            for (int a = 0; a < TCO; ++a) {
+                f32x4 ya = f32x4{0.f, 0.f, 0.f, 0.f};
+                ya = __builtin_amdgcn_mfma_f32_16x16x4f32(f0.xr.x, w1r[a].x, ya, 0, 0, 0);
+                ya = __builtin_amdgcn_mfma_f32_16x16x4f32(f0.xr.y, w1r[a].y, ya, 0, 0, 0);
+                ya = __builtin_amdgcn_mfma_f32_16x16x4f32(f0.xr.z, w1r[a].z, ya, 0, 0, 0);
+                ya = __builtin_amdgcn_mfma_f32_16x16x4f32(f0.xr.w, w1r[a].w, ya, 0, 0, 0);
+#pragma unroll
+                for (int u = 0; u < 4; ++u) fr.yv[u][a] = f0.ok[u][a] ? ya[u] : cm[a];
+            }
+        }
+        const Frag& f = RC ? fr : f0;
 #pragma unroll
         for (int u = 0; u < 4; ++u) {
 #pragma unroll
@@ -774,11 +804,12 @@
 #endif
 constexpr int LF_BLOCK = LF_BLOCK_, LF_WAVES = LF_BLOCK / WAVE;
 
-constexpr int EPI_NONE = 0, EPI_ADD = 1, EPI_DROPOUT = 2;
+constexpr int EPI_NONE = 0, EPI_ADD = 1, EPI_DROPOUT = 2, EPI_STATS = 3;
+constexpr int RC_LD = 20;
 #ifndef LF_PF_MAX_
 #define LF_PF_MAX_ 4
 #endif
-template <int TCO, bool PRO = false, bool VEC4 = true, int EPI = EPI_NONE, int NCH = 0>
+template <int TCO, bool PRO = false, bool VEC4 = true, int EPI = EPI_NONE, int NCH = 0, bool RC = false>
 __global__ __launch_bounds__(LF_BLOCK) void linear_fwd_kernel(const float* __restrict__ X, const float* __restrict__ W,
                                                               const float* __restrict__ bias, int64_t M, int Ci, int Co,
                                                               int transpose_w, float* __restrict__ Y,
@@ -790,16 +821,26 @@
                                                               const float* __restrict__ addend = nullptr,
                                                               const long long* __restrict__ drop_counter = nullptr,
                                                               unsigned long long drop_seed = 0ull, unsigned drop_threshold = 0u,
-                                                              float drop_scale = 1.f) {
+                                                              float drop_scale = 1.f, const float* __restrict__ W1 = nullptr,
+                                                              int rci = 0) {
+    static_assert(!RC || (PRO && NCH > 0 && VEC4), "the rebuilt-y prologue is a form of the hoisted dX kernel");
+    static_assert(EPI != EPI_STATS || !PRO, "statistics-only is a forward form");
     extern __shared__ float sW[];
     const int Cip = ((Ci + 15) / 16) * 16 + 4;
     const int Cik = ((Ci + 15) / 16) * 16;
     float* sPro = sW + 16 * TCO * Cip;
     [[maybe_unused]] float* sTile = sPro + (PRO ? 5 * Cik : 0);
+    [[maybe_unused]] float* sW1 = sTile + (TCO >= 2 ? LF_WAVES * 16 * (16 * TCO + 4) : 0);
     if constexpr (PRO) {
         for (int t = threadIdx.x; t < 5 * Cik; t += LF_BLOCK) {
             const int which = t / Cik, k = t - which * Cik;
             sPro[t] = k < Ci ? pro[which * Ci + k] : 0.f;
+        }
+    }
+    if constexpr (RC) {
+        for (int t = threadIdx.x; t < Cik * RC_LD; t += LF_BLOCK) {
+            const int r = t / RC_LD, k = t - r * RC_LD;
+            sW1[t] = (r < Ci && k < rci) ? W1[(int64_t)r * rci + k] : 0.f;
         }
     }
     const int co_base = blockIdx.y * 16 * TCO;
@@ -846,6 +887,12 @@
         const int k0 = 16 * c + 4 * g;
         xa = zero4;
         xb2 = zero4;
+        if constexpr (RC) {
+            if (!rv) return;
+            if (k0 < Ci) xa = *reinterpret_cast<const float4*>(X + r * Ci + k0);
+            if (c == 0 && 4 * g < rci) xb2 = *reinterpret_cast<const float4*>(Y2 + r * rci + 4 * g);
+            return;
+        }
         if (!rv || k0 >= Ci) return;
         if constexpr (PRO) {
             xa = *reinterpret_cast<const float4*>(X + r * Ci + k0);
@@ -866,6 +913,15 @@
     auto operand = [&](bool rv, int c, float4 gv, float4 yv) -> float4 {
         if constexpr (PRO) {
             const int k0 = 16 * c + 4 * g;
+            if constexpr (RC) {
+                const float4 wv = *reinterpret_cast<const float4*>(sW1 + (16 * c + rr) * RC_LD + 4 * g);
+                f32x4 ya = f32x4{0.f, 0.f, 0.f, 0.f};
+                ya = __builtin_amdgcn_mfma_f32_16x16x4f32(wv.x, yv.x, ya, 0, 0, 0);
+                ya = __builtin_amdgcn_mfma_f32_16x16x4f32(wv.y, yv.y, ya, 0, 0, 0);
+                ya = __builtin_amdgcn_mfma_f32_16x16x4f32(wv.z, yv.z, ya, 0, 0, 0);
+                ya = __builtin_amdgcn_mfma_f32_16x16x4f32(wv.w, yv.w, ya, 0, 0, 0);
+                yv = make_float4(ya[0], ya[1], ya[2], ya[3]);
+            }
             float4 xv = zero4;
             if (rv && k0 < Ci) {
                 const float4 pa = *reinterpret_cast<const float4*>(sPro + k0), pb = *reinterpret_cast<const float4*>(sPro + Cik + k0);
@@ -913,7 +969,7 @@
 #pragma unroll
             for (int c = 0; c < NCH; ++c) {
                 const int k0 = 16 * c + 4 * g;
-                const float4 xv = operand(rv, c, fa[c], fb[PRO ? c : 0]);
+                const float4 xv = operand(rv, c, fa[c], fb[(PRO && !RC) ? c : 0]);
 #pragma unroll
                 for (int t = 0; t < TCO; ++t) {
                     const float4 wv = *reinterpret_cast<const float4*>(sW + (16 * t + rr) * Cip + k0);
@@ -946,7 +1002,8 @@
             }
         }
         }
-        if constexpr (TCO >= 2) {
+        if constexpr (EPI == EPI_STATS) {
+        } else if constexpr (TCO >= 2) {
             constexpr int TW = 16 * TCO, TLD = TW + 4, F4R = TW / 4;
             float* tile = sTile + wave * 16 * TLD;
 #pragma unroll
@@ -1261,6 +1318,62 @@
     else bn_apply_records_body<false, 4>(rec, nrec, M, C, gamma, beta, eps, run_mean, run_var, momentum, coef, x, nullptr, slope, rows, y, slab, tile);
 }
 
+template <bool ADD>
+__global__ __launch_bounds__(FR_BLOCK) void mlp_rc_apply_kernel(const float* __restrict__ rec, int nrec, const float* __restrict__ X,
+                                                               const float* __restrict__ W, int64_t M, int Ci, int Co,
+                                                               const float* __restrict__ gamma, const float* __restrict__ beta,
+                                                               float eps, float* __restrict__ run_mean, float* __restrict__ run_var,
+                                                               float momentum, float* __restrict__ coef, const float* __restrict__ skip,
+                                                               float slope, int rows_per_tile, float* __restrict__ out) {
+    __shared__ __attribute__((aligned(16))) float sW[FR_CH * RC_LD];
+    __shared__ __attribute__((aligned(16))) float s_ab[2][FR_CH];
+    const int slab = blockIdx.y, tile = blockIdx.x;
+    for (int t = threadIdx.x; t < FR_CH * RC_LD; t += FR_BLOCK) {
+        const int r = t / RC_LD, k = t - r * RC_LD;
+        sW[t] = k < Ci ? W[(int64_t)(FR_CH * slab + r) * Ci + k] : 0.f;
+    }
+    const int lane = threadIdx.x & 63, wave = threadIdx.x >> 6, rr = lane & 15, g = lane >> 4;
+    const int64_t r0 = (int64_t)tile * rows_per_tile;
+    const int64_t r1 = r0 + rows_per_tile < M ? r0 + rows_per_tile : M;
+    const int c = FR_CH * slab + 4 * g;
+    const bool kv = 4 * g < Ci;
+    float4 xv, sk;
+    auto request = [&](int64_t row0) {
+        const int64_t r = row0 + rr;
+        const bool rv = r < r1;
+        xv = (rv && kv) ? *reinterpret_cast<const float4*>(X + r * Ci + 4 * g) : make_float4(0.f, 0.f, 0.f, 0.f);
+        if constexpr (ADD) sk = rv ? *reinterpret_cast<const float4*>(skip + r * Co + c) : make_float4(0.f, 0.f, 0.f, 0.f);
+    };
+    request(r0 + 16 * wave);
+    float ab[2];
+    if (bn_finalize_records_body<8>(rec, nrec, M, Co, gamma, beta, eps, run_mean, run_var, momentum, coef, slab, tile == 0, ab)) {
+        s_ab[0][threadIdx.x] = ab[0];
+        s_ab[1][threadIdx.x] = ab[1];
+    }
+    __syncthreads();
+    const float4 a = *reinterpret_cast<const float4*>(&s_ab[0][4 * g]), b = *reinterpret_cast<const float4*>(&s_ab[1][4 * g]);
+    const float4 wv = *reinterpret_cast<const float4*>(sW + rr * RC_LD + 4 * g);
+    for (int64_t row0 = r0 + 16 * wave; row0 < r1; row0 += 16 * (FR_BLOCK / WAVE)) {
+        if (row0 != r0 + 16 * wave) request(row0);
+        const int64_t r = row0 + rr;
+        f32x4 acc = f32x4{0.f, 0.f, 0.f, 0.f};
+        acc = __builtin_amdgcn_mfma_f32_16x16x4f32(wv.x, xv.x, acc, 0, 0, 0);
+        acc = __builtin_amdgcn_mfma_f32_16x16x4f32(wv.y, xv.y, acc, 0, 0, 0);
+        acc = __builtin_amdgcn_mfma_f32_16x16x4f32(wv.z, xv.z, acc, 0, 0, 0);
+        acc = __builtin_amdgcn_mfma_f32_16x16x4f32(wv.w, xv.w, acc, 0, 0, 0);
+        if (r >= r1) continue;
+        float4 o = make_float4(fmaf(a.x, acc[0], b.x), fmaf(a.y, acc[1], b.y), fmaf(a.z, acc[2], b.z), fmaf(a.w, acc[3], b.w));
+        if constexpr (ADD) {
+            o.x = add_rn(o.x, sk.x); o.y = add_rn(o.y, sk.y); o.z = add_rn(o.z, sk.z); o.w = add_rn(o.w, sk.w);
+        }
+        o.x = o.x > 0.f ? o.x : slope * o.x;
+        o.y = o.y > 0.f ? o.y : slope * o.y;
+        o.z = o.z > 0.f ? o.z : slope * o.z;
+        o.w = o.w > 0.f ? o.w : slope * o.w;
+        *reinterpret_cast<float4*>(out + r * Co + c) = o;
+    }
+}
+
 static int lf_blocks(int64_t M) {
     constexpr int cap = 512;
     int64_t nb = (M + 16 * LF_WAVES - 1) / (16 * LF_WAVES);
@@ -1447,6 +1560,53 @@
     return CRF_OK;
 }
 
+extern "C" int crfconv_mlp_rc_supported(int64_t M, int Ci, int Co) {
+    if (!(M > 0 && Ci >= 4 && Ci <= 16 && Ci % 4 == 0 && (Co == 16 || Co == 32 || Co == 64))) return 0;
+    return crfconv_linear_forward_supported(Ci, Co) && crfconv_mlp_backward_supported(M, Ci, Co) == 1 ? 1 : 0;
+}
+
+extern "C" int crfconv_linear_forward_stats_only(const float* X, const float* W, int64_t M, int Ci, int Co, float* stat_rec,
+                                                 crf_stream_t stream) {
+    CRF_REQUIRE(X && W && stat_rec, CRF_ERR_ARG, "null pointer");
+    CRF_REQUIRE(crfconv_mlp_rc_supported(M, Ci, Co) == 1, CRF_ERR_UNSUPPORTED, "shape M=%lld Ci=%d Co=%d not supported", (long long)M, Ci, Co);
+    const int tiles = (Co + 15) / 16;
+    const int tco = lf_tco(Ci, Co, false);
+    const dim3 grid((unsigned)crf::lf_blocks(M), (unsigned)((tiles + tco - 1) / tco)), blk(crf::LF_BLOCK);
+    const size_t lds = lf_lds_bytes(Ci, Co, false);
+    CRF_REQUIRE(lf_hoist_chunks(Ci, true) == 1, CRF_ERR_UNSUPPORTED, "Ci=%d", Ci);
+    hipStream_t st = crf::as_stream(stream);
+#define LFS(T) hipLaunchKernelGGL((crf::linear_fwd_kernel<T, false, true, crf::EPI_STATS, 1>), grid, blk, lds, st, X, W, (const float*)nullptr, M, Ci, Co, 0, (float*)nullptr, stat_rec)
+    switch (tco) {
+        case 1: LFS(1); break;
+        case 2: LFS(2); break;
+        default: LFS(4); break;
+    }
+#undef LFS
+    CRF_LAUNCH_CHECK();
+    return CRF_OK;
+}
+
+extern "C" int crfconv_mlp_rc_apply(const float* stat_rec, int64_t nrec, const float* x, const float* W, int64_t M, int Ci, int Co,
+                                    const float* gamma, const float* beta, float* run_mean, float* run_var, float momentum, float eps,
+                                    const float* skip, float slope, float* coef, float* out, crf_stream_t stream) {
+    CRF_REQUIRE(stat_rec && x && W && gamma && beta && coef && out, CRF_ERR_ARG, "null pointer");
+    CRF_REQUIRE(crfconv_mlp_rc_supported(M, Ci, Co) == 1, CRF_ERR_UNSUPPORTED, "shape M=%lld Ci=%d Co=%d not supported", (long long)M, Ci, Co);
+    CRF_REQUIRE(nrec > 0 && nrec < ((int64_t)1 << 31), CRF_ERR_ARG, "bad record count");
+    const int slabs = Co / crf::FR_CH;
+    int64_t tiles, rows;
+    bn_apply_plan(M, Co, BN_APPLY_WGS_, tiles, rows);
+    const dim3 grid((unsigned)tiles, (unsigned)slabs), blk(crf::FR_BLOCK);
+    hipStream_t st = crf::as_stream(stream);
+    if (skip != nullptr)
+        hipLaunchKernelGGL(crf::mlp_rc_apply_kernel<true>, grid, blk, 0, st, stat_rec, (int)nrec, x, W, M, Ci, Co, gamma, beta, eps, run_mean,
+                           run_var, momentum, coef, skip, slope, (int)rows, out);
+    else
+        hipLaunchKernelGGL(crf::mlp_rc_apply_kernel<false>, grid, blk, 0, st, stat_rec, (int)nrec, x, W, M, Ci, Co, gamma, beta, eps, run_mean,
+                           run_var, momentum, coef, skip, slope, (int)rows, out);
+    CRF_LAUNCH_CHECK();
+    return CRF_OK;
+}
+
 namespace crf {
 struct MlpPlan {
     int tco, tci, gy, gz, nblk, rows_per_block;
@@ -1501,7 +1661,7 @@
 static int mlp_backward_impl(const float* gA, const float* Y, const float* X, const float* Xb, int xsplit, const float* W,
                              const float* coef, float slope, int64_t M, int Ci, int Co, float* dX, float* dXb, float* dW,
                              float* dgamma, float* dbeta, void* workspace, size_t workspace_bytes, unsigned* ticket,
-                             crf_stream_t stream, const float* dX_add = nullptr);
+                             crf_stream_t stream, const float* dX_add = nullptr, bool rc = false);
 
 extern "C" int crfconv_mlp_backward(const float* gA, const float* Y, const float* X, const float* W, const float* coef,
                                     float slope, int64_t M, int Ci, int Co, float* dX, float* dW, float* dgamma,
@@ -1518,6 +1678,16 @@
     CRF_REQUIRE(dX != nullptr || dX_add == nullptr, CRF_ERR_ARG, "dX_add without dX");
     return mlp_backward_impl(gA, Y, X, nullptr, 0, W, coef, slope, M, Ci, Co, dX, nullptr, dW, dgamma, dbeta, workspace,
                              workspace_bytes, ticket, stream, dX_add);
+}
+
+extern "C" size_t crfconv_mlp_backward_rc_workspace(int64_t M, int Ci, int Co) { return crfconv_mlp_backward_workspace(M, Ci, Co); }
+extern "C" int crfconv_mlp_backward_rc(const float* gA, const float* X, const float* W, const float* coef, float slope, int64_t M,
+                                       int Ci, int Co, const float* dX_add, float* dX, float* dW, float* dgamma, float* dbeta,
+                                       void* workspace, size_t workspace_bytes, unsigned* ticket, crf_stream_t stream) {
+    CRF_REQUIRE(dX != nullptr || dX_add == nullptr, CRF_ERR_ARG, "dX_add without dX");
+    CRF_REQUIRE(crfconv_mlp_rc_supported(M, Ci, Co) == 1, CRF_ERR_UNSUPPORTED, "shape M=%lld Ci=%d Co=%d not supported", (long long)M, Ci, Co);
+    return mlp_backward_impl(gA, nullptr, X, nullptr, 0, W, coef, slope, M, Ci, Co, dX, nullptr, dW, dgamma, dbeta, workspace,
+                             workspace_bytes, ticket, stream, dX_add, true);
 }
 
 extern "C" int crfconv_mlp_backward_cat(const float* gA, const float* Y, const float* Xa, const float* Xb, int split,
@@ -1588,8 +1758,8 @@
 static int mlp_backward_impl(const float* gA, const float* Y, const float* X, const float* Xb, int xsplit, const float* W,
                              const float* coef, float slope, int64_t M, int Ci, int Co, float* dX, float* dXb, float* dW,
                              float* dgamma, float* dbeta, void* workspace, size_t workspace_bytes, unsigned* ticket,
-                             crf_stream_t stream, const float* dX_add) {
-    CRF_REQUIRE(gA && Y && X && W && coef && dgamma && dbeta && workspace, CRF_ERR_ARG, "null pointer");
+                             crf_stream_t stream, const float* dX_add, bool rc) {
+    CRF_REQUIRE(gA && (Y || rc) && X && W && coef && dgamma && dbeta && workspace, CRF_ERR_ARG, "null pointer");
     CRF_REQUIRE(dX_add == nullptr || dXb == nullptr, CRF_ERR_ARG, "dX_add is for the one-operand form");
     CRF_REQUIRE(crfconv_mlp_backward_supported(M, Ci, Co) == 1, CRF_ERR_UNSUPPORTED, "shape M=%lld Ci=%d Co=%d not supported",
                 (long long)M, Ci, Co);
@@ -1604,10 +1774,15 @@
     float* PX = reinterpret_cast<float*>(base + off[3]);
     float* pro = reinterpret_cast<float*>(base + off[4]);
     const crf::MlpPlan p = crf::mlp_plan(M, Co, Ci);
+    CRF_REQUIRE(!rc || (p.tci == 1 && p.gz == 1 && Xb == nullptr), CRF_ERR_UNSUPPORTED, "rebuilt-y form: Ci=%d", Ci);
     if (!(2 * Co <= crf::WG_BLOCK && crf::WG_BLOCK % (Co / 2) == 0 && (int64_t)p.nblk * 2 * Co * 4 < ((int64_t)1 << 31))) ticket = nullptr;
     {
         const dim3 grid((unsigned)p.nblk, (unsigned)p.gy, (unsigned)p.gz), blk(crf::WG_BLOCK);
 #define P1(TA, TB) hipLaunchKernelGGL((crf::mlp_bwd_p1_kernel<TA, TB>), grid, blk, 0, st, gA, Y, X, Xb, xsplit, coef, slope, M, Co, Ci, p.rows_per_block, PA, PB, PG, PX, ticket, dgamma, dbeta, pro)
+#define P1RC(TA) hipLaunchKernelGGL((crf::mlp_bwd_p1_kernel<TA, 1, true>), grid, blk, 0, st, gA, Y, X, Xb, xsplit, coef, slope, M, Co, Ci, p.rows_per_block, PA, PB, PG, PX, ticket, dgamma, dbeta, pro, W)
+        if (rc) {
+            if (p.tco == 1) P1RC(1); else if (p.tco == 2) P1RC(2); else P1RC(4);
+        } else
         switch (p.tco * 10 + p.tci) {
             case 11: P1(1, 1); break;
             case 12: P1(1, 2); break;
@@ -1619,6 +1794,7 @@
             default: P1(4, 2); break;
         }
 #undef P1
+#undef P1RC
         CRF_LAUNCH_CHECK();
     }
     const int nw = dW != nullptr ? (int)crf::cdiv((int64_t)Co * Ci, 64) : 0;
@@ -1634,9 +1810,19 @@
         const int tco = lf_tco(gCi, gCo, true);
         const int gy = (tiles + tco - 1) / tco;
         const dim3 grid((unsigned)crf::lf_blocks(M), (unsigned)gy), blk(crf::LF_BLOCK);
-        const size_t lds = lf_lds_bytes(gCi, gCo, true);
+        const size_t lds = lf_lds_bytes(gCi, gCo, true) + (rc ? sizeof(float) * (size_t)((gCi + 15) / 16 * 16) * crf::RC_LD : 0);
         const bool vec4 = (gCi % 4) == 0 && (gCo % 4) == 0;
         const int nch = lf_hoist_chunks(gCi, vec4);
+        if (rc) {
+            CRF_REQUIRE(tco == 1 && vec4 && (nch == 1 || nch == 2 || nch == 4) && lds <= 64 * 1024, CRF_ERR_UNSUPPORTED, "rebuilt-y dX: Co=%d", Co);
+#define DXR(E, N) hipLaunchKernelGGL((crf::linear_fwd_kernel<1, true, true, E, N, true>), grid, blk, lds, st, gA, W, (const float*)nullptr, M, gCi, gCo, 1, dX, (float*)nullptr, X, pro, slope, (const float*)nullptr, 0, (float*)nullptr, 0, dX_add, (const long long*)nullptr, 0ull, 0u, 1.f, W, Ci)
+#define DXR2(E) do { if (nch == 1) DXR(E, 1); else if (nch == 2) DXR(E, 2); else DXR(E, 4); } while (0)
+            if (dX_add != nullptr) DXR2(crf::EPI_ADD); else DXR2(crf::EPI_NONE);
+#undef DXR2
+#undef DXR
+            CRF_LAUNCH_CHECK();
+            return CRF_OK;
+        }
 #define DX4(T, V, E, N) hipLaunchKernelGGL((crf::linear_fwd_kernel<T, true, V, E, N>), grid, blk, lds, st, gA, W, (const float*)nullptr, M, gCi, gCo, 1, dX, (float*)nullptr, Y, pro, slope, (const float*)nullptr, 0, dXb, xsplit, dX_add)
 #define DX3(T, V, E) do { if (V && nch == 1) DX4(T, V, E, 1); else if (V && nch == 2) DX4(T, V, E, 2); else if (V && nch == 4) DX4(T, V, E, 4); else if (V && nch == 8) DX4(T, V, E, 8); else DX4(T, V, E, 0); } while (0)
 #define DX2(T, V) do { if (dX_add != nullptr) DX3(T, V, crf::EPI_ADD); else DX3(T, V, crf::EPI_NONE); } while (0)
diff --git a/crfconv_amd/ops/_base.py b/crfconv_amd/ops/_base.py
--- a/crfconv_amd/ops/_base.py
+++ b/crfconv_amd/ops/_base.py
@@ -134,6 +134,7 @@
     small_bwd_one_launch = __import__('os').environ.get('CRFCONV_SMALL_BWD_TWO_LAUNCHES') is None
     dw_hosts_mats = __import__('os').environ.get('CRFCONV_NO_TAIL_RIDERS') is None
     mfma_min_rows = 12288
+    mlp_recompute = __import__('os').environ.get('CRFCONV_MLP_RECOMPUTE', '1') != '0'
     mf_block = __import__('os').environ.get('CRFCONV_MF_BLOCK', 'auto')
     mf_block_min_rows = 65536
     mf_block_min_locality = 0.6
diff --git a/crfconv_amd/ops/mlp.py b/crfconv_amd/ops/mlp.py
--- a/crfconv_amd/ops/mlp.py
+++ b/crfconv_amd/ops/mlp.py
@@ -16,12 +16,15 @@
         Wc = W.contiguous()
         m, ci = x.shape
         co = Wc.shape[0]
-        y, rec = _mfma_matmul(x, Wc, None, False, True)
         coef = torch.empty(4 * co, dtype=torch.float32, device=x.device)
         g, b = _f32c(gamma), _f32c(beta)
-        out = torch.empty_like(y)
-        _lib.call('crfconv_bn_apply_from_records', ptr(rec), rec.shape[0], ptr(y), m, co, ptr(g), ptr(b), ptr(run_mean), ptr(run_var),
-                  float(momentum), float(eps), None, float(slope), ptr(coef), ptr(out), stream_ptr())
+        if _rc_ok(m, ci, co):
+            y, out = None, _rc_forward(x, Wc, g, b, run_mean, run_var, momentum, eps, None, slope, coef)
+        else:
+            y, rec = _mfma_matmul(x, Wc, None, False, True)
+            out = torch.empty_like(y)
+            _lib.call('crfconv_bn_apply_from_records', ptr(rec), rec.shape[0], ptr(y), m, co, ptr(g), ptr(b), ptr(run_mean), ptr(run_var),
+                      float(momentum), float(eps), None, float(slope), ptr(coef), ptr(out), stream_ptr())
         ctx.prm = (W, gamma, beta)
         ctx.save_for_backward(x, Wc, y, coef)
         ctx.slope = float(slope)
@@ -36,18 +39,40 @@
         m, ci = x.shape
         co = W.shape[0]
         dev = x.device
-        gA = torch.zeros_like(y) if gA is None else gA.contiguous()
+        gA = torch.zeros((m, co), dtype=torch.float32, device=dev) if gA is None else gA.contiguous()
         dX = torch.empty_like(x) if ctx.needs_input_grad[0] else None
         add = _f32c(g_alias) if (g_alias is not None and dX is not None) else None
         outs, dfr = _mlp_param_outs(ctx.prm, W, dev)
         dW, dgamma, dbeta = (o[0] for o in outs)
         nbytes = _lib.load().crfconv_mlp_backward_workspace(m, ci, co)
         ws = torch.empty(nbytes, dtype=torch.uint8, device=dev)
-        _lib.call('crfconv_mlp_backward_add', ptr(gA), ptr(y), ptr(x), ptr(W), ptr(coef), ctx.slope, m, ci, co, ptr(add), ptr(dX),
-                  ptr(None if dfr else dW), ptr(dgamma), ptr(dbeta), ptr(ws), nbytes, _mlp_ticket(dev), stream_ptr())
+        if y is None:
+            _lib.call('crfconv_mlp_backward_rc', ptr(gA), ptr(x), ptr(W), ptr(coef), ctx.slope, m, ci, co, ptr(add), ptr(dX),
+                      ptr(None if dfr else dW), ptr(dgamma), ptr(dbeta), ptr(ws), nbytes, _mlp_ticket(dev), stream_ptr())
+        else:
+            _lib.call('crfconv_mlp_backward_add', ptr(gA), ptr(y), ptr(x), ptr(W), ptr(coef), ctx.slope, m, ci, co, ptr(add), ptr(dX),
+                      ptr(None if dfr else dW), ptr(dgamma), ptr(dbeta), ptr(ws), nbytes, _mlp_ticket(dev), stream_ptr())
         return dX, *_mlp_param_rets(ctx.prm, outs, dfr, ws, m, ci, co, coef), None, None, None, None, None, None
 
 
+
+
+def _rc_ok(m, ci, co):
+    return state.mlp_recompute and co >= 2 * ci and _lib.load().crfconv_mlp_rc_supported(m, ci, co) == 1
+
+
+def _rc_forward(x, Wc, g, b, run_mean, run_var, momentum, eps, skip, slope, coef):
+    m, ci = x.shape
+    co = Wc.shape[0]
+    lib = _lib.load()
+    st = stream_ptr()
+    nrec = lib.crfconv_linear_forward_stat_records(m)
+    rec = torch.empty((nrec, co, 4), dtype=torch.float32, device=x.device)
+    _lib.call('crfconv_linear_forward_stats_only', ptr(x), ptr(Wc), m, ci, co, ptr(rec), st)
+    out = torch.empty((m, co), dtype=torch.float32, device=x.device)
+    _lib.call('crfconv_mlp_rc_apply', ptr(rec), nrec, ptr(x), ptr(Wc), m, ci, co, ptr(g), ptr(b), ptr(run_mean), ptr(run_var),
+              float(momentum), float(eps), ptr(skip), float(slope), ptr(coef), ptr(out), st)
+    return out
 
 
 class _MLPBlockJoin(torch.autograd.Function):
@@ -57,12 +82,14 @@
         x, Wc, skip = x.contiguous(), W.contiguous(), skip.contiguous()
         m, ci = x.shape
         co = Wc.shape[0]
-        y, rec = _mfma_matmul(x, Wc, None, False, True)
         coef = torch.empty(4 * co, dtype=torch.float32, device=x.device)
-        st = stream_ptr()
-        out = torch.empty_like(y)
-        _lib.call('crfconv_bn_apply_from_records', ptr(rec), rec.shape[0], ptr(y), m, co, ptr(_f32c(gamma)), ptr(_f32c(beta)),
-                  ptr(run_mean), ptr(run_var), float(momentum), float(eps), ptr(skip), float(slope), ptr(coef), ptr(out), st)
+        if _rc_ok(m, ci, co):
+            y, out = None, _rc_forward(x, Wc, _f32c(gamma), _f32c(beta), run_mean, run_var, momentum, eps, skip, slope, coef)
+        else:
+            y, rec = _mfma_matmul(x, Wc, None, False, True)
+            out = torch.empty_like(y)
+            _lib.call('crfconv_bn_apply_from_records', ptr(rec), rec.shape[0], ptr(y), m, co, ptr(_f32c(gamma)), ptr(_f32c(beta)),
+                      ptr(run_mean), ptr(run_var), float(momentum), float(eps), ptr(skip), float(slope), ptr(coef), ptr(out), stream_ptr())
         ctx.prm = (W, gamma, beta)
         ctx.save_for_backward(x, Wc, y, coef, out)
         ctx.slope = float(slope)
@@ -83,8 +110,12 @@
         dW, dgamma, dbeta = (o[0] for o in outs)
         nbytes = _lib.load().crfconv_mlp_backward_workspace(m, ci, co)
         ws = torch.empty(nbytes, dtype=torch.uint8, device=dev)
-        _lib.call('crfconv_mlp_backward', ptr(g1), ptr(y), ptr(x), ptr(W), ptr(coef), 1.0, m, ci, co, ptr(dX), ptr(None if dfr else dW),
-                  ptr(dgamma), ptr(dbeta), ptr(ws), nbytes, _mlp_ticket(dev), st)
+        if y is None:
+            _lib.call('crfconv_mlp_backward_rc', ptr(g1), ptr(x), ptr(W), ptr(coef), 1.0, m, ci, co, None, ptr(dX),
+                      ptr(None if dfr else dW), ptr(dgamma), ptr(dbeta), ptr(ws), nbytes, _mlp_ticket(dev), st)
+        else:
+            _lib.call('crfconv_mlp_backward', ptr(g1), ptr(y), ptr(x), ptr(W), ptr(coef), 1.0, m, ci, co, ptr(dX), ptr(None if dfr else dW),
+                      ptr(dgamma), ptr(dbeta), ptr(ws), nbytes, _mlp_ticket(dev), st)
         gskip = g1 if ctx.needs_input_grad[8] else None
         return dX, *_mlp_param_rets(ctx.prm, outs, dfr, ws, m, ci, co, coef), None, None, None, None, gskip, None
 
diff --git a/include/crfconv_amd.h b/include/crfconv_amd.h
--- a/include/crfconv_amd.h
+++ b/include/crfconv_amd.h
@@ -284,6 +284,15 @@
 int crfconv_mlp_backward_add(const float* gA, const float* Y, const float* X, const float* W, const float* coef, float slope,
                              int64_t M, int Ci, int Co, const float* dX_add, float* dX, float* dW, float* dgamma, float* dbeta,
                              void* workspace, size_t workspace_bytes, unsigned* ticket, crf_stream_t stream);
+int crfconv_mlp_rc_supported(int64_t M, int Ci, int Co);
+int crfconv_linear_forward_stats_only(const float* X, const float* W, int64_t M, int Ci, int Co, float* stat_rec, crf_stream_t stream);
+int crfconv_mlp_rc_apply(const float* stat_rec, int64_t nrec, const float* x, const float* W, int64_t M, int Ci, int Co,
+                         const float* gamma, const float* beta, float* run_mean, float* run_var, float momentum, float eps,
+                         const float* skip, float slope, float* coef, float* out, crf_stream_t stream);
+size_t crfconv_mlp_backward_rc_workspace(int64_t M, int Ci, int Co);
+int crfconv_mlp_backward_rc(const float* gA, const float* X, const float* W, const float* coef, float slope, int64_t M, int Ci, int Co,
+                            const float* dX_add, float* dX, float* dW, float* dgamma, float* dbeta, void* workspace,
+                            size_t workspace_bytes, unsigned* ticket, crf_stream_t stream);
 int crfconv_linear_forward_cat(const float* Xa, const float* Xb, int split, const float* W, const float* bias, int64_t M,
                                int Ci, int Co, float* Y, float* stat_rec, crf_stream_t stream);
 int crfconv_mlp_backward_cat(const float* gA, const float* Y, const float* Xa, const float* Xb, int split, const float* W,
```
